# talmolab/VNL-Brax-Imitation

Hardware: AMD Instinct MI355X
Metric: env-steps/sec (whole node), rodent imitation, num_envs=4096/GPU (higher is better)
Workload: dtype f32; 1 GPU; rodent imitation rollout, single groom clip, 4096 envs/GPU: intention-policy forward (HIP) -> RodentTracking.step (5 substeps, CG 6/6) -> auto-reset on -> Transition logging (unroll 20, the 20 steps replayed as one captured hipGraph); envs_per_gpu=4096, clips=1, parallelism=env-sharded x1, no data-path collective

## Files before the change

### __graft_entry__.py

```python
from __future__ import annotations

import os
import sys

ROOT = os.path.dirname(os.path.abspath(__file__))
if ROOT not in sys.path:
    sys.path.insert(0, ROOT)


def build() -> None:
    import vnl_brax_imitation_amd
    from vnl_brax_imitation_amd.csrc import build as hip_build

    from concurrent.futures import ThreadPoolExecutor

    with ThreadPoolExecutor(5) as pool:
        futs = {v: pool.submit(hip_build.build, variant=v) for v in ("product", "spill", "noblk", "nospec", "tail")}
        paths = {v: f.result() for v, f in futs.items()}
    path = paths["product"]
    assert all(os.path.exists(p_) for p_ in paths.values()), paths
    from oracle import oracle as _oracle

    _oracle.build()
    from vnl_brax_imitation_amd import _lib

    _lib.load_library(path)
    print(f"[build] {path} ok; oracle ok")


def smoke() -> None:
    import numpy as np
    import torch

    sys.path.insert(0, os.path.join(ROOT, "tests"))
    import helpers as H
    from vnl_brax_imitation_amd.envs.rodent import RodentTracking

    assert torch.cuda.is_available(), "smoke() needs a HIP device"
    B = 256
    env = RodentTracking(H.reference_clip(), num_envs=B, device="cuda:0", **H.env_kwargs())
    rng = np.random.default_rng(0)
    sf = rng.integers(0, 235, B).astype(np.int32)
    noise = (1e-3 * rng.standard_normal((B, 74))).astype(np.float32)
    st = env.reset(start_frame=torch.from_numpy(sf), noise=torch.from_numpy(noise))
    act = np.clip(0.3 * rng.standard_normal((B, 30)), -1, 1).astype(np.float32)
    o = H.make_oracle(env, "f64")
    ost = o.env_reset(sf, noise)
    e_reset = H.scaled_err(st.pipeline_state.qacc_warmstart.cpu().numpy(), ost["qacc_warmstart"])
    e_obs = H.scaled_err(st.obs.cpu().numpy(), ost["obs"])
    import parity as P

    o32 = H.make_oracle(env, "f32")
    st, err, dev, rep, ost = P.control_step_follow(env, o, o32, sf, noise, act)
    torch.cuda.synchronize()
    print(f"[smoke] reset qacc err {e_reset:.2e}, obs err {e_obs:.2e}; control step vs oracle (following the product's "
          f"solver decisions): qvel err max {err['qvel'].max():.2e} median {np.median(err['qvel']):.2e}, qpos max "
          f"{err['qpos'].max():.2e}; reward {st.reward.mean().item():.5f} vs {ost['reward'].mean():.5f}")
    w = int(np.argmax(err["qvel"]))
    print(f"[smoke] worst env {w}: product vs float64 oracle {err['qvel'][w]:.2e}, float32 oracle vs float64 oracle "
          f"{dev['qvel'][w]:.2e} on the same env (bound: max(1e-5, {P.K_SENS} x that))")
    cp, co = P.compliance(err), P.compliance(dev)
    print(f"[smoke] envs within 1e-5 after ONE CONTROL STEP ({B} envs): product qpos {cp['qpos']:.3f} qvel {cp['qvel']:.3f} | "
          f"float32 oracle qpos {co['qpos']:.3f} qvel {co['qvel']:.3f}")
    env1 = RodentTracking(H.reference_clip(), num_envs=B, device="cuda:0", **{**H.env_kwargs(), "n_frames": 1})
    o1, o1_32 = H.make_oracle(env1, "f64"), H.make_oracle(env1, "f32")
    _, err1, dev1, rep1, _ = P.control_step_follow(env1, o1, o1_32, sf, noise, act)
    cp1, co1 = P.compliance(err1), P.compliance(dev1)
    print(f"[smoke] envs within 1e-5 after ONE SUBSTEP: product qpos {cp1['qpos']:.3f} qvel {cp1['qvel']:.3f} | float32 oracle "
          f"qpos {co1['qpos']:.3f} qvel {co1['qvel']:.3f}; followed decisions: {P.assert_legitimate(rep1)}")
    for f, idx in P.bound_violations(err1, dev1).items():
        assert len(idx) == 0, (f, idx[:8], err1[f][idx[:8]], dev1[f][idx[:8]])
    assert e_reset < 1e-4 and e_obs < 1e-5, (e_reset, e_obs)
    P.check_control_step(err, dev, rep)
    assert np.abs(st.reward.cpu().numpy() - ost["reward"]).max() < 2e-4
    assert np.array_equal(st.done.cpu().numpy(), ost["done"].astype(np.float32))
    assert torch.isfinite(st.obs).all()


if __name__ == "__main__":
    build()
    if "--smoke" in sys.argv:
        smoke()
```

### include/vnl.h

```cpp
#ifndef VNL_H_
#define VNL_H_

#include <stddef.h>
#include <stdint.h>

#ifdef __cplusplus
extern "C" {
#endif

#define VNL_OK 0
#define VNL_ERR_ARG -1
#define VNL_ERR_BLOB -2
#define VNL_ERR_HIP -3
#define VNL_ERR_NO_DEVICE -4
#define VNL_ERR_UNSUPPORTED -5

typedef struct vnl_model vnl_model;
typedef struct vnl_env vnl_env;
typedef struct vnl_policy vnl_policy;

typedef struct vnl_envspec {
  int32_t clip_frames;
  int32_t num_clips;
  int32_t ref_traj_length;
  int32_t sub_clip_length;
  int32_t n_frames;
  int32_t num_track_bodies;
  int32_t num_end_eff;
  int32_t num_appendages;
  int32_t num_joint_cols;
  int32_t com_ref_col;
  const int32_t* body_idxs;
  const int32_t* end_eff_idx;
  const int32_t* app_body;
  const int32_t* app_ref_col;
  const int32_t* joint_cols;
  float healthy_z_lo, healthy_z_hi;
  float termination_threshold;
  float body_error_multiplier;
  const float* position;
  const float* quaternion;
  const float* joints;
  const float* body_positions;
  const float* velocity;
  const float* angular_velocity;
  const float* joints_velocity;
  int32_t flags;
  float done_threshold;
  const float* center_of_mass;
  float reward_weights[6];
} vnl_envspec;
#define VNL_ENV_REWARD_OLD_STATE 1
#define VNL_ENV_TERM_MEAN 2
#define VNL_ENV_NO_RAPP 4
#define VNL_ENV_OBS_QPOS_QVEL 8
#define VNL_ENV_WEIGHTS 16
#define VNL_ENV_RACT_ACTION 32
#define VNL_ENV_METRICS_UNSCALED 64
#define VNL_ENV_TRAJ_OLD_FRAME 128

typedef struct vnl_state {
  float* qpos;
  float* qvel;
  float* act;
  float* qacc_warmstart;
  float* xpos;
  float* xquat;
  float* subtree_com1;
  float* qfrc_actuator;
  float* obs;
  float* reward;
  float* done;
  float* metrics;
  float* traj;
  float* termination_error;
  int32_t* cur_frame;
  int32_t* sub_clip_frame;
  int32_t* clip_id;
} vnl_state;

typedef struct vnl_dims {
  int32_t nq, nv, nu, nbody, njnt, ngeom_collide, ncon, nefc, obs_size, traj_size;
  int32_t workspace_floats_per_env;
  int32_t workgroups_per_cu;
  int32_t nbody_dynamic;
  int32_t kernel_specialised;
  int32_t factor_route;
} vnl_dims;

const char* vnl_last_error(void);
int vnl_version(void);

int vnl_model_create(const void* blob, size_t nbytes, vnl_model** out);
void vnl_model_destroy(vnl_model*);

int vnl_env_create(const vnl_model*, const vnl_envspec*, int32_t num_envs, int32_t device, vnl_env** out);
void vnl_env_destroy(vnl_env*);
int vnl_env_dims(const vnl_env*, vnl_dims* out);

int vnl_env_reset(vnl_env*, const int32_t* start_frame, const float* noise, const vnl_state* state, void* stream);

int vnl_env_step(vnl_env*, const float* action, const vnl_state* state, void* stream);
int vnl_env_fk(vnl_env* env, const float* qpos, const vnl_state* state, void* stream);

typedef struct vnl_domain {
  const double *cg_friction, *act_gain, *dof_damping, *dof_armature;
} vnl_domain;
int vnl_env_set_domain(vnl_env* env, const vnl_domain* domain, void* stream);

typedef struct vnl_body_domain {
  const double *body_mass, *body_inertia, *body_ipos;
} vnl_body_domain;
int vnl_env_set_body_domain(vnl_env* env, const vnl_body_domain* domain, void* stream);

int vnl_env_debug(vnl_env*, int32_t enable, int32_t* row_stride);
int vnl_env_scratch(const vnl_env*, const char* name, float** dev_ptr, int32_t* count);

typedef struct vnl_policy_spec {
  int32_t traj_size, obs_size, action_size, latent_size;
  int32_t num_encoder_layers, num_decoder_layers;
  int32_t encoder_layers[8], decoder_layers[8];
} vnl_policy_spec;

int vnl_policy_create(const vnl_policy_spec*, int32_t max_batch, int32_t device, vnl_policy** out);
void vnl_policy_destroy(vnl_policy*);
int64_t vnl_policy_num_params(const vnl_policy*);
int vnl_policy_forward(vnl_policy*, const float* params, const float* obs_mean, const float* obs_std,
                       const float* traj, const float* obs, const float* eps_latent, const float* eps_action,
                       int32_t batch, int32_t deterministic, float* action, float* raw_action, float* log_prob,
                       float* logits, float* latent_mean, float* latent_logvar,
                       const float* rand_action ,
                       float* rand_log_prob ,
                       void* stream);

typedef struct vnl_policy_noise {
  uint64_t seed;
  const int64_t* step_base;
  int64_t step_offset;
  int64_t env_offset;
  float *eps_latent_out, *eps_action_out, *rand_action_out;
} vnl_policy_noise;
int vnl_policy_forward_noise(vnl_policy*, const float* params, const float* obs_mean, const float* obs_std,
                             const float* traj, const float* obs, const vnl_policy_noise*, int32_t batch,
                             int32_t deterministic, float* action, float* raw_action, float* log_prob, float* logits,
                             float* latent_mean, float* latent_logvar, float* rand_log_prob , void* stream);

#define VNL_POST_MAX_OPS 24
typedef struct vnl_post_op {
  float* dst;
  const float* src;
  const float* first;
  float* log;
  int32_t width;
  int32_t pad_;
} vnl_post_op;
typedef struct vnl_post_desc {
  float *steps, *prev_done, *done, *truncation;
  const float* reward;
  float *log_reward, *log_discount, *log_truncation;
  int32_t episode_length, action_repeat, num_ops, pad_;
  vnl_post_op ops[VNL_POST_MAX_OPS];
} vnl_post_desc;
int vnl_rollout_post(const vnl_post_desc*, int32_t num_envs, void* stream);

typedef struct vnl_ppo_head_args {
  int32_t T, B, act, latent;
  const float *logits, *baseline, *bootstrap, *lat_mean, *lat_logvar;
  const float *raw_action, *behaviour_log_prob, *reward, *truncation, *discount, *eps_entropy;
  float entropy_cost, discounting, reward_scaling, gae_lambda, clipping_epsilon, kl_weight, min_std, var_scale;
  int32_t normalize_advantage, pad_;
  float *g_logits, *g_baseline, *g_lat_mean, *g_lat_logvar;
  float *vs, *advantages;
  float *metrics;
} vnl_ppo_head_args;
#define VNL_PPO_HEAD_WORKSPACE_FLOATS (4 + 4 * 256)
int vnl_ppo_head(const vnl_ppo_head_args*, float* workspace, void* stream);

typedef struct vnl_gather_op {
  float* dst;
  const float* src;
  int32_t T, width;
} vnl_gather_op;
typedef struct vnl_gather_desc {
  const int64_t* idx;
  int32_t N, M, num_ops, pad_;
  vnl_gather_op ops[VNL_POST_MAX_OPS];
} vnl_gather_desc;
int vnl_gather_rows(const vnl_gather_desc*, void* stream);

int vnl_adam_step(float* params, const float* grads, float* mu, float* nu, const int64_t* count, int64_t n,
                  double lr, double b1, double b2, double eps, void* stream);

typedef struct vnl_ppo_net_spec {
  int32_t traj_size, obs_size, action_size, latent_size;
  int32_t num_encoder_layers, num_decoder_layers , num_value_layers ;
  int32_t encoder_layers[8], decoder_layers[8], value_layers[8];
} vnl_ppo_net_spec;
typedef struct vnl_ppo_batch {
  const float *traj;
  const float *obs;
  const float *next_obs_last;
  const float *raw_action, *behaviour_log_prob, *reward, *truncation, *discount;
  const float *eps_latent;
  const float *eps_entropy;
  const float *obs_mean, *obs_std;
} vnl_ppo_batch;
typedef struct vnl_ppo_hparams {
  float entropy_cost, discounting, reward_scaling, gae_lambda, clipping_epsilon, kl_weight, min_std, var_scale;
  int32_t normalize_advantage, pad_;
} vnl_ppo_hparams;
typedef struct vnl_ppo_update vnl_ppo_update;
int vnl_ppo_update_create(const vnl_ppo_net_spec*, int32_t T, int32_t B, int32_t device, vnl_ppo_update** out);
void vnl_ppo_update_destroy(vnl_ppo_update*);
int64_t vnl_ppo_update_num_params(const vnl_ppo_update*);
int vnl_ppo_update_buffer(const vnl_ppo_update*, const char* name, float** dev_ptr, int64_t* count);
int vnl_ppo_minibatch_grad(vnl_ppo_update*, const float* params, const vnl_ppo_batch*, const vnl_ppo_hparams*, float* grads,
                           float* metrics, void* stream);
int vnl_ppo_minibatch_grad_part(vnl_ppo_update*, const float* params, const vnl_ppo_batch*, const vnl_ppo_hparams*, float* grads,
                                float* metrics, void* stream, int part);

typedef struct vnl_corr_plan {
  int32_t route;
  int32_t chunks, chunk_cols, row_tiles;
  int64_t workspace_floats;
} vnl_corr_plan;
int vnl_prediction_corr_plan(int32_t T, int32_t B, int32_t route_request, vnl_corr_plan* out);
int vnl_prediction_corr(const float* vs, const float* reward, float reward_scaling, int32_t T, int32_t B, int32_t route_request,
                        float* workspace, int64_t workspace_floats, float* out, void* stream);

#ifdef __cplusplus
}
#endif
#endif
```

### vnl-brax-imitation_amd/_lib.py

```python
from __future__ import annotations

import ctypes as C
import os

_HERE = os.path.dirname(os.path.abspath(__file__))
DEFAULT_LIB = os.path.join(_HERE, "csrc", "libvnl.so")

i32p = C.POINTER(C.c_int32)
f32p = C.POINTER(C.c_float)


class EnvSpec(C.Structure):
    _fields_ = [
        ("clip_frames", C.c_int32),
        ("num_clips", C.c_int32),
        ("ref_traj_length", C.c_int32),
        ("sub_clip_length", C.c_int32),
        ("n_frames", C.c_int32),
        ("num_track_bodies", C.c_int32),
        ("num_end_eff", C.c_int32),
        ("num_appendages", C.c_int32),
        ("num_joint_cols", C.c_int32),
        ("com_ref_col", C.c_int32),
        ("body_idxs", i32p),
        ("end_eff_idx", i32p),
        ("app_body", i32p),
        ("app_ref_col", i32p),
        ("joint_cols", i32p),
        ("healthy_z_lo", C.c_float),
        ("healthy_z_hi", C.c_float),
        ("termination_threshold", C.c_float),
        ("body_error_multiplier", C.c_float),
        ("position", f32p),
        ("quaternion", f32p),
        ("joints", f32p),
        ("body_positions", f32p),
        ("velocity", f32p),
        ("angular_velocity", f32p),
        ("joints_velocity", f32p),
        ("flags", C.c_int32),
        ("done_threshold", C.c_float),
        ("center_of_mass", f32p),
        ("reward_weights", C.c_float * 6),
    ]


ENV_REWARD_OLD_STATE, ENV_TERM_MEAN, ENV_NO_RAPP, ENV_OBS_QPOS_QVEL = 1, 2, 4, 8
ENV_WEIGHTS, ENV_RACT_ACTION, ENV_METRICS_UNSCALED, ENV_TRAJ_OLD_FRAME = 16, 32, 64, 128


STATE_FLOAT_FIELDS = ("qpos", "qvel", "act", "qacc_warmstart", "xpos", "xquat", "subtree_com1", "qfrc_actuator",
                      "obs", "reward", "done", "metrics", "traj", "termination_error")
STATE_INT_FIELDS = ("cur_frame", "sub_clip_frame", "clip_id")


class StatePtrs(C.Structure):
    _fields_ = [(n, C.c_void_p) for n in STATE_FLOAT_FIELDS + STATE_INT_FIELDS]


class Dims(C.Structure):
    _fields_ = [(n, C.c_int32) for n in ("nq", "nv", "nu", "nbody", "njnt", "ngeom_collide", "ncon", "nefc",
                                          "obs_size", "traj_size", "workspace_floats_per_env", "workgroups_per_cu",
                                          "nbody_dynamic", "kernel_specialised", "factor_route")]


class PolicySpec(C.Structure):
    _fields_ = [
        ("traj_size", C.c_int32),
        ("obs_size", C.c_int32),
        ("action_size", C.c_int32),
        ("latent_size", C.c_int32),
        ("num_encoder_layers", C.c_int32),
        ("num_decoder_layers", C.c_int32),
        ("encoder_layers", C.c_int32 * 8),
        ("decoder_layers", C.c_int32 * 8),
    ]


class PolicyNoise(C.Structure):
    _fields_ = [("seed", C.c_uint64), ("step_base", C.c_void_p), ("step_offset", C.c_int64), ("env_offset", C.c_int64),
                ("eps_latent_out", C.c_void_p), ("eps_action_out", C.c_void_p), ("rand_action_out", C.c_void_p)]


POST_MAX_OPS = 24


class PostOp(C.Structure):
    _fields_ = [("dst", C.c_void_p), ("src", C.c_void_p), ("first", C.c_void_p), ("log", C.c_void_p),
                ("width", C.c_int32), ("pad_", C.c_int32)]


class PostDesc(C.Structure):
    _fields_ = [(n, C.c_void_p) for n in ("steps", "prev_done", "done", "truncation", "reward", "log_reward",
                                          "log_discount", "log_truncation")] + \
               [("episode_length", C.c_int32), ("action_repeat", C.c_int32), ("num_ops", C.c_int32),
                ("pad_", C.c_int32), ("ops", PostOp * POST_MAX_OPS)]


class GatherOp(C.Structure):
    _fields_ = [("dst", C.c_void_p), ("src", C.c_void_p), ("T", C.c_int32), ("width", C.c_int32)]


class GatherDesc(C.Structure):
    _fields_ = [("idx", C.c_void_p), ("N", C.c_int32), ("M", C.c_int32), ("num_ops", C.c_int32), ("pad_", C.c_int32),
                ("ops", GatherOp * POST_MAX_OPS)]


class PPOHeadArgs(C.Structure):
    _fields_ = [(n, C.c_int32) for n in ("T", "B", "act", "latent")] + \
               [(n, C.c_void_p) for n in ("logits", "baseline", "bootstrap", "lat_mean", "lat_logvar", "raw_action",
                                          "behaviour_log_prob", "reward", "truncation", "discount", "eps_entropy")] + \
               [(n, C.c_float) for n in ("entropy_cost", "discounting", "reward_scaling", "gae_lambda",
                                         "clipping_epsilon", "kl_weight", "min_std", "var_scale")] + \
               [("normalize_advantage", C.c_int32), ("pad_", C.c_int32)] + \
               [(n, C.c_void_p) for n in ("g_logits", "g_baseline", "g_lat_mean", "g_lat_logvar", "vs", "advantages",
                                          "metrics")]


PPO_HEAD_WORKSPACE_FLOATS = 4 + 4 * 256


class PPONetSpec(C.Structure):
    _fields_ = [(n, C.c_int32) for n in ("traj_size", "obs_size", "action_size", "latent_size", "num_encoder_layers",
                                          "num_decoder_layers", "num_value_layers")] + \
               [("encoder_layers", C.c_int32 * 8), ("decoder_layers", C.c_int32 * 8), ("value_layers", C.c_int32 * 8)]


class PPOBatch(C.Structure):
    _fields_ = [(n, C.c_void_p) for n in ("traj", "obs", "next_obs_last", "raw_action", "behaviour_log_prob", "reward",
                                          "truncation", "discount", "eps_latent", "eps_entropy", "obs_mean", "obs_std")]


class PPOHParams(C.Structure):
    _fields_ = [(n, C.c_float) for n in ("entropy_cost", "discounting", "reward_scaling", "gae_lambda",
                                         "clipping_epsilon", "kl_weight", "min_std", "var_scale")] + \
               [("normalize_advantage", C.c_int32), ("pad_", C.c_int32)]

class CorrPlan(C.Structure):
    _fields_ = [(n, C.c_int32) for n in ("route", "chunks", "chunk_cols", "row_tiles")] + [("workspace_floats", C.c_int64)]


class Domain(C.Structure):
    _fields_ = [(n, C.c_void_p) for n in ("cg_friction", "act_gain", "dof_damping", "dof_armature")]

class BodyDomain(C.Structure):
    _fields_ = [(n, C.c_void_p) for n in ("body_mass", "body_inertia", "body_ipos")]


EXPORTS = (
    "vnl_last_error", "vnl_version", "vnl_model_create", "vnl_model_destroy", "vnl_env_create", "vnl_env_destroy",
    "vnl_env_dims", "vnl_env_reset", "vnl_env_step", "vnl_env_fk", "vnl_env_debug", "vnl_env_scratch", "vnl_policy_create", "vnl_policy_destroy",
    "vnl_policy_num_params", "vnl_policy_forward", "vnl_policy_forward_noise", "vnl_rollout_post", "vnl_ppo_head", "vnl_adam_step", "vnl_gather_rows",
    "vnl_ppo_update_create", "vnl_ppo_update_destroy", "vnl_ppo_update_num_params", "vnl_ppo_update_buffer",
    "vnl_ppo_minibatch_grad",
    "vnl_ppo_minibatch_grad_part",
    "vnl_env_set_domain", "vnl_env_set_body_domain",
    "vnl_prediction_corr_plan", "vnl_prediction_corr",
)
_HIP_ONLY = ("vnl_policy_", "vnl_ppo_update_", "vnl_ppo_minibatch_", "vnl_prediction_corr")


class VnlError(RuntimeError):
    pass


def _declare(lib: C.CDLL) -> C.CDLL:
    vp = C.c_void_p
    lib.vnl_last_error.restype = C.c_char_p
    lib.vnl_version.restype = C.c_int
    lib.vnl_model_create.argtypes = [vp, C.c_size_t, C.POINTER(vp)]
    lib.vnl_model_destroy.argtypes = [vp]
    lib.vnl_model_destroy.restype = None
    lib.vnl_env_create.argtypes = [vp, C.POINTER(EnvSpec), C.c_int32, C.c_int32, C.POINTER(vp)]
    lib.vnl_env_destroy.argtypes = [vp]
    lib.vnl_env_destroy.restype = None
    lib.vnl_env_dims.argtypes = [vp, C.POINTER(Dims)]
    lib.vnl_env_reset.argtypes = [vp, vp, vp, C.POINTER(StatePtrs), vp]
    lib.vnl_env_step.argtypes = [vp, vp, C.POINTER(StatePtrs), vp]
    lib.vnl_env_fk.argtypes = [vp, vp, C.POINTER(StatePtrs), vp]
    lib.vnl_env_debug.argtypes = [vp, C.c_int32, C.POINTER(C.c_int32)]
    lib.vnl_env_scratch.argtypes = [vp, C.c_char_p, C.POINTER(vp), C.POINTER(C.c_int32)]
    lib.vnl_env_set_domain.argtypes = [vp, C.POINTER(Domain), vp]
    lib.vnl_env_set_body_domain.argtypes = [vp, C.POINTER(BodyDomain), vp]
    lib.vnl_rollout_post.argtypes = [C.POINTER(PostDesc), C.c_int32, vp]
    lib.vnl_ppo_head.argtypes = [C.POINTER(PPOHeadArgs), vp, vp]
    lib.vnl_gather_rows.argtypes = [C.POINTER(GatherDesc), vp]
    lib.vnl_adam_step.argtypes = [vp, vp, vp, vp, vp, C.c_int64] + [C.c_double] * 4 + [vp]
    if hasattr(lib, "vnl_ppo_update_create"):
        lib.vnl_ppo_update_create.argtypes = [C.POINTER(PPONetSpec), C.c_int32, C.c_int32, C.c_int32, C.POINTER(vp)]
        lib.vnl_ppo_update_destroy.argtypes = [vp]
        lib.vnl_ppo_update_destroy.restype = None
        lib.vnl_ppo_update_num_params.argtypes = [vp]
        lib.vnl_ppo_update_num_params.restype = C.c_int64
        lib.vnl_ppo_update_buffer.argtypes = [vp, C.c_char_p, C.POINTER(vp), C.POINTER(C.c_int64)]
        lib.vnl_ppo_minibatch_grad.argtypes = [vp, vp, C.POINTER(PPOBatch), C.POINTER(PPOHParams), vp, vp, vp]
        lib.vnl_ppo_minibatch_grad_part.argtypes = [vp, vp, C.POINTER(PPOBatch), C.POINTER(PPOHParams), vp, vp, vp, C.c_int]
        lib.vnl_prediction_corr_plan.argtypes = [C.c_int32, C.c_int32, C.c_int32, C.POINTER(CorrPlan)]
        lib.vnl_prediction_corr.argtypes = [vp, vp, C.c_float, C.c_int32, C.c_int32, C.c_int32, vp, C.c_int64, vp, vp]
    if hasattr(lib, "vnl_policy_create"):
        lib.vnl_policy_create.argtypes = [C.POINTER(PolicySpec), C.c_int32, C.c_int32, C.POINTER(vp)]
        lib.vnl_policy_destroy.argtypes = [vp]
        lib.vnl_policy_destroy.restype = None
        lib.vnl_policy_num_params.argtypes = [vp]
        lib.vnl_policy_num_params.restype = C.c_int64
        lib.vnl_policy_forward.argtypes = [vp] + [vp] * 7 + [C.c_int32, C.c_int32] + [vp] * 6 + [vp, vp] + [vp]
        lib.vnl_policy_forward_noise.argtypes = [vp] + [vp] * 5 + [C.POINTER(PolicyNoise), C.c_int32, C.c_int32] + [vp] * 7 + [vp]
    return lib


_cache = {}


def load_library(path: str | None = None, env_only: bool = False) -> C.CDLL:
    path = os.path.abspath(path or os.environ.get("VNL_LIB", DEFAULT_LIB))
    if path not in _cache:
        if not os.path.exists(path):
            raise VnlError(
                f"HIP extension not found at {path}. Build it with `python -c 'import __graft_entry__ as g; "
                "g.build()'` (hipcc --offload-arch=gfx950). There is no CPU fallback for the rollout.")
        lib = C.CDLL(path)
        missing = [s for s in EXPORTS if not hasattr(lib, s) and not (env_only and s.startswith(_HIP_ONLY))]
        if missing:
            raise VnlError(f"{path} lacks symbols {missing}")
        _cache[path] = _declare(lib)
    return _cache[path]


def check(lib: C.CDLL, rc: int) -> None:
    if rc != 0:
        raise VnlError(f"vnl error {rc}: {lib.vnl_last_error().decode()}")
```

### vnl-brax-imitation_amd/csrc/build.py

```python
from __future__ import annotations

import os
import subprocess
import sys

HERE = os.path.dirname(os.path.abspath(__file__))
SOURCES = ["vnl_lib.hip", "vnl_policy.hip", "vnl_ppo.hip", "vnl_domain.hip"]
DEPS = SOURCES + ["vnl_env_kernels.h", "vnl_body.h", "vnl_types.h", "vnl_policy_train.h", "../../include/vnl.h"]
OUT = os.path.join(HERE, "libvnl.so")

VARIANTS = {
    "product": ("libvnl.so", ["-DVNL_KERNEL_ATTR=__attribute__((amdgpu_waves_per_eu(2,2)))"]),
    "prof": ("libvnl_prof.so", ["-DVNL_PROFILE", "-DVNL_KERNEL_ATTR=__attribute__((amdgpu_waves_per_eu(2,2)))"]),
    "knobs": ("libvnl_knobs.so", ["-DVNL_STAGE_KNOBS", "-DVNL_KERNEL_ATTR=__attribute__((amdgpu_waves_per_eu(2,2)))"]),
    "spill": ("libvnl_spill.so", ["-DVNL_KERNEL_ATTR=__attribute__((amdgpu_waves_per_eu(4,4)))"]),
    "noblk": ("libvnl_noblk.so", ["-DVNL_NO_BLK", "-DVNL_KERNEL_ATTR=__attribute__((amdgpu_waves_per_eu(2,2)))"]),
    "tail": ("libvnl_tail.so", ["-DVNL_SOLVER_TAIL", "-DVNL_KERNEL_ATTR=__attribute__((amdgpu_waves_per_eu(2,2)))"]),
    "nospec": ("libvnl_nospec.so", ["-DVNL_NO_SPEC", "-DVNL_KERNEL_ATTR=__attribute__((amdgpu_waves_per_eu(2,2)))"]),
}
ENV_KERNELS = ("vnl_step_kernel", "vnl_reset_kernel")


def resource_usage(stderr_text: str) -> dict:
    out, name = {}, None
    for line in stderr_text.splitlines():
        if "Function Name:" in line:
            name = line.split("Function Name:")[1].split()[0]
            out[name] = {}
        elif name and "remark:" in line:
            body = line.split("remark:")[1].split("[-Rpass")[0].strip()
            key, _, val = body.rpartition(":")
            try:
                out[name][key.strip()] = int(val.strip())
            except ValueError:
                pass
    return out


def build(force: bool = False, verbose: bool = False, profile: bool = False, knobs: bool = False,
          variant: str | None = None) -> str:
    variant = variant or ("prof" if profile else ("knobs" if knobs else "product"))
    fname, defs = VARIANTS[variant]
    out = os.path.join(HERE, fname)
    deps = [os.path.join(HERE, d) for d in DEPS] + [os.path.abspath(__file__)]
    newest = max(os.path.getmtime(d) for d in deps)
    if not force and os.path.exists(out) and os.path.getmtime(out) >= newest:
        return out
    hipcc = os.environ.get("HIPCC", "/opt/rocm/bin/hipcc")
    objdir = os.path.join(HERE, "_obj", variant)
    os.makedirs(objdir, exist_ok=True)
    flags = ["-Rpass-analysis=kernel-resource-usage", "--offload-arch=gfx950", "-O3", "-fno-slp-vectorize", "-std=c++17", "-fPIC"] + \
        defs + os.environ.get("VNL_HIPCC_EXTRA", "").split()
    stamp = " ".join(flags)
    headers = [d for d in deps if not d.endswith(".hip")]
    SRC_DEPS = {"vnl_lib.hip": headers, "vnl_policy.hip": [h for h in headers if h.endswith("vnl.h")] + [os.path.join(HERE, "vnl_policy_train.h")],
                "vnl_ppo.hip": [h for h in headers if h.endswith("vnl.h")] + [os.path.join(HERE, "vnl_policy_train.h")]}
    objs, remarks = [], ""
    for src in SOURCES:
        obj = os.path.join(objdir, src + ".o")
        rem = obj + ".remarks.txt"
        srcdeps = [os.path.join(HERE, src)] + [h for h in SRC_DEPS.get(src, headers) if os.path.exists(h)]
        fresh = (not force and os.path.exists(obj) and os.path.exists(rem) and
                 os.path.getmtime(obj) >= max(os.path.getmtime(d) for d in srcdeps) and
                 open(rem).readline().rstrip("\n") == stamp)
        if not fresh:
            cmd = [hipcc] + flags + ["-c", os.path.join(HERE, src), "-o", obj]
            if verbose:
                print(" ".join(cmd), file=sys.stderr)
            r = subprocess.run(cmd, stderr=subprocess.PIPE, text=True)
            if verbose or r.returncode:
                sys.stderr.write(r.stderr)
            if r.returncode:
                raise subprocess.CalledProcessError(r.returncode, cmd)
            with open(rem, "w") as f:
                f.write(stamp + "\n" + r.stderr)
        objs.append(obj)
        remarks += open(rem).read().split("\n", 1)[1]
    cmd = [hipcc, "--offload-arch=gfx950", "-shared", "-fPIC", "-o", out] + objs
    r = subprocess.run(cmd, stderr=subprocess.PIPE, text=True)
    if r.returncode:
        sys.stderr.write(r.stderr)
        raise subprocess.CalledProcessError(r.returncode, cmd)

    class _R:
        stderr = remarks
    r = _R()
    usage = resource_usage(r.stderr)
    seen = {k: [u for n, u in usage.items() if k in n] for k in ENV_KERNELS}
    missing = [k for k, v in seen.items() if not v or "Occupancy [waves/SIMD]" not in v[0]]
    if missing:
        os.remove(out)
        raise RuntimeError(f"no resource-usage remark for {missing}: cannot check the register budget of this build")
    if variant == "product":
        for k, u in ((k, u) for k, v in seen.items() for u in v):
            if u.get("ScratchSize [bytes/lane]", 0) > 64 or u["Occupancy [waves/SIMD]"] < 2:
                if os.environ.get("VNL_ALLOW_SPILL") != "1":
                    os.remove(out)
                    raise RuntimeError(
                        f"{k}: {u.get('VGPRs')} VGPRs, {u.get('ScratchSize [bytes/lane]')} B scratch per lane, "
                        f"{u['Occupancy [waves/SIMD]']} waves/SIMD -- below the two waves per SIMD without spilling that the "
                        "published numbers were measured with.  Results do not depend on spilling (tests/test_gpu_spill.py); "
                        "this gate keeps a performance regression from shipping silently: set VNL_ALLOW_SPILL=1 to build anyway")
                sys.stderr.write(f"[build] WARNING (performance): {k} uses {u.get('VGPRs')} VGPRs, "
                                 f"{u.get('ScratchSize [bytes/lane]')} B scratch per lane, "
                                 f"{u['Occupancy [waves/SIMD]']} waves/SIMD: below the two waves per SIMD without "
                                 "spilling that the published numbers were measured with\n")
    with open(os.path.join(HERE, fname + ".resources.txt"), "w") as f:
        for n, u in usage.items():
            f.write(n + " " + " ".join(f"{a}={b}" for a, b in sorted(u.items())) + "\n")
    return out


if __name__ == "__main__":
    v = next((k for k in VARIANTS if "--" + k in sys.argv), None)
    if "--profile" in sys.argv:
        v = "prof"
    print(build(force="--force" in sys.argv, verbose=True, variant=v))
```

### vnl-brax-imitation_amd/csrc/vnl_body.h

```cpp
#pragma once
#include <math.h>

#include "vnl_types.h"

#ifndef VNL_HD
#define VNL_HD __device__ __forceinline__
#endif

#ifndef VNL_FORKJOIN_DEFINED
#define VNL_LANES 64
#define VNL_ROWS_PER_LANE 8
#define VNL_ROWS_SMALL 5
#define VNL_CHAIN_WIDTH 8
#define VNL_ROWSETS_1 1
#define VNL_ROWSETS_2 2
#define VNL_FOR(i, n) for (int i = (int)lane; i < (n); i += VNL_LANES)
#define VNL_SERIAL if (lane == 0)
#define VNL_SYNC() __builtin_amdgcn_fence(__ATOMIC_ACQ_REL, "wavefront")
#define VNL_SYNC_GLOBAL()                                     \
  do {                                                        \
    __builtin_amdgcn_fence(__ATOMIC_ACQ_REL, "wavefront");    \
    asm volatile("s_waitcnt vmcnt(0)" ::: "memory");          \
    __builtin_amdgcn_fence(__ATOMIC_ACQ_REL, "wavefront");    \
  } while (0)
#define VNL_LDS_DECL(name) extern __shared__ __align__(16) vreal name[]
VNL_HD float vnl_wave_sum(float x) {
#define VNL_DPP_STEP(ctrl) x += __builtin_bit_cast(float, __builtin_amdgcn_update_dpp(0, __builtin_bit_cast(int, x), ctrl, 0xf, 0xf, true))
  VNL_DPP_STEP(0xB1);
  VNL_DPP_STEP(0x4E);
  VNL_DPP_STEP(0x141);
  VNL_DPP_STEP(0x140);
#undef VNL_DPP_STEP
  x += __builtin_bit_cast(float, __builtin_amdgcn_update_dpp(0, __builtin_bit_cast(int, x), 0x142, 0xa, 0xf, false));
  x += __builtin_bit_cast(float, __builtin_amdgcn_update_dpp(0, __builtin_bit_cast(int, x), 0x143, 0xc, 0xf, false));
  return __builtin_bit_cast(float, __builtin_amdgcn_readlane(__builtin_bit_cast(int, x), 63));
}
VNL_HD float vnl_wave_sum16(float x) {
#define VNL_DPP_STEP(ctrl) x += __builtin_bit_cast(float, __builtin_amdgcn_update_dpp(0, __builtin_bit_cast(int, x), ctrl, 0xf, 0xf, true))
  VNL_DPP_STEP(0xB1);
  VNL_DPP_STEP(0x4E);
  VNL_DPP_STEP(0x141);
  VNL_DPP_STEP(0x140);
#undef VNL_DPP_STEP
  return __builtin_bit_cast(float, __builtin_amdgcn_readlane(__builtin_bit_cast(int, x), 0));
}
VNL_HD bool vnl_wave_any(bool x) { return __ballot(x) != 0ull; }
VNL_HD float vnl_wave_scan(float x) {
#define VNL_DPP_SCAN(ctrl, rmask) \
  x += __builtin_bit_cast(float, __builtin_amdgcn_update_dpp(0, __builtin_bit_cast(int, x), ctrl, rmask, 0xf, false))
  VNL_DPP_SCAN(0x111, 0xf);
  VNL_DPP_SCAN(0x112, 0xf);
  VNL_DPP_SCAN(0x114, 0xf);
  VNL_DPP_SCAN(0x118, 0xf);
  VNL_DPP_SCAN(0x142, 0xa);
  VNL_DPP_SCAN(0x143, 0xc);
#undef VNL_DPP_SCAN
  return x;
}
#define VNL_SCAN_ADD(x, run) (x = vnl_wave_scan(x))
#define VNL_WAVE_ITEMS(n) VNL_LANES
#define VNL_PAD_ITEMS(n) (((n) + VNL_LANES - 1) / VNL_LANES * VNL_LANES)
#define VNL_SCAN_ADD_C(x, run, carry) \
  (x = vnl_wave_scan(x) + carry, carry = __builtin_bit_cast(float, __builtin_amdgcn_readlane(__builtin_bit_cast(int, x), 63)))
#define VNL_PERLANE(T, name) T name
#define VNL_AT(name, j) name
#define VNL_GETF(name, a) __builtin_bit_cast(float, __builtin_amdgcn_readlane(__builtin_bit_cast(int, name), a))
#define VNL_GETI(name, a) __builtin_amdgcn_readlane(name, a)
#define VNL_ROWGETI(name, q, l) __builtin_amdgcn_readlane(name[q], l)
#define VNL_ROWGETF(expr, q, l) __builtin_bit_cast(float, __builtin_amdgcn_readlane(__builtin_bit_cast(int, expr), l))
VNL_HD float vnl_seg_sum(float x, unsigned cont, int steps) {
#define VNL_DPP_SEG(ctrl, bit)                                                                                          \
  do {                                                                                                                  \
    const float t_ = __builtin_bit_cast(float, __builtin_amdgcn_update_dpp(0, __builtin_bit_cast(int, x), ctrl, 0xf, 0xf, true)); \
    x += (cont & (bit)) ? t_ : 0.0f;                                                                                     \
  } while (0)
  if (steps > 0) VNL_DPP_SEG(0x101, 1u);
  if (steps > 1) VNL_DPP_SEG(0x102, 2u);
  if (steps > 2) VNL_DPP_SEG(0x104, 4u);
  if (steps > 3) VNL_DPP_SEG(0x108, 8u);
#undef VNL_DPP_SEG
  return x;
}
#define VNL_SEG_SUM(part, dsc, steps) (part = vnl_seg_sum(part, (dsc) >> 28, steps))
#define VNL_WAVE_FENCE() __builtin_amdgcn_fence(__ATOMIC_ACQ_REL, "wavefront")
#define VNL_LINE_HEADERS(out, base, stride)                                                       \
  do {                                                                                            \
    int hv_ = (int)(base)[((int)lane < VNL_FAC_LINES ? (int)lane : VNL_FAC_LINES - 1) * (stride)]; \
    _Pragma("unroll") for (int k_ = 0; k_ < VNL_FAC_LINES; k_++) out[k_] = __builtin_amdgcn_readlane(hv_, k_); \
  } while (0)
#define VNL_COUNT(pred) __popcll(__ballot(pred))
#define VNL_RANK(pred, run, rank)                                                   \
  do {                                                                              \
    const unsigned long long b_ = __ballot(pred);                                   \
    rank = run + (int)__popcll(b_ & ((1ull << (threadIdx.x & 63)) - 1ull));         \
    run += (int)__popcll(b_);                                                       \
  } while (0)
#define VNL_UNIFORM_I(x) __builtin_amdgcn_readfirstlane(x)
VNL_HD float vnl_recip(float x) {
  float r = __builtin_amdgcn_rcpf(x);
  return r * (2.0f - x * r);
}
#endif

#ifdef VNL_PROFILE
#define VNL_NPROF 40
__device__ unsigned long long g_vnl_prof[VNL_NPROF];
#define VNL_PROF(i)                                                                             \
  do {                                                                                          \
    if (lane == 0) {                                                                            \
      unsigned t_ = (unsigned)__builtin_amdgcn_s_memtime();                                     \
      s[LO(prof) + (i)] += (float)(t_ - __builtin_bit_cast(unsigned, (float)s[LO(prof) + VNL_NPROF])); \
      s[LO(prof) + VNL_NPROF] = __builtin_bit_cast(float, (unsigned)__builtin_amdgcn_s_memtime()); \
    }                                                                                           \
  } while (0)
#else
#define VNL_PROF(i)
#endif

#define VNL_MINVAL vreal(1e-15)
#define VNL_MINIMP vreal(0.0001)
#define VNL_MAXIMP vreal(0.9999)

struct V3 {
  vreal x, y, z;
};
VNL_HD V3 v3(vreal x, vreal y, vreal z) { return V3{x, y, z}; }
VNL_HD V3 operator+(V3 a, V3 b) { return V3{a.x + b.x, a.y + b.y, a.z + b.z}; }
VNL_HD V3 operator-(V3 a, V3 b) { return V3{a.x - b.x, a.y - b.y, a.z - b.z}; }
VNL_HD V3 operator*(V3 a, vreal s) { return V3{a.x * s, a.y * s, a.z * s}; }
VNL_HD vreal dot(V3 a, V3 b) { return a.x * b.x + a.y * b.y + a.z * b.z; }
VNL_HD V3 cross(V3 a, V3 b) { return V3{a.y * b.z - a.z * b.y, a.z * b.x - a.x * b.z, a.x * b.y - a.y * b.x}; }
struct Q4 {
  vreal w, x, y, z;
};
VNL_HD Q4 qmul(Q4 u, Q4 v) {
  return Q4{u.w * v.w - u.x * v.x - u.y * v.y - u.z * v.z, u.w * v.x + u.x * v.w + u.y * v.z - u.z * v.y,
            u.w * v.y - u.x * v.z + u.y * v.w + u.z * v.x, u.w * v.z + u.x * v.y - u.y * v.x + u.z * v.w};
}
VNL_HD V3 qrot(V3 v, Q4 q) {
  V3 u = v3(q.x, q.y, q.z);
  vreal uv = dot(u, v), uu = dot(u, u);
  V3 c = cross(u, v);
  return u * (vreal(2.) * uv) + v * (q.w * q.w - uu) + c * (vreal(2.) * q.w);
}
struct M3 {
  vreal a[9];
};
VNL_HD M3 qmat(Q4 q) {
  M3 m;
  vreal q00 = q.w * q.w, q01 = q.w * q.x, q02 = q.w * q.y, q03 = q.w * q.z;
  vreal q11 = q.x * q.x, q12 = q.x * q.y, q13 = q.x * q.z, q22 = q.y * q.y, q23 = q.y * q.z, q33 = q.z * q.z;
  m.a[0] = q00 + q11 - q22 - q33, m.a[1] = vreal(2.) * (q12 - q03), m.a[2] = vreal(2.) * (q13 + q02);
  m.a[3] = vreal(2.) * (q12 + q03), m.a[4] = q00 - q11 + q22 - q33, m.a[5] = vreal(2.) * (q23 - q01);
  m.a[6] = vreal(2.) * (q13 - q02), m.a[7] = vreal(2.) * (q23 + q01), m.a[8] = q00 - q11 - q22 + q33;
  return m;
}
VNL_HD V3 mmul(const M3& m, V3 v) {
  return V3{m.a[0] * v.x + m.a[1] * v.y + m.a[2] * v.z, m.a[3] * v.x + m.a[4] * v.y + m.a[5] * v.z,
            m.a[6] * v.x + m.a[7] * v.y + m.a[8] * v.z};
}
struct S6 {
  V3 a, l;
};
VNL_HD S6 operator+(S6 p, S6 q) { return S6{p.a + q.a, p.l + q.l}; }
VNL_HD S6 operator*(S6 p, vreal s) { return S6{p.a * s, p.l * s}; }
VNL_HD vreal dot(S6 p, S6 q) { return dot(p.a, q.a) + dot(p.l, q.l); }
VNL_HD S6 mcross(S6 u, S6 v) { return S6{cross(u.a, v.a), cross(u.l, v.a) + cross(u.a, v.l)}; }
VNL_HD S6 mcross_force(S6 v, S6 f) { return S6{cross(v.a, f.a) + cross(v.l, f.l), cross(v.a, f.l)}; }

#if defined(__HIP_DEVICE_COMPILE__)
#define VNL_CAS __attribute__((address_space(4)))
#define VNL_TO_CAS(T, p) ((const VNL_CAS T*)(unsigned long long)(p))
#define VNL_LAUNDER(p) asm volatile("" : "+s"(p))
#else
#define VNL_CAS
#define VNL_TO_CAS(T, p) ((const T*)(p))
#define VNL_LAUNDER(p)
#endif
#define MI(f) (SP::fixed ? SP::D.f : m.f)
#define LO(f) (SP::fixed ? SP::L.f : L.f)
template <class SP>
struct EnvWaveT {
  const VNL_CAS DevModel& m;
  const VNL_CAS DevEnv& ev;
  const DevState& st;
  const VNL_CAS WsLayout& L;
  vreal* s;
  unsigned e, lane;
  const VNL_CAS KernelConsts* kc;
  int* trace;
  VNL_HD EnvWaveT with_trace(int* t) const { return EnvWaveT{m, ev, st, L, s, e, lane, kc, t}; }
  VNL_HD EnvWaveT fresh() const {
    const VNL_CAS KernelConsts* k = kc;
    VNL_LAUNDER(k);
    return EnvWaveT{k->m, k->ev, st, k->L, s, e, lane, k, trace};
  }
#ifdef VNL_PROFILE
  VNL_HD void prof_begin() const {
    if (lane == 0) {
      for (int i = 0; i < VNL_NPROF; i++) s[LO(prof) + i] = 0.f;
      s[LO(prof) + VNL_NPROF] = __builtin_bit_cast(float, (unsigned)__builtin_amdgcn_s_memtime());
    }
  }
  VNL_HD void prof_end() const {
    if (lane == 0)
      for (int i = 0; i < VNL_NPROF; i++) atomicAdd(&g_vnl_prof[i], (unsigned long long)s[LO(prof) + i]);
  }
#else
  VNL_HD void prof_begin() const {}
  VNL_HD void prof_end() const {}
#endif

  VNL_HD V3 ld3(int o) const { return V3{s[o], s[o + 1], s[o + 2]}; }
  VNL_HD void st3(int o, V3 v) const { s[o] = v.x, s[o + 1] = v.y, s[o + 2] = v.z; }
  VNL_HD Q4 ld4(int o) const { return Q4{s[o], s[o + 1], s[o + 2], s[o + 3]}; }
  VNL_HD S6 ld6(int o) const { return S6{ld3(o), ld3(o + 3)}; }
  VNL_HD void st6(int o, S6 v) const { st3(o, v.a), st3(o + 3, v.l); }
  VNL_HD static V3 t3(const vreal* t, int i) { return V3{t[3 * i], t[3 * i + 1], t[3 * i + 2]}; }
  VNL_HD static Q4 t4(const vreal* t, int i) { return Q4{t[4 * i], t[4 * i + 1], t[4 * i + 2], t[4 * i + 3]}; }

  VNL_HD S6 inert_mul(int o, S6 v) const {
    vreal ixx = s[o], iyy = s[o + 1], izz = s[o + 2], ixy = s[o + 3], ixz = s[o + 4], iyz = s[o + 5];
    V3 mp = ld3(o + 6);
    vreal mass = s[o + 9];
    V3 ang = V3{ixx * v.a.x + ixy * v.a.y + ixz * v.a.z, ixy * v.a.x + iyy * v.a.y + iyz * v.a.z,
                ixz * v.a.x + iyz * v.a.y + izz * v.a.z} +
             cross(mp, v.l);
    V3 lin = v.l * mass - cross(mp, v.a);
    return S6{ang, lin};
  }

  VNL_HD vreal* gxpos() const { return st.xpos + (size_t)e * 3 * MI(nbody_out); }
  VNL_HD vreal* gxquat() const { return st.xquat + (size_t)e * 4 * MI(nbody_out); }
  VNL_HD vreal* gqfrc_act() const { return st.qfrc_actuator + (size_t)e * MI(nv); }
  VNL_HD vreal* fac2() const { return ev.fac2 + (size_t)e * (MI(nM) + MI(nv)); }
  enum { P_MU, P_INVW, P_GAIN, P_DAMP, P_ARM, P_MASS, P_IPOS, P_INERTIA6 };
// ... 452 lines not shown
      int a = (int)lane + q * VNL_LANES;
      bool ok = a < MI(nv);
      int adr = ok ? madr(a) : 0, d = ok ? eadr(a) - adr : 0;
      dep[q] = d, last[q] = ok ? a + ndesc(a) : -1;
      dg[q] = ok ? s[LDb + adr] : vreal(1.);
#pragma unroll
      for (int c = 0; c < MAXD; c++)
        if (c < qd(q)) rr[q][c] = c < d ? s[LDb + adr + d - c] : vreal(0.);
    }
    constexpr int LW = MAXD + 4;
    int ftime[NSET], fslot[NSET];
#pragma unroll
    for (int q = 0; q < NSET; q++) {
      int a = (int)lane + q * VNL_LANES;
      fslot[q] = a < MI(nv) ? m.dof_fslot[a] : 0;
      ftime[q] = a < MI(nv) ? m.dof_ftime[a] : -1;
    }
    VNL_SYNC();
    VNL_PROF(7);
    const int nsteps = with_loop ? MI(fac_steps) : 0;
    for (int step = 0; step < nsteps; step++) {
      int npub = 0;
#pragma unroll
      for (int q = 0; q < NSET; q++) {
        bool mine = ftime[q] == step;
        npub += VNL_COUNT(mine);
        if (mine) {
          int line = sc + fslot[q] * LW, a = (int)lane + q * VNL_LANES;
#pragma unroll
          for (int c0 = 0; c0 < MAXD; c0 += CH) {
            if (c0 < qd(q) && c0 < dep[q]) {
#pragma unroll
              for (int c = c0; c < c0 + CH; c += 4)
                if (c < qd(q)) st4a(s + line + c, rr[q][c], rr[q][c + 1], rr[q][c + 2], rr[q][c + 3]);
            }
          }
          if constexpr (GUARD) {
            if (!(dg[q] > vreal(0.))) dg[q] = VNL_MINVAL;
          }
          vreal inv = vnl_recip(dg[q]);
          s[line + MAXD] = inv;
          s[line + MAXD + 1] = vreal(a);
          s[dinvb + a] = inv;
        }
      }
      VNL_WAVE_FENCE();
      unsigned match[NSET];
#pragma unroll
      for (int q = 0; q < NSET; q++) match[q] = 0u;
      int jk[VNL_FAC_LINES];
      VNL_LINE_HEADERS(jk, s + sc + MAXD + 1, LW);
#pragma unroll
      for (int k = 0; k < VNL_FAC_LINES; k++) {
        if (k < npub) {
          const int j = jk[k];
#pragma unroll
          for (int q = 0; q < NSET; q++) {
            int a = (int)lane + q * VNL_LANES;
            match[q] |= (a < j && j <= last[q]) ? (1u << k) : 0u;
          }
        }
      }
      for (int pass = 0; pass < VNL_FAC_LINES; pass++) {
        bool more = false;
#pragma unroll
        for (int q = 0; q < NSET; q++) more = more || match[q] != 0u;
        if (!vnl_wave_any(more)) break;
#pragma unroll
        for (int q = 0; q < NSET; q++) {
          if (match[q] != 0u) {
            const int k = __builtin_ctz(match[q]);
            match[q] &= match[q] - 1u;
            const vreal* line = s + sc + k * LW;
            R4 x0[CH / 4];
#pragma unroll
            for (int c = 0; c < CH; c += 4) x0[c / 4] = ld4a(line + c);
            vreal traw = line[dep[q]];
            vreal t = traw * line[MAXD];
#pragma unroll
            for (int c = 0; c < CH; c += 4) {
              R4 x = x0[c / 4];
              rr[q][c] -= t * x.x, rr[q][c + 1] -= t * x.y, rr[q][c + 2] -= t * x.z, rr[q][c + 3] -= t * x.w;
            }
#pragma unroll
            for (int c0 = CH; c0 < MAXD; c0 += CH) {
              if (c0 < qd(q) && c0 < dep[q]) {
#pragma unroll
                for (int c = c0; c < c0 + CH; c += 4) {
                  if (c < qd(q)) {
                    R4 x = ld4a(line + c);
                    rr[q][c] -= t * x.x, rr[q][c + 1] -= t * x.y, rr[q][c + 2] -= t * x.z, rr[q][c + 3] -= t * x.w;
                  }
                }
              }
            }
            dg[q] -= t * traw;
          }
        }
      }
      VNL_WAVE_FENCE();
    }
    VNL_SYNC();
    VNL_PROF(8);
#pragma unroll
    for (int q = 0; q < NSET; q++) {
      int a = (int)lane + q * VNL_LANES;
      if (a < MI(nv)) {
        int adr = madr(a), d = dep[q];
        vreal di = s[dinvb + a];
        s[LDb + adr] = dg[q];
#pragma unroll
        for (int c = 0; c < MAXD; c++)
          if (c < qd(q) && c < d) s[LDb + adr + d - c] = rr[q][c] * di;
      }
    }
    VNL_SYNC();
    VNL_PROF(9);
  }

  template <int NSET, int MAXD, int MAXD1 = MAXD>
  VNL_HD void invert_rows(int LDb) const {
    auto qd = [](int q) constexpr { return (NSET == 2 && q == 1) ? MAXD1 : MAXD; };
#pragma unroll
    for (int q = NSET - 1; q >= 0; q--) {
      vreal nn[MAXD];
      int a = (int)lane + q * VNL_LANES;
      bool ok = a < MI(nv);
      int adr = ok ? madr(a) : 0, d = ok ? eadr(a) - adr : 0;
      int own = LDb + adr;
      const vreal* pb[MAXD];
#pragma unroll
      for (int u = 1; u < MAXD; u++)
        if (u < qd(q)) pb[u] = s + LDb + (u < d ? madr(anc_of(adr + u)) : 0);
#pragma unroll
      for (int t = 1; t < MAXD; t++) {
        if (t < qd(q) && vnl_wave_any(t <= d)) {
          vreal x[MAXD];
#pragma unroll
          for (int u = 1; u < t; u++) x[u] = pb[u][t - u];
          vreal acc = t <= d ? -s[own + t] : vreal(0.);
#pragma unroll
          for (int u = 1; u < t; u++) acc -= nn[u] * x[u];
          nn[t] = acc;
        }
      }
      VNL_SYNC();
#pragma unroll
      for (int t = 1; t < MAXD; t++)
        if (t < qd(q) && t <= d) s[own + t] = nn[t];
      VNL_SYNC();
    }
  }

  template <int NSET>
  VNL_HD void factor_aba(vreal h) const {
    constexpr int LW = 16;
    const int sc = (LO(Mgrad) + 3) & ~3;
    const int VS = vstore();
    vreal* g2 = fac2();
    const int nsteps = MI(fac_steps);
    v2r U[NSET][6], diag[NSET];
    vreal S[NSET][6];
    int dep[NSET], ftime[NSET], myline[NSET], adrs[NSET];
    const unsigned char* mt[NSET];
    unsigned nxt[NSET];
#pragma unroll
    for (int q = 0; q < NSET; q++) {
      const int a = (int)lane + q * VNL_LANES;
      const bool ok = a < MI(nv);
      const int aa = ok ? a : 0;
      const S6 c = ld6(LO(cdof) + 6 * aa), f = inert_mul(LO(P) + 10 * m.dof_body[aa], c);
      S[q][0] = c.a.x, S[q][1] = c.a.y, S[q][2] = c.a.z, S[q][3] = c.l.x, S[q][4] = c.l.y, S[q][5] = c.l.z;
      U[q][0] = v2r{f.a.x, f.a.x}, U[q][1] = v2r{f.a.y, f.a.y}, U[q][2] = v2r{f.a.z, f.a.z};
      U[q][3] = v2r{f.l.x, f.l.x}, U[q][4] = v2r{f.l.y, f.l.y}, U[q][5] = v2r{f.l.z, f.l.z};
      const vreal arm = par<P_ARM>(aa);
      diag[q] = v2r{arm, arm + h * par<P_DAMP>(aa)};
      adrs[q] = madr(aa), dep[q] = eadr(aa) - adrs[q];
      myline[q] = m.dof_fslot[aa];
      ftime[q] = ok ? m.dof_ftime[aa] : -1;
      mt[q] = m.fac_match + (size_t)aa * nsteps;
      nxt[q] = (ok && nsteps > 0) ? mt[q][0] : 0u;
    }
    VNL_SYNC();
    VNL_PROF(7);
    for (int step = 0; step < nsteps; step++) {
      unsigned cur[NSET];
#pragma unroll
      for (int q = 0; q < NSET; q++) {
        cur[q] = nxt[q];
        nxt[q] = (ftime[q] >= 0 && step + 1 < nsteps) ? mt[q][step + 1] : 0u;
        if (ftime[q] == step) {
          const int a = (int)lane + q * VNL_LANES;
          v2r D = diag[q];
#pragma unroll
          for (int i = 0; i < 6; i++) D += v2r{S[q][i], S[q][i]} * U[q][i];
          const v2r iv = v2r{vnl_recip(D[0]), vnl_recip(D[1])};
          vreal* ln = s + sc + myline[q] * LW;
          st4a(ln, U[q][0][0], U[q][0][1], U[q][1][0], U[q][1][1]);
          st4a(ln + 4, U[q][2][0], U[q][2][1], U[q][3][0], U[q][3][1]);
          st4a(ln + 8, U[q][4][0], U[q][4][1], U[q][5][0], U[q][5][1]);
          st4a(ln + 12, iv[0], iv[1], (vreal)(adrs[q] + dep[q]), vreal(0.));
          vreal* vs = s + VS + 12 * a;
          const v2r v0 = U[q][0] * iv, v1 = U[q][1] * iv, v2 = U[q][2] * iv, v3_ = U[q][3] * iv, v4 = U[q][4] * iv, v5 = U[q][5] * iv;
          st4a(vs, v0[0], v0[1], v1[0], v1[1]);
          st4a(vs + 4, v2[0], v2[1], v3_[0], v3_[1]);
          st4a(vs + 8, v4[0], v4[1], v5[0], v5[1]);
          s[LO(dinv) + a] = iv[0];
          g2[MI(nM) + a] = iv[1];
        }
      }
      VNL_WAVE_FENCE();
      for (int pass = 0; pass < VNL_FAC_LINES; pass++) {
        bool more = false;
#pragma unroll
        for (int q = 0; q < NSET; q++) more = more || cur[q] != 0u;
        if (!vnl_wave_any(more)) break;
#pragma unroll
        for (int q = 0; q < NSET; q++) {
          if (cur[q] != 0u) {
            const int k = __builtin_ctz(cur[q]);
            cur[q] &= cur[q] - 1u;
            const vreal* ln = s + sc + k * LW;
            const R4 u0 = ld4a(ln), u1 = ld4a(ln + 4), u2 = ld4a(ln + 8), hd = ld4a(ln + 12);
            const v2r Uk[6] = {v2r{u0.x, u0.y}, v2r{u0.z, u0.w}, v2r{u1.x, u1.y}, v2r{u1.z, u1.w}, v2r{u2.x, u2.y}, v2r{u2.z, u2.w}};
            v2r pa = v2r{S[q][0], S[q][0]} * Uk[0], pb = v2r{S[q][1], S[q][1]} * Uk[1];
            pa += v2r{S[q][2], S[q][2]} * Uk[2], pb += v2r{S[q][3], S[q][3]} * Uk[3];
            pa += v2r{S[q][4], S[q][4]} * Uk[4], pb += v2r{S[q][5], S[q][5]} * Uk[5];
            const v2r Lk = (pa + pb) * v2r{hd.x, hd.y};
#pragma unroll
            for (int i = 0; i < 6; i++) U[q][i] -= Lk * Uk[i];
            s[LO(LD) + (int)hd.z - dep[q]] = Lk[0];
          }
        }
      }
      VNL_WAVE_FENCE();
    }
    VNL_SYNC();
    VNL_PROF(8);
    VNL_PROF(9);
  }

  VNL_HD int vstore() const { return vnl_vstore(LO(P)); }
  VNL_HD int cvel_at() const { return vnl_cvel_at(LO(P), LO(smooth), MI(nbody), MI(nv)); }

  template <int NSET, bool GUESTS>
  VNL_HD void invert_aba(vreal* g2) const {
    const int VS = vstore();
    const unsigned char* an = (const unsigned char*)(s + LO(tab_anc));
    auto load_v = [&](int r, v2r* C) {
      const vreal* vs = s + VS + 12 * r;
      const R4 a = ld4a(vs), b = ld4a(vs + 4), c = ld4a(vs + 8);
      C[0] = v2r{a.x, a.y}, C[1] = v2r{a.z, a.w}, C[2] = v2r{b.x, b.y}, C[3] = v2r{b.z, b.w}, C[4] = v2r{c.x, c.y}, C[5] = v2r{c.z, c.w};
    };
#pragma unroll
    for (int q = 0; q < NSET; q++) {
      const int a = (int)lane + q * VNL_LANES;
      int row = a < MI(nv) ? a : -1, next = -1;
      if (GUESTS && q == 0 && m.fac_guest) next = m.fac_guest[lane];
      int adr = madr(row >= 0 ? row : 0), d = row >= 0 ? eadr(row) - adr : 0, tt = 0;
      v2r C[6];
      load_v(row >= 0 ? row : 0, C);
      int jn = an[adr + (d > 0 ? 1 : 0)];
      while (vnl_wave_any(row >= 0)) {
        if (row >= 0 && tt == d) {
          row = next, next = -1;
          if (row >= 0) {
            adr = madr(row), d = eadr(row) - adr, tt = 0;
            load_v(row, C);
            jn = an[adr + (d > 0 ? 1 : 0)];
          }
        }
        if (row >= 0 && tt < d) {
          const int j = jn;
          jn = an[adr + (tt + 2 <= d ? tt + 2 : d)];
          const S6 c = ld6(LO(cdof) + 6 * j);
          v2r V[6];
          load_v(j, V);
          v2r pa = v2r{c.a.x, c.a.x} * C[0], pb = v2r{c.a.y, c.a.y} * C[1];
          pa += v2r{c.a.z, c.a.z} * C[2], pb += v2r{c.l.x, c.l.x} * C[3];
          pa += v2r{c.l.y, c.l.y} * C[4], pb += v2r{c.l.z, c.l.z} * C[5];
          const v2r n = -(pa + pb);
#pragma unroll
          for (int i = 0; i < 6; i++) C[i] += n * V[i];
          tt++;
          s[LO(LD) + adr + tt] = n[0], g2[adr + tt] = n[1];
        }
      }
    }
    VNL_SYNC();
  }

  VNL_HD int route(int at) const { return (MI(fac_route) >> at) & 0xf; }
  VNL_HD bool factor_pair_ok() const { return route(VNL_ROUTE_PAIR) != 0; }
  VNL_HD void factor_both(vreal h) const {
    if (route(VNL_ROUTE_PAIR) == 1) factor_aba<VNL_ROWSETS_1>(h);
    else factor_aba<VNL_ROWSETS_2>(h);
  }
  VNL_HD void factor(bool with_loop = true) const {
    const int sc = (LO(Ma) + 3) & ~3;
    switch (route(VNL_ROUTE_QM_FACTOR)) {
      case VNL_ROUTE_ROWS16: factor_rows_at<VNL_ROWSETS_1, 16>(with_loop, LO(LD), LO(dinv), sc); break;
      case VNL_ROUTE_ROWS36: factor_rows_at<VNL_ROWSETS_1, 36>(with_loop, LO(LD), LO(dinv), sc); break;
      case VNL_ROUTE_ROWS36X2: factor_rows_at<VNL_ROWSETS_2, 36, 16>(with_loop, LO(LD), LO(dinv), sc); break;
      default: factor_lds(LO(LD), LO(dinv), false);
    }
  }
  VNL_HD void invert_factor(int LDb) const {
    switch (route(VNL_ROUTE_QM_INVERSE)) {
      case VNL_ROUTE_ROWS16: invert_rows<VNL_ROWSETS_1, 16>(LDb); break;
      case VNL_ROUTE_ROWS36: invert_rows<VNL_ROWSETS_1, 36>(LDb); break;
      case VNL_ROUTE_ROWS36X2: invert_rows<VNL_ROWSETS_2, 36, 16>(LDb); break;
      default: invert_factor_lds();
    }
  }
  VNL_HD void invert_factor() const { invert_factor(LO(LD)); }

  template <int ST = 1>
  VNL_HD vreal row_dot(int adr, int dep, int in, int LDb) const {
    const unsigned char* an = (const unsigned char*)(s + LO(tab_anc)) + adr;
    const vreal* row = s + LDb + ST * adr;
    vreal acc = vreal(0.);
    int t = 1;
    constexpr int W = VNL_CHAIN_WIDTH;
    for (; t + W - 1 <= dep; t += W) {
      int j[W];
      vreal l[W], x[W];
#pragma unroll
      for (int u = 0; u < W; u++) j[u] = an[t + u];
#pragma unroll
      for (int u = 0; u < W; u++) l[u] = row[ST * (t + u)];
#pragma unroll
      for (int u = 0; u < W; u++) x[u] = s[in + j[u]];
      vreal p0 = vreal(0.), p1 = vreal(0.);
#pragma unroll
      for (int u = 0; u < W; u += 2) p0 += l[u] * x[u], p1 += l[u + 1] * x[u + 1];
      acc += p0 + p1;
    }
    if (t <= dep) {
      int j[W];
      vreal l[W], x[W];
#pragma unroll
      for (int u = 0; u < W; u++) {
        const int tt = t + u <= dep ? t + u : dep;
        j[u] = an[tt], l[u] = row[ST * tt];
      }
#pragma unroll
      for (int u = 0; u < W; u++) x[u] = s[in + j[u]];
      vreal p0 = vreal(0.), p1 = vreal(0.);
#pragma unroll
      for (int u = 0; u < W; u += 2) {
        p0 += t + u <= dep ? l[u] * x[u] : vreal(0.);
        p1 += t + u + 1 <= dep ? l[u + 1] * x[u + 1] : vreal(0.);
      }
      acc += p0 + p1;
    }
    return acc;
  }

  VNL_HD void row_apply(int in, int out, bool scale_by_dinv, int LDb, int dinvb) const {
    VNL_FOR(i, MI(nv)) {
      int adr = madr(i), dep = eadr(i) - adr;
      vreal acc = s[in + i] + row_dot(adr, dep, in, LDb);
      s[out + i] = scale_by_dinv ? acc * s[dinvb + i] : acc;
    }
    VNL_SYNC();
  }
  template <int ST = 1>
  VNL_HD void col_apply(int in, int out, int dmode , int LDb, int dinvb) const {
    VNL_FOR(a, MI(nv)) {
      int da = eadr(a) - madr(a), nd = ndesc(a);
      vreal acc = s[in + a];
      const unsigned short* ea = (const unsigned short*)(s + LO(tab_madr)) + MI(nv);
      const vreal* ld = s + LDb - ST * da;
      int i = a + 1, iend = a + nd;
      constexpr int W = VNL_CHAIN_WIDTH;
      for (; i + W - 1 <= iend; i += W) {
        int e[W];
        vreal l[W], x[W];
#pragma unroll
        for (int u = 0; u < W; u++) e[u] = ea[i + u];
#pragma unroll
        for (int u = 0; u < W; u++) x[u] = s[in + i + u];
#pragma unroll
        for (int u = 0; u < W; u++) l[u] = ld[ST * e[u]];
        vreal p0 = vreal(0.), p1 = vreal(0.);
#pragma unroll
        for (int u = 0; u < W; u += 2) p0 += l[u] * x[u], p1 += l[u + 1] * x[u + 1];
        acc += p0 + p1;
      }
      if (i <= iend) {
        int e[W];
        vreal l[W], x[W];
#pragma unroll
// ... 1272 lines not shown
```

### vnl-brax-imitation_amd/csrc/vnl_domain.hip

```cpp
#include <hip/hip_runtime.h>
#include <stdint.h>

#include "../../include/vnl.h"
#ifdef VNL_PROFILE
#define g_vnl_prof g_vnl_prof_domain
#endif
#include "vnl_env_kernels.h"

int vnl_domain_reset_(const KernelConsts* kc, int spec, int B, size_t lds, void* stream, const DevState& ds, const int* start_frame,
                      const vreal* noise, vreal* dump, int* trace) {
  if (spec)
    hipLaunchKernelGGL((vnl_reset_kernel<VnlSpecDom<VnlSpecRodent>>), dim3(B), dim3(64), lds, (hipStream_t)stream, kc, ds,
                       start_frame, noise, dump, trace);
  else
    hipLaunchKernelGGL((vnl_reset_kernel<VnlSpecDom<VnlSpecGeneric>>), dim3(B), dim3(64), lds, (hipStream_t)stream, kc, ds,
                       start_frame, noise, dump, trace);
  return (int)hipGetLastError();
}

int vnl_domain_step_(const KernelConsts* kc, int spec, int B, size_t lds, void* stream, const DevState& ds, const vreal* action,
                     vreal* dump, vreal* dump_mid, int* trace) {
  if (spec)
    hipLaunchKernelGGL((vnl_step_kernel<VnlSpecDom<VnlSpecRodent>>), dim3(B), dim3(64), lds, (hipStream_t)stream, kc, ds,
                       action, dump, dump_mid, trace);
  else
    hipLaunchKernelGGL((vnl_step_kernel<VnlSpecDom<VnlSpecGeneric>>), dim3(B), dim3(64), lds, (hipStream_t)stream, kc, ds,
                       action, dump, dump_mid, trace);
  return (int)hipGetLastError();
}
```

### vnl-brax-imitation_amd/csrc/vnl_env_kernels.h

```cpp
#pragma once
#include "vnl_body.h"

#ifndef VNL_KERNEL_ATTR
#define VNL_KERNEL_ATTR
#endif
#define VNL_ENV_KERNEL __launch_bounds__(64) VNL_KERNEL_ATTR

template <class SP>
__global__ void VNL_ENV_KERNEL vnl_step_kernel(const KernelConsts* kc, DevState st, const vreal* action,
                                                      vreal* dump, vreal* dump_mid, int* trace) {
  VNL_LDS_DECL(lds);
  const VNL_CAS KernelConsts* k = VNL_TO_CAS(KernelConsts, kc);
  EnvWaveT<SP> w{k->m, k->ev, st, k->L, lds, blockIdx.x, threadIdx.x, k, nullptr};
  w.step(action, dump_mid, trace);
  if (dump) w.dump(dump);
}

template <class SP>
__global__ void VNL_ENV_KERNEL vnl_reset_kernel(const KernelConsts* kc, DevState st, const int* start_frame,
                                                       const vreal* noise, vreal* dump, int* trace) {
  VNL_LDS_DECL(lds);
  const VNL_CAS KernelConsts* k = VNL_TO_CAS(KernelConsts, kc);
  EnvWaveT<SP> w{k->m, k->ev, st, k->L, lds, blockIdx.x, threadIdx.x, k, nullptr};
  w.reset(start_frame, noise, trace);
  if (dump) w.dump(dump);
}
```

### vnl-brax-imitation_amd/csrc/vnl_lib.hip

```cpp
#include <hip/hip_runtime.h>
#include <stdint.h>
#include <stdio.h>
#include <stdlib.h>
#include <string.h>

#include <algorithm>
#include <cmath>
#include <cstddef>
#include <map>
#include <string>
#include <vector>

#include "../../include/vnl.h"
#include "vnl_body.h"

static thread_local char g_err[512] = "";
static int fail(int code, const char* fmt, const char* a = "", const char* b = "") {
  snprintf(g_err, sizeof(g_err), fmt, a, b);
  return code;
}
#define HIPCHK(call)                                                              \
  do {                                                                            \
    hipError_t e_ = (call);                                                       \
    if (e_ != hipSuccess) return fail(VNL_ERR_HIP, "%s: %s", #call, hipGetErrorString(e_)); \
// ... 149 lines not shown
                          std::vector<double>* Mo, std::vector<double>* nipo, std::vector<double>* nIo) {
  const FuseMap* fm = &fmr;
  const int nb = fm->nb_out;
  std::vector<double>&M = *Mo, &nip = *nipo, &nI = *nIo;
  if (nd == nb) {
    M.assign(mass, mass + nb), nip.assign(ipos, ipos + 3 * (size_t)nb), nI.assign(ifull, ifull + 9 * (size_t)nb);
    return;
  }
  M.assign(nd, 0.0);
  std::vector<double> mc(3 * (size_t)nd, 0.0), J(9 * (size_t)nd, 0.0);
  for (int b = 0; b < nb; b++) {
    const int dyn = fm->out_dyn[b];
    double R[9], c[3], t[3];
    qmat_d(&fm->out_quat[4 * (size_t)b], R), mulv_d(R, &ipos[3 * (size_t)b], t);
    for (int k = 0; k < 3; k++) c[k] = fm->out_pos[3 * (size_t)b + k] + t[k];
    const double m = mass[b], cc = c[0] * c[0] + c[1] * c[1] + c[2] * c[2];
    M[dyn] += m;
    for (int k = 0; k < 3; k++) mc[3 * (size_t)dyn + k] += m * c[k];
    const double* I = &ifull[9 * (size_t)b];
    for (int r = 0; r < 3; r++)
      for (int q = 0; q < 3; q++) {
        double v = 0;
        for (int a = 0; a < 3; a++)
          for (int e = 0; e < 3; e++) v += R[3 * r + a] * I[3 * a + e] * R[3 * q + e];
        J[9 * (size_t)dyn + 3 * r + q] += v + m * ((r == q ? cc : 0.0) - c[r] * c[q]);
      }
  }
  nip.assign(3 * (size_t)nd, 0.0), nI.assign(9 * (size_t)nd, 0.0);
  for (int dyn = 0; dyn < nd; dyn++) {
    double c[3] = {0, 0, 0};
    if (M[dyn] > 0)
      for (int k = 0; k < 3; k++) c[k] = mc[3 * (size_t)dyn + k] / M[dyn];
    else
      for (int k = 0; k < 3; k++) c[k] = ipos[3 * (size_t)fm->body_out[dyn] + k];
    const double cc = c[0] * c[0] + c[1] * c[1] + c[2] * c[2];
    for (int k = 0; k < 3; k++) nip[3 * (size_t)dyn + k] = c[k];
    for (int r = 0; r < 3; r++)
      for (int q = 0; q < 3; q++) nI[9 * (size_t)dyn + 3 * r + q] = J[9 * (size_t)dyn + 3 * r + q] - M[dyn] * ((r == q ? cc : 0.0) - c[r] * c[q]);
  }
}
static std::vector<double> pack_inertia6(const std::vector<double>& f9) {
  const size_t nb = f9.size() / 9;
  std::vector<double> i6(6 * nb);
  for (size_t b = 0; b < nb; b++) {
    const double* s = &f9[9 * b];
    double* o = &i6[6 * b];
    o[0] = s[0], o[1] = s[4], o[2] = s[8], o[3] = s[1], o[4] = s[2], o[5] = s[5];
  }
  return i6;
}
static double total_mass_inv_of(const std::vector<double>& mass) {
  double tm = 0;
  for (double x : mass) tm += x;
  return 1.0 / tm;
}
static bool fuse_welded_bodies(const vnl_model& in, vnl_model* out, FuseMap* fm) {
  const int nb = (int)in.scalar("nbody");
  const auto& bp = in.i.at("body_parentid");
  const auto& jn = in.i.at("body_jntnum");
  std::vector<char> keep(nb, 1);
  int nd = 0;
  for (int b = 0; b < nb; b++) {
    keep[b] = (b < 2 || jn[b] > 0) ? 1 : 0;
    if (!keep[b]) {
      int a = bp[b];
      while (a > 1 && !keep[a]) a = bp[a];
      if (a == 0) keep[b] = 1;
    }
    nd += keep[b];
  }
  fm->nb_out = nb;
  fm->out_dyn.assign(nb, 0), fm->out_pos.assign(3 * (size_t)nb, 0.0), fm->out_quat.assign(4 * (size_t)nb, 0.0);
  fm->body_out.clear();
  const auto& bpos = in.f.at("body_pos");
  const auto& bquat = in.f.at("body_quat");
  for (int b = 0, k = 0; b < nb; b++) {
    double* fp = &fm->out_pos[3 * (size_t)b];
    double* fq = &fm->out_quat[4 * (size_t)b];
    if (keep[b]) {
      fm->out_dyn[b] = k++, fm->body_out.push_back(b);
      fq[0] = 1.0;
    } else {
      const int p = bp[b];
      fm->out_dyn[b] = fm->out_dyn[p];
      double R[9], t[3];
      qmat_d(&fm->out_quat[4 * (size_t)p], R), mulv_d(R, &bpos[3 * (size_t)b], t);
      for (int c = 0; c < 3; c++) fp[c] = fm->out_pos[3 * (size_t)p + c] + t[c];
      qmul_d(&fm->out_quat[4 * (size_t)p], &bquat[4 * (size_t)b], fq);
    }
  }
  if (nd == nb) return false;
  *out = in;
  out->f["nbody"] = {(double)nd};
  auto pick_i = [&](const char* k) {
    std::vector<int> v;
    for (int b = 0; b < nb; b++)
      if (keep[b]) v.push_back(in.i.at(k)[b]);
    out->i[k] = v;
  };
  auto pick_f = [&](const char* k, int w) {
    std::vector<double> v;
    for (int b = 0; b < nb; b++)
      if (keep[b]) v.insert(v.end(), in.f.at(k).begin() + (size_t)w * b, in.f.at(k).begin() + (size_t)w * (b + 1));
    out->f[k] = v;
  };
  pick_i("body_jntadr"), pick_i("body_jntnum"), pick_i("body_rootid"), pick_i("body_dofadr"), pick_i("body_dofnum");
  pick_f("body_invweight0", 2);
  std::vector<int> par;
  std::vector<double> pos, quat;
  for (int b = 0; b < nb; b++) {
    if (!keep[b]) continue;
    const int p = b > 0 ? bp[b] : 0;
    par.push_back(fm->out_dyn[p]);
    double R[9], t[3], q[4];
    qmat_d(&fm->out_quat[4 * (size_t)p], R), mulv_d(R, &bpos[3 * (size_t)b], t);
    for (int c = 0; c < 3; c++) pos.push_back(fm->out_pos[3 * (size_t)p + c] + t[c]);
    qmul_d(&fm->out_quat[4 * (size_t)p], &bquat[4 * (size_t)b], q);
    quat.insert(quat.end(), q, q + 4);
  }
  out->i["body_parentid"] = par, out->f["body_pos"] = pos, out->f["body_quat"] = quat;
  std::vector<double> M, nip, nI;
  fuse_inertial(*fm, nd, in.f.at("body_mass").data(), in.f.at("body_ipos").data(), in.f.at("body_inertia_full").data(), &M, &nip, &nI);
  out->f["body_mass"] = M, out->f["body_ipos"] = nip, out->f["body_inertia_full"] = nI;
  for (const char* k : {"jnt_bodyid", "dof_bodyid"}) {
    std::vector<int> v = in.i.at(k);
    for (int& x : v) x = fm->out_dyn[x];
    out->i[k] = v;
  }
  {
    const auto& gb = in.i.at("cg_bodyid");
    const auto& gp = in.f.at("cg_pos");
    const auto& gq = in.f.at("cg_quat");
    const auto& iw0 = in.f.at("body_invweight0");
    std::vector<int> nb_(gb.size());
    std::vector<double> np = gp, nq = gq, giw(gb.size());
    for (size_t g = 0; g < gb.size(); g++) {
      const int ob = gb[g];
      nb_[g] = fm->out_dyn[ob], giw[g] = iw0[2 * (size_t)ob];
      double R[9], t[3];
      qmat_d(&fm->out_quat[4 * (size_t)ob], R), mulv_d(R, &gp[3 * g], t);
      for (int c = 0; c < 3; c++) np[3 * g + c] = fm->out_pos[3 * (size_t)ob + c] + t[c];
      qmul_d(&fm->out_quat[4 * (size_t)ob], &gq[4 * g], &nq[4 * g]);
    }
    out->i["cg_bodyid"] = nb_, out->f["cg_pos"] = np, out->f["cg_quat"] = nq, out->f["cg_body_invweight0"] = giw;
  }
  return true;
}

static double contact_invweight(double t, double mu, double impratio) { return (t + mu * mu * t) * 2 * mu * mu / impratio; }

static VnlDims dims_of(const DevModel& d) {
  return VnlDims{d.nq, d.nv, d.nu, d.nbody, d.njnt, d.ncg, d.ncon, d.nlimit, d.nefc, d.nM, d.iterations, d.ls_iterations, d.eulerdamp,
                 d.root_free, d.max_depth, d.jump_rounds, d.fac_steps, d.fac_route, d.solver_newton, d.blk_cfg, d.path_runs, d.nbody_out};
}

static int choose_routes(const DevModel& d, int deep1) {
  const WsLayout L = vnl_make_layout(dims_of(d));
  const int nv = d.nv, md = d.max_depth, set1 = VNL_ROWSETS_1 * VNL_LANES, set2 = VNL_ROWSETS_2 * VNL_LANES;
  auto rows = [&](int room) {
    auto fits = [&](int maxd) { return room < 0 || VNL_FAC_LINES * (maxd + 4) <= room; };
    if (nv <= set1 && md < 16 && fits(16)) return VNL_ROUTE_ROWS16;
    if (nv <= set1 && md < 36 && fits(36)) return VNL_ROUTE_ROWS36;
    if (nv <= set2 && md < 36 && deep1 < 16 && fits(36)) return VNL_ROUTE_ROWS36X2;
    return VNL_ROUTE_LDS;
  };
  const int factor = rows(4 * nv - 3);
  const int inverse = rows(-1);
  const int hessian = d.solver_newton ? rows(L.smooth - ((L.P + 3 * d.nefc + 3) & ~3)) : 0;
  const bool pair = d.eulerdamp && nv <= set2 && vnl_vstore(L.P) + 12 * nv <= vnl_cvel_at(L.P, L.smooth, d.nbody, nv) &&
                    VNL_FAC_LINES * 16 + 3 <= 6 * nv;
  return factor << VNL_ROUTE_QM_FACTOR | inverse << VNL_ROUTE_QM_INVERSE | hessian << VNL_ROUTE_HESSIAN |
         (pair ? (nv <= set1 ? 1 : 2) : 0) << VNL_ROUTE_PAIR;
}

static int build_dev_model(vnl_env* env, const vnl_model* hm) {
  DevModel& d = env->dm;
  vnl_model fused;
  FuseMap fmap;
  for (const char* k : {"body_parentid", "body_jntnum"})
    if (hm->i.find(k) == hm->i.end()) return fail(VNL_ERR_BLOB, "blob section %s missing", k);
  for (const char* k : {"body_pos", "body_quat", "body_ipos", "body_inertia_full", "body_mass", "body_invweight0", "cg_pos", "cg_quat"})
    if (hm->f.find(k) == hm->f.end()) return fail(VNL_ERR_BLOB, "blob section %s missing", k);
  for (const char* k : {"jnt_bodyid", "dof_bodyid", "cg_bodyid", "body_jntadr", "body_rootid", "body_dofadr", "body_dofnum"})
    if (hm->i.find(k) == hm->i.end()) return fail(VNL_ERR_BLOB, "blob section %s missing", k);
  {
    env->mass0 = hm->f.at("body_mass"), env->ipos0 = hm->f.at("body_ipos"), env->ifull0 = hm->f.at("body_inertia_full");
    const size_t nbo = env->mass0.size();
    if (env->ipos0.size() != 3 * nbo || env->ifull0.size() != 9 * nbo || (double)nbo != hm->scalar("nbody"))
      return fail(VNL_ERR_BLOB, "blob section %s missing or of unexpected size", "body_ipos / body_inertia_full");
    if (hm->has_f("body_inertia", 3 * nbo) && hm->has_f("body_iquat", 4 * nbo))
      env->inertia0 = hm->f.at("body_inertia"), env->iquat0 = hm->f.at("body_iquat");
  }
  if (fuse_welded_bodies(*hm, &fused, &fmap)) hm = &fused;
  d.nbody_out = fmap.nb_out;
  env->fmap = new FuseMap(fmap);
  env->dyn_dofnum = hm->i.at("body_dofnum");
  auto S = [&](const char* k) { return hm->scalar(k); };
  d.nq = (int)S("nq"), d.nv = (int)S("nv"), d.nu = (int)S("nu"), d.nbody = (int)S("nbody"), d.njnt = (int)S("njnt");
  d.ncg = (int)S("ncg"), d.ncon = (int)S("ncon"), d.nlimit = (int)S("nlimit"), d.nefc = (int)S("nefc");
  d.iterations = (int)S("iterations"), d.ls_iterations = (int)S("ls_iterations"), d.eulerdamp = (int)S("eulerdamp");
  d.dt = (vreal)S("timestep"), d.tolerance = (vreal)S("tolerance"), d.ls_tolerance = (vreal)S("ls_tolerance");
  d.solver_newton = S("solver_newton") != 0;
  d.dbg_stage = 0, d.dbg_count = 0;
#ifdef VNL_STAGE_KNOBS
  if (const char* dbg = getenv("VNL_DBG_REPEAT")) sscanf(dbg, "%d:%d", &d.dbg_stage, &d.dbg_count);
#endif
  d.scale = (vreal)(S("meaninertia") * (d.nv > 1 ? d.nv : 1));
  const int nb = d.nbody, nj = d.njnt, nv = d.nv, nu = d.nu, ng = d.ncg;
  std::vector<int> nsub_host, limrow_host;
  struct Need {
    const char* k;
    size_t n;
    bool isint;
  } needs[] = {{"body_parentid", (size_t)nb, true}, {"body_jntadr", (size_t)nb, true}, {"body_jntnum", (size_t)nb, true},
               {"body_rootid", (size_t)nb, true}, {"body_dofadr", (size_t)nb, true}, {"body_dofnum", (size_t)nb, true}, {"body_pos", 3u * nb, false}, {"body_quat", 4u * nb, false},
               {"body_ipos", 3u * nb, false}, {"body_inertia_full", 9u * nb, false}, {"body_mass", (size_t)nb, false},
               {"body_invweight0", 2u * nb, false}, {"jnt_type", (size_t)nj, true}, {"jnt_qposadr", (size_t)nj, true},
               {"jnt_dofadr", (size_t)nj, true}, {"jnt_bodyid", (size_t)nj, true}, {"jnt_limited", (size_t)nj, true}, {"jnt_pos", 3u * nj, false},
               {"jnt_axis", 3u * nj, false}, {"jnt_range", 2u * nj, false}, {"jnt_stiffness", (size_t)nj, false},
               {"jnt_margin", (size_t)nj, false}, {"jnt_solref", 2u * nj, false}, {"jnt_solimp", 5u * nj, false},
               {"qpos0", (size_t)d.nq, false}, {"qpos_spring", (size_t)d.nq, false}, {"dof_bodyid", (size_t)nv, true},
               {"dof_parentid", (size_t)nv, true}, {"dof_armature", (size_t)nv, false},
               {"dof_damping", (size_t)nv, false}, {"dof_invweight0", (size_t)nv, false}, {"act_dof", (size_t)nu, true},
               {"act_ctrllimited", (size_t)nu, true}, {"act_gain", (size_t)nu, false}, {"act_gear", (size_t)nu, false},
               {"act_tau", (size_t)nu, false}, {"act_ctrlrange", 2u * nu, false}, {"cg_type", (size_t)ng, true},
               {"cg_bodyid", (size_t)ng, true}, {"cg_ncon", (size_t)ng, true}, {"cg_conadr", (size_t)ng, true},
               {"cg_pos", 3u * ng, false}, {"cg_quat", 4u * ng, false}, {"cg_size", 3u * ng, false},
               {"cg_friction", 3u * ng, false}, {"cg_solref", 2u * ng, false}, {"cg_solimp", 5u * ng, false},
               {"cg_margin", (size_t)ng, false}, {"gravity", 3, false}, {"plane_pos", 3, false},
               {"plane_normal", 3, false}};
  for (auto& n : needs)
    if (!(n.isint ? hm->has_i(n.k, n.n) : hm->has_f(n.k, n.n)))
      return fail(VNL_ERR_BLOB, "blob section %s missing or of unexpected size", n.k);
  auto F = [&](const char* k) -> const std::vector<double>& { return hm->f.at(k); };
  auto I = [&](const char* k) -> const std::vector<int>& { return hm->i.at(k); };

  for (int b = 1; b < nb; b++)
    if (I("body_rootid")[b] != 1) return fail(VNL_ERR_UNSUPPORTED, "model must be a single tree rooted at body 1");
  const auto& jt = I("jnt_type");
  for (int j = 0; j < nj; j++)
    if (jt[j] != VNL_JNT_FREE && jt[j] != VNL_JNT_HINGE)
      return fail(VNL_ERR_UNSUPPORTED, "only free and hinge joints are implemented");
  d.root_free = (I("body_jntnum")[1] > 0 && jt[I("body_jntadr")[1]] == VNL_JNT_FREE) ? 1 : 0;
  d.root_px = (vreal)F("body_pos")[3], d.root_py = (vreal)F("body_pos")[4], d.root_pz = (vreal)F("body_pos")[5];
  d.gx = (vreal)F("gravity")[0], d.gy = (vreal)F("gravity")[1], d.gz = (vreal)F("gravity")[2];
  const auto& pn = F("plane_normal");
  const auto& pp = F("plane_pos");
  d.pnx = (vreal)pn[0], d.pny = (vreal)pn[1], d.pnz = (vreal)pn[2];
  d.ppx = (vreal)pp[0], d.ppy = (vreal)pp[1], d.ppz = (vreal)pp[2];
  {
    double a[3] = {pn[0], pn[1], pn[2]}, bb[3] = {0, 0, 0};
    if (-0.5 < a[1] && a[1] < 0.5) bb[1] = 1; else bb[2] = 1;
    double ab = a[0] * bb[0] + a[1] * bb[1] + a[2] * bb[2];
    for (int k = 0; k < 3; k++) bb[k] -= a[k] * ab;
    double nn = sqrt(bb[0] * bb[0] + bb[1] * bb[1] + bb[2] * bb[2]);
    d.t1x = (vreal)(bb[0] / nn), d.t1y = (vreal)(bb[1] / nn), d.t1z = (vreal)(bb[2] / nn);
  }
  d.total_mass_inv = (vreal)total_mass_inv_of(F("body_mass"));

  int rc;
#define UPF(name, vec) if ((rc = upload<vreal, double>(env, vec, &d.name)) != VNL_OK) return rc;
#define UPI(name, vec) if ((rc = upload<int, int>(env, vec, &d.name)) != VNL_OK) return rc;
  UPI(body_parent, I("body_parentid")) UPI(body_jntadr, I("body_jntadr")) UPI(body_jntnum, I("body_jntnum"))
  UPI(out_dyn, fmap.out_dyn) UPI(body_out, fmap.body_out) UPF(out_pos, fmap.out_pos) UPF(out_quat, fmap.out_quat)
  {
    std::vector<int> da(nb, 0), dn(nb, 0);
    for (int b = 0; b < nb; b++) {
      dn[b] = I("body_dofnum")[b];
      da[b] = dn[b] > 0 ? I("body_dofadr")[b] : 0;
    }
    UPI(body_dofadr, da) UPI(body_dofnum, dn)
    const auto& bp = I("body_parentid");
    std::vector<int> nsub(nb, 0);
    for (int b = nb - 1; b > 0; b--) nsub[bp[b]] += nsub[b] + 1;
    for (int b = 1; b < nb; b++)
      for (int c = b + 1; c <= b + nsub[b]; c++) {
        bool in = false;
        for (int a = c; a > 0; a = bp[a]) in |= (a == b);
        if (!in) return fail(VNL_ERR_UNSUPPORTED, "body numbering is not depth-first");
      }
    UPI(body_nsub, nsub)
    nsub_host = nsub;
    std::vector<int> lastdof(nb, nv);
    for (int b = 1; b < nb; b++) lastdof[b] = dn[b] > 0 ? da[b] + dn[b] - 1 : lastdof[bp[b]];
    UPI(body_lastdof, lastdof)
    {
      const auto& dpar = I("dof_parentid");
      std::vector<int> seg(8 * (size_t)nb, 0);
      int most = 1;
      for (int b = 1; b < nb; b++) {
        {
          std::vector<int> anc;
          for (int a = b; a > 0; a = bp[a]) anc.push_back(a);
          std::sort(anc.begin(), anc.end());
          int nseg = 0;
          for (size_t i = 0; i < anc.size();) {
            size_t j = i;
            while (j + 1 < anc.size() && anc[j + 1] == anc[j] + 1) j++;
            if (nseg == 4) return fail(VNL_ERR_UNSUPPORTED, "a body has more than 4 runs of consecutive ancestor bodies");
            seg[8 * b + 4 + nseg++] = anc[i] | ((anc[j] + 1) << 8);
            i = j + 1;
          }
          most = nseg > most ? nseg : most;
        }
        std::vector<int> path;
        for (int dd = lastdof[b] < nv ? lastdof[b] : -1; dd >= 0; dd = dpar[dd]) path.push_back(dd);
        std::sort(path.begin(), path.end());
        int nseg = 0;
        for (size_t i = 0; i < path.size();) {
          size_t j = i;
          while (j + 1 < path.size() && path[j + 1] == path[j] + 1) j++;
          if (nseg == 4) return fail(VNL_ERR_UNSUPPORTED, "a body path has more than 4 runs of consecutive dofs");
          seg[8 * b + nseg++] = path[i] | ((path[j] + 1) << 8);
          i = j + 1;
        }
        most = nseg > most ? nseg : most;
      }
      d.path_runs = most;
      UPI(body_pathseg, seg)
    }
    int bdepth = 0;
    for (int b = 1; b < nb; b++) {
      int dd = 0;
      for (int a = b; a > 0; a = bp[a]) dd++;
      bdepth = dd > bdepth ? dd : bdepth;
    }
    int rounds = 0;
    while ((1 << rounds) < bdepth) rounds++;
    d.jump_rounds = rounds;
    std::vector<unsigned char> jump((size_t)(rounds > 0 ? rounds : 1) * nb, 0);
    for (int b = 0; b < nb; b++) jump[b] = (unsigned char)bp[b];
    for (int r = 1; r < rounds; r++)
      for (int b = 0; b < nb; b++) jump[(size_t)r * nb + b] = jump[(size_t)(r - 1) * nb + jump[(size_t)(r - 1) * nb + b]];
    {
      const unsigned char* dp = nullptr;
      if ((rc = upload<unsigned char, unsigned char>(env, jump, &dp)) != VNL_OK) return rc;
      d.jump = dp;
    }
  }
  UPF(body_pos, F("body_pos")) UPF(body_quat, F("body_quat")) UPF(body_ipos, F("body_ipos")) UPF(body_mass, F("body_mass"))
  UPF(body_inertia6, pack_inertia6(F("body_inertia_full")))
  UPI(jnt_type, jt) UPI(jnt_qposadr, I("jnt_qposadr")) UPI(jnt_dofadr, I("jnt_dofadr")) UPI(jnt_body, I("jnt_bodyid"))
  UPF(jnt_pos, F("jnt_pos")) UPF(jnt_axis, F("jnt_axis")) UPF(jnt_stiffness, F("jnt_stiffness"))
  {
    std::vector<double> q0(nj), qs(nj);
    for (int j = 0; j < nj; j++) q0[j] = F("qpos0")[I("jnt_qposadr")[j]], qs[j] = F("qpos_spring")[I("jnt_qposadr")[j]];
    UPF(jnt_qpos0, q0) UPF(jnt_springref, qs)
  }
  {
    std::vector<int> qa, dof;
    std::vector<double> lo, hi, mg, iw, sr, si;
    for (int j = 0; j < nj; j++) {
      if (!I("jnt_limited")[j] || jt[j] != VNL_JNT_HINGE) continue;
      qa.push_back(I("jnt_qposadr")[j]), dof.push_back(I("jnt_dofadr")[j]);
      lo.push_back(F("jnt_range")[2 * j]), hi.push_back(F("jnt_range")[2 * j + 1]), mg.push_back(F("jnt_margin")[j]);
      iw.push_back(F("dof_invweight0")[I("jnt_dofadr")[j]]);
      for (int k = 0; k < 2; k++) sr.push_back(F("jnt_solref")[2 * j + k]);
      for (int k = 0; k < 5; k++) si.push_back(F("jnt_solimp")[5 * j + k]);
    }
    if ((int)qa.size() != d.nlimit) return fail(VNL_ERR_BLOB, "nlimit does not match jnt_limited");
    UPI(lim_qadr, qa) UPI(lim_dof, dof) UPF(lim_lo, lo) UPF(lim_hi, hi) UPF(lim_margin, mg) UPF(lim_invweight, iw)
    UPF(lim_solref, sr) UPF(lim_solimp, si)
  }
  {
    const auto& par = I("dof_parentid");
    std::vector<int> madr(nv), depth(nv), anc;
    for (int i = 0; i < nv; i++) {
      madr[i] = (int)anc.size();
      int dep = 0;
      for (int j = i; j >= 0; j = par[j]) anc.push_back(j), dep++;
      depth[i] = dep - 1;
    }
    d.nM = (int)anc.size();
    std::vector<int> row(anc.size());
    for (int i = 0; i < nv; i++)
      for (int a = 0; a <= depth[i]; a++) row[madr[i] + a] = i;
    std::vector<int> ndesc(nv, 0);
    for (int i = 0; i < nv; i++)
      for (int j = par[i]; j >= 0; j = par[j]) ndesc[j]++;
    for (int a = 0; a < nv; a++)
      for (int i = a + 1; i <= a + ndesc[a]; i++) {
        bool is_desc = false;
        for (int j = par[i]; j >= 0; j = par[j]) is_desc |= (j == a);
        if (!is_desc) return fail(VNL_ERR_UNSUPPORTED, "dof numbering is not depth-first");
      }
    int maxd = 0;
    for (int i = 0; i < nv; i++) maxd = depth[i] > maxd ? depth[i] : maxd;
    d.max_depth = maxd;
    if (nv > 255 || nb > 255 || maxd > 62) return fail(VNL_ERR_UNSUPPORTED, "model too large for 8-bit index tables");
    std::vector<unsigned char> lvl_tab;
    std::vector<int> lvl_start(maxd + 2, 0);
    for (int lev = 0; lev <= maxd; lev++) {
      lvl_start[lev] = (int)lvl_tab.size();
      int cnt = 0;
      for (int i = 0; i < nv; i++)
        if (depth[i] == lev) lvl_tab.push_back((unsigned char)i), cnt++;
      if (cnt * lev > 2 * nv) return fail(VNL_ERR_UNSUPPORTED, "tree level too wide for the inversion staging buffer");
    }
    lvl_start[maxd + 1] = (int)lvl_tab.size();
    for (int v : lvl_start) lvl_tab.push_back((unsigned char)v);
    {
      const unsigned char* dp = nullptr;
      if ((rc = upload<unsigned char, unsigned char>(env, lvl_tab, &dp)) != VNL_OK) return rc;
      d.lvl_tab = dp;
    }
    std::vector<int> limrow(nv, -1);
    {
      int r = 0;
      for (int j = 0; j < nj; j++)
        if (I("jnt_limited")[j] && jt[j] == VNL_JNT_HINGE) limrow[I("jnt_dofadr")[j]] = r++;
    }
    UPI(dof_body, I("dof_bodyid")) UPI(dof_Madr, madr) UPI(dof_depth, depth) UPI(M_anc, anc) UPI(M_row, row)
    UPI(dof_ndesc, ndesc)
    limrow_host = limrow;
    std::vector<int> ftime(nv, 0), fslot(nv, 0), count;
    for (int j = nv - 1; j >= 0; j--) {
      int t = 0;
      for (int i = j + 1; i <= j + ndesc[j]; i++)
        if (par[i] == j) t = ftime[i] + 1 > t ? ftime[i] + 1 : t;
      while ((int)count.size() <= t) count.push_back(0);
      while (count[t] >= VNL_FAC_LINES) {
        t++;
        if ((int)count.size() <= t) count.push_back(0);
      }
      ftime[j] = t, fslot[j] = count[t]++;
    }
    for (int j = nv - 1; j >= 0; j--)
      if (par[j] >= 0 && ftime[par[j]] <= ftime[j]) return fail(VNL_ERR_UNSUPPORTED, "factorisation schedule is not causal");
    d.fac_steps = (int)count.size();
    UPI(dof_ftime, ftime) UPI(dof_fslot, fslot)
    {
      int deep1 = 0;
      for (int j = 64; j < nv; j++) deep1 = depth[j] > deep1 ? depth[j] : deep1;
      d.fac_route = choose_routes(d, deep1);
    }
    {
      d.fac_guest = nullptr;
      if (nv > 64 && nv <= 128) {
        std::vector<int> guest(64, -1), order;
        for (int j = 64; j < nv; j++) order.push_back(j);
        std::sort(order.begin(), order.end(), [&](int x, int y) { return depth[x] > depth[y]; });
        bool ok = true;
        for (int j : order) {
          int host = -1;
          for (int l = 0; l < 64 && host < 0; l++)
            if (guest[l] < 0 && depth[l] <= 12) host = l;
          if (host < 0 || depth[j] > 24) ok = false;
          else guest[host] = j;
        }
        if (ok) UPI(fac_guest, guest)
      }
    }
    {
      const int nst = d.fac_steps;
      std::vector<unsigned char> match((size_t)nv * (nst > 0 ? nst : 1), 0);
      for (int j = 0; j < nv; j++)
        for (int a = par[j]; a >= 0; a = par[a]) match[(size_t)a * nst + ftime[j]] |= (unsigned char)(1u << fslot[j]);
      const unsigned char* dp = nullptr;
      if ((rc = upload<unsigned char, unsigned char>(env, match, &dp)) != VNL_OK) return rc;
      d.fac_match = dp;
    }
    {
      d.blk_tab = nullptr, d.blk_cfg = 0;
      auto pack = [&](bool colform, std::vector<unsigned>& out, int& trips, int& steps) -> bool {
        struct Item { int r, nblk; };
        std::vector<Item> items;
        int total = 0, longest = 1;
        for (int r = 0; r < nv; r++) {
          const int len = colform ? ndesc[r] : depth[r], nb_ = len > 0 ? (len + VNL_BLK_W - 1) / VNL_BLK_W : 1;
          if (nb_ > 16) return false;
          items.push_back({r, nb_}), total += nb_, longest = nb_ > longest ? nb_ : longest;
        }
        std::stable_sort(items.begin(), items.end(), [](const Item& a, const Item& b) { return a.nblk > b.nblk; });
        steps = longest > 8 ? 4 : (longest > 4 ? 3 : (longest > 2 ? 2 : (longest > 1 ? 1 : 0)));
        for (trips = (total + 63) / 64; trips <= 8; trips++) {
          std::vector<int> fill(trips * 4, 0);
          std::vector<unsigned> tab((size_t)trips * 64, 0u);
          bool ok = true;
          for (const Item& it : items) {
            int bin = -1;
            for (int b = 0; b < trips * 4 && bin < 0; b++)
              if (fill[b] + it.nblk <= 16) bin = b;
            if (bin < 0) { ok = false; break; }
            const int len = colform ? ndesc[it.r] : depth[it.r];
            for (int k = 0; k < it.nblk; k++) {
              const int slot = bin * 16 + fill[bin] + k, left = it.nblk - 1 - k;
              const int n = len - VNL_BLK_W * k > VNL_BLK_W ? VNL_BLK_W : (len - VNL_BLK_W * k > 0 ? len - VNL_BLK_W * k : 0);
              unsigned payload;
              if (colform) payload = (unsigned)(n > 0 ? it.r + 1 + VNL_BLK_W * k : it.r) | ((unsigned)depth[it.r] << 7);
              else payload = (unsigned)(madr[it.r] + (n > 0 ? 1 + VNL_BLK_W * k : 0));
              unsigned mask = 0;
              for (int b = 0; b < 4; b++)
                if ((1 << b) <= left) mask |= 1u << b;
              tab[slot] = payload | ((unsigned)n << 16) | ((unsigned)it.r << 20) | ((k == 0 ? 1u : 0u) << 27) | (mask << 28);
            }
            fill[bin] += it.nblk;
          }
          if (ok) {
            out = tab;
            return true;
          }
        }
        return false;
      };
      std::vector<unsigned> rowtab, coltab;
      int tr = 0, tc = 0, sr = 0, sc = 0;
      if (nv <= 127 && maxd <= 63 && d.nM < 65536 && pack(false, rowtab, tr, sr) && pack(true, coltab, tc, sc)) {
        rowtab.insert(rowtab.end(), coltab.begin(), coltab.end());
        const unsigned* dp = nullptr;
        if ((rc = upload<unsigned, unsigned>(env, rowtab, &dp)) != VNL_OK) return rc;
        d.blk_tab = dp;
        d.blk_cfg = tr | (tc << 4) | (sr << 8) | (sc << 12);
      }
    }
  }
  UPF(dof_armature, F("dof_armature")) UPF(dof_damping, F("dof_damping"))
  UPI(act_dof, I("act_dof")) UPI(act_limited, I("act_ctrllimited")) UPF(act_gain, F("act_gain"))
  {
    std::vector<int> packed(nv, 0), cnt(nv, 0);
    bool ok = nu < 255;
    for (int a = 0; a < nu && ok; a++) {
      const int dd = I("act_dof")[a];
      if (dd < 0 || dd >= nv) continue;
      if (cnt[dd] == 4) ok = false;
      else packed[dd] |= (a + 1) << (8 * cnt[dd]++);
    }
    d.dof_act = nullptr;
    if (ok) UPI(dof_act, packed)
  }
  UPF(act_tau, F("act_tau")) UPF(act_gear, F("act_gear"))
  {
    std::vector<double> lo(nu), hi(nu);
    for (int k = 0; k < nu; k++) lo[k] = F("act_ctrlrange")[2 * k], hi[k] = F("act_ctrlrange")[2 * k + 1];
    UPF(act_lo, lo) UPF(act_hi, hi)
  }
  UPI(cg_type, I("cg_type")) UPI(cg_body, I("cg_bodyid")) UPI(cg_conadr, I("cg_conadr")) UPI(cg_ncon, I("cg_ncon"))
  {
    std::vector<int> cgeom(d.ncon, 0);
    for (int g = 0; g < ng; g++)
      for (int q = 0; q < I("cg_ncon")[g]; q++) cgeom[I("cg_conadr")[g] + q] = g;
    const auto& cgb = I("cg_bodyid");
    const bool ok_ = d.ncon <= 64 && d.nlimit < 1023 && ng < 256;
    if (!ok_) return fail(VNL_ERR_UNSUPPORTED, "more than 64 contacts / 255 collision geoms / 1022 limit rows (constraint_force scans the contact wrenches in one wave)");
    std::vector<int> order(d.ncon);
    for (int c = 0; c < d.ncon; c++) order[c] = c;
    std::stable_sort(order.begin(), order.end(), [&](int a, int b) { return cgb[cgeom[a]] < cgb[cgeom[b]]; });
    if (ok_)
      for (int k = 0; k < d.ncon; k++) cgeom[k] |= order[k] << 8;
    UPI(con_geom, cgeom)
    std::vector<int> packed(nv);
    for (int dd = 0; dd < nv; dd++) {
      int b0 = I("dof_bodyid")[dd], b1 = b0 + nsub_host[b0], c0 = 0, c1 = 0;
      while (c0 < d.ncon && cgb[cgeom[order[c0]] & 0xff] < b0) c0++;
      c1 = c0;
      while (c1 < d.ncon && cgb[cgeom[order[c1]] & 0xff] <= b1) c1++;
      packed[dd] = (limrow_host[dd] + 1) | (c0 << 10) | (c1 << 18) | ((ok_ ? 1 : 0) << 26);
    }
    UPI(dof_limrow, packed)
  }
  UPF(cg_pos, F("cg_pos")) UPF(cg_quat, F("cg_quat")) UPF(cg_size, F("cg_size")) UPF(cg_solref, F("cg_solref"))
  UPF(cg_solimp, F("cg_solimp")) UPF(cg_margin, F("cg_margin"))
  {
    std::vector<double> mu(ng), iw(ng);
    double impratio = S("impratio");
    env->cg_t.assign(ng, 0.0);
    for (int g = 0; g < ng; g++) {
      mu[g] = F("cg_friction")[3 * g];
      double t = F("body_invweight0")[0] + (hm->f.count("cg_body_invweight0") ? F("cg_body_invweight0")[g]
                                                                                : F("body_invweight0")[2 * (size_t)I("cg_bodyid")[g]]);
      iw[g] = contact_invweight(t, mu[g], impratio);
      env->cg_t[g] = t;
    }
    UPF(cg_mu, mu) UPF(cg_invweight, iw)
    env->impratio = impratio, env->mu0 = mu;
    env->gain0 = F("act_gain"), env->damp0 = F("dof_damping"), env->arm0 = F("dof_armature");
  }
#undef UPF
#undef UPI
  if (d.solver_newton) {
    std::vector<int> nlim(nv, 0);
    for (int j = 0; j < nj; j++)
      if (I("jnt_limited")[j] && I("jnt_type")[j] == VNL_JNT_HINGE) {
// ... 86 lines not shown
  for (int k = 0; ok && k < e.napp; k++)
    ok = es->app_body[k] >= 0 && es->app_body[k] < d.nbody_out && es->app_ref_col[k] >= 0 && es->app_ref_col[k] < e.nb;
  for (int k = 0; ok && k < e.njc; k++) ok = es->joint_cols[k] >= 0 && es->joint_cols[k] < d.nq - 7;
  if (!ok) {
    vnl_env_destroy(env);
    return fail(VNL_ERR_ARG, "vnl_envspec: index out of range or unsupported shape");
  }
  size_t CT = (size_t)e.C * e.T, nj = d.nq - 7;
#define UP(call)              \
  if ((rc = (call)) != VNL_OK) { \
    vnl_env_destroy(env);     \
    return rc;                \
  }
  UP(upload_raw<int>(env, es->body_idxs, e.nb, &e.body_idxs))
  UP(upload_raw<int>(env, es->end_eff_idx, e.nee, &e.end_eff_idx))
  UP(upload_raw<int>(env, es->app_body, e.napp, &e.app_body))
  UP(upload_raw<int>(env, es->app_ref_col, e.napp, &e.app_ref_col))
  UP(upload_raw<int>(env, es->joint_cols, e.njc, &e.joint_cols))
  UP(upload_raw<float>(env, es->position, CT * 3, &e.position))
  UP(upload_raw<float>(env, es->quaternion, CT * 4, &e.quaternion))
  UP(upload_raw<float>(env, es->joints, CT * nj, &e.joints))
  UP(upload_raw<float>(env, es->body_positions, CT * e.nb * 3, &e.body_positions))
  UP(upload_raw<float>(env, es->velocity, CT * 3, &e.velocity))
  UP(upload_raw<float>(env, es->angular_velocity, CT * 3, &e.angular_velocity))
  UP(upload_raw<float>(env, es->joints_velocity, CT * nj, &e.joints_velocity))
  if (es->center_of_mass) UP(upload_raw<float>(env, es->center_of_mass, CT * 3, &e.center_of_mass))
#undef UP
  {
    void* p = nullptr;
    HIPCHK(hipMalloc(&p, (size_t)num_envs * (d.nM + d.nv) * sizeof(vreal)));
    env->allocs.push_back(p);
    e.fac2 = (vreal*)p;
  }
  layout(env);
  env->spec = (same_dims(dims_of(env->dm), VnlSpecRodent::D) && same_layout(env->L, VnlSpecRodent::L)) ? 1 : 0;
#ifdef VNL_NO_SPEC
  env->spec = 0;
#endif
  env->lds_bytes = (size_t)env->L.total * sizeof(vreal);
#ifdef VNL_STAGE_KNOBS
  if (const char* padk = getenv("VNL_DBG_LDS_BYTES")) {
    size_t want = (size_t)atol(padk);
    if (want > env->lds_bytes) env->lds_bytes = want;
  }
#endif
  if (6 * d.nbody > 512) {
    vnl_env_destroy(env);
    return fail(VNL_ERR_UNSUPPORTED, "more than 85 dynamic bodies (the per-body scans of bias_forces keep 8 elements per lane)");
  }
  if (d.nu > d.nv) {
    vnl_env_destroy(env);
    return fail(VNL_ERR_UNSUPPORTED, "more actuators than dofs (the actuator forces are staged in two dof vectors)");
  }
  if (d.nefc > 512) {
    vnl_env_destroy(env);
    return fail(VNL_ERR_UNSUPPORTED, "more than 512 constraint rows (line-search rows are register-resident)");
  }
  if (env->lds_bytes > 64 * 1024) {
    vnl_env_destroy(env);
    return fail(VNL_ERR_UNSUPPORTED, "model too large: per-env working set exceeds 64 KB of LDS");
  }
  {
    int nb_ = 0;
    hipError_t r = env->spec ? hipOccupancyMaxActiveBlocksPerMultiprocessor(&nb_, vnl_step_kernel<VnlSpecRodent>, 64, env->lds_bytes)
                             : hipOccupancyMaxActiveBlocksPerMultiprocessor(&nb_, vnl_step_kernel<VnlSpecGeneric>, 64, env->lds_bytes);
    if (r == hipSuccess) env->blocks_per_cu = nb_;
  }
  {
    KernelConsts host{env->dm, env->de, env->L};
    void* p = nullptr;
    HIPCHK(hipMalloc(&p, sizeof(KernelConsts)));
    env->allocs.push_back(p);
    HIPCHK(hipMemcpy(p, &host, sizeof(KernelConsts), hipMemcpyHostToDevice));
    env->kc = (KernelConsts*)p;
  }
  *out = env;
  return VNL_OK;
}

extern "C" int vnl_env_dims(const vnl_env* env, vnl_dims* o) {
  if (!env || !o) return fail(VNL_ERR_ARG, "vnl_env_dims: null argument");
  const DevModel& d = env->dm;
  o->nq = d.nq, o->nv = d.nv, o->nu = d.nu, o->nbody = d.nbody_out, o->njnt = d.njnt, o->ngeom_collide = d.ncg;
  o->ncon = d.ncon, o->nefc = d.nefc, o->obs_size = env->de.obs_size, o->traj_size = env->de.traj_size;
  o->workspace_floats_per_env = env->L.total;
  o->workgroups_per_cu = env->blocks_per_cu;
  o->nbody_dynamic = d.nbody, o->kernel_specialised = env->spec;
  o->factor_route = d.fac_route;
  return VNL_OK;
}

extern "C" int vnl_env_scratch(const vnl_env* env, const char* name, float** dev_ptr, int32_t* count) {
  if (!env || !name || !dev_ptr || !count) return fail(VNL_ERR_ARG, "vnl_env_scratch: null argument");
  if (strncmp(name, "dom_", 4) == 0) {
    if (!env->has_dom) return fail(VNL_ERR_ARG, "vnl_env_scratch: %s: the env has no domain (vnl_env_set_domain / vnl_env_set_body_domain)", name);
    const DevModel& d = env->dm;
    const size_t B = (size_t)env->B;
    const size_t n4 = B * (2 * d.ncg + d.nu + 2 * d.nv), nd = (size_t)d.nbody;
    const struct { const char* k; size_t off; int n; } tabs[] = {
        {"dom_mu", 0, d.ncg}, {"dom_invw", B * d.ncg, d.ncg}, {"dom_gain", 2 * B * d.ncg, d.nu},
        {"dom_damp", B * (2 * d.ncg + d.nu), d.nv}, {"dom_arm", B * (2 * d.ncg + d.nu + d.nv), d.nv},
        {"dom_mass", n4, d.nbody}, {"dom_ipos", n4 + B * nd, 3 * d.nbody}, {"dom_inertia6", n4 + 4 * B * nd, 6 * d.nbody},
        {"dom_tminv", n4 + 10 * B * nd, 1}};
    for (const auto& t : tabs)
      if (strcmp(name, t.k) == 0) {
        *dev_ptr = (float*)(env->dom + t.off);
        *count = t.n;
        return VNL_OK;
      }
    return fail(VNL_ERR_ARG, "unknown scratch section %s", name);
  }
  if (!env->dump) return fail(VNL_ERR_ARG, "scratch dump is off: call vnl_env_debug(env, 1) before reset/step");
  if (strcmp(name, "solver_trace") == 0) {
    *dev_ptr = (float*)env->trace;
    *count = (env->de.n_frames > 0 ? env->de.n_frames : 1) * VNL_TRACE_INTS;
    return VNL_OK;
  }
  auto it = env->sections.find(name);
  if (it == env->sections.end()) return fail(VNL_ERR_ARG, "unknown scratch section %s", name);
  *dev_ptr = (float*)(env->dump + it->second.first);
  *count = it->second.second;
  return VNL_OK;
}

extern "C" int vnl_env_debug(vnl_env* env, int32_t enable, int32_t* row_stride) {
  if (!env) return fail(VNL_ERR_ARG, "vnl_env_debug: null argument");
  if (enable < 0 || enable > 2) return fail(VNL_ERR_ARG, "vnl_env_debug: mode must be 0, 1 or 2");
  if (enable && !env->dump) {
    void* p = nullptr;
    HIPCHK(hipMalloc(&p, (size_t)env->L.total * env->B * sizeof(vreal)));
    env->allocs.push_back(p);
    env->dump = (vreal*)p;
    const size_t nt = (size_t)env->B * (env->de.n_frames > 0 ? env->de.n_frames : 1) * VNL_TRACE_INTS * sizeof(int);
    HIPCHK(hipMalloc(&p, nt));
    env->allocs.push_back(p);
    HIPCHK(hipMemset(p, 0, nt));
    env->trace = (int*)p;
  }
  env->debug = enable;
  if (row_stride) *row_stride = env->L.total;
  return VNL_OK;
}

__global__ void __launch_bounds__(64) vnl_fk_kernel(const KernelConsts* kc, DevState st, const vreal* qpos) {
  VNL_LDS_DECL(lds);
  const VNL_CAS KernelConsts* k = VNL_TO_CAS(KernelConsts, kc);
  EnvWave w{k->m, k->ev, st, k->L, lds, blockIdx.x, threadIdx.x, k, nullptr};
  w.fk(qpos);
}

int vnl_domain_reset_(const KernelConsts* kc, int spec, int B, size_t lds, void* stream, const DevState& ds, const int* start_frame,
                      const vreal* noise, vreal* dump, int* trace);
int vnl_domain_step_(const KernelConsts* kc, int spec, int B, size_t lds, void* stream, const DevState& ds, const vreal* action,
                     vreal* dump, vreal* dump_mid, int* trace);

static int to_dev_state(const vnl_state* s, DevState* d) {
  const void* ptrs[] = {s->qpos, s->qvel, s->act, s->qacc_warmstart, s->xpos, s->xquat, s->subtree_com1,
                        s->qfrc_actuator, s->obs, s->reward, s->done, s->metrics, s->traj, s->termination_error,
                        s->cur_frame, s->sub_clip_frame, s->clip_id};
  for (const void* p : ptrs)
    if (!p) return fail(VNL_ERR_ARG, "vnl_state: null buffer");
  d->qpos = (vreal*)s->qpos, d->qvel = (vreal*)s->qvel, d->act = (vreal*)s->act, d->warm = (vreal*)s->qacc_warmstart;
  d->xpos = (vreal*)s->xpos, d->xquat = (vreal*)s->xquat, d->com1 = (vreal*)s->subtree_com1;
  d->qfrc_actuator = (vreal*)s->qfrc_actuator, d->obs = (vreal*)s->obs, d->reward = (vreal*)s->reward;
  d->done = (vreal*)s->done, d->metrics = (vreal*)s->metrics, d->traj = (vreal*)s->traj;
  d->term_err = (vreal*)s->termination_error, d->cur_frame = s->cur_frame, d->sub_clip_frame = s->sub_clip_frame;
  d->clip_id = s->clip_id;
  return VNL_OK;
}

extern "C" int vnl_env_reset(vnl_env* env, const int32_t* start_frame, const float* noise, const vnl_state* state,
                             void* stream) {
  if (!env || !start_frame || !noise || !state) return fail(VNL_ERR_ARG, "vnl_env_reset: null argument");
  DevState ds;
  int rc = to_dev_state(state, &ds);
  if (rc != VNL_OK) return rc;
  DeviceGuard guard(env->device);
  if (!guard.ok) return fail(VNL_ERR_HIP, "hipSetDevice failed");
  if (env->has_dom) {
    HIPCHK((hipError_t)vnl_domain_reset_(env->kc, env->spec, env->B, env->lds_bytes, stream, ds, (const int*)start_frame,
                                         (const vreal*)noise, env->debug ? env->dump : nullptr, env->debug ? env->trace : nullptr));
    return VNL_OK;
  }
  if (env->spec)
    hipLaunchKernelGGL((vnl_reset_kernel<VnlSpecRodent>), dim3(env->B), dim3(64), env->lds_bytes, (hipStream_t)stream,
                       (const KernelConsts*)env->kc, ds, (const int*)start_frame, (const vreal*)noise,
                       env->debug ? env->dump : nullptr, env->debug ? env->trace : nullptr);
  else
    hipLaunchKernelGGL((vnl_reset_kernel<VnlSpecGeneric>), dim3(env->B), dim3(64), env->lds_bytes, (hipStream_t)stream,
                       (const KernelConsts*)env->kc, ds, (const int*)start_frame, (const vreal*)noise,
                       env->debug ? env->dump : nullptr, env->debug ? env->trace : nullptr);
  HIPCHK(hipGetLastError());
  return VNL_OK;
}

extern "C" int vnl_env_fk(vnl_env* env, const float* qpos, const vnl_state* state, void* stream) {
  if (!env || !qpos || !state) return fail(VNL_ERR_ARG, "vnl_env_fk: null argument");
  DevState ds;
  int rc = to_dev_state(state, &ds);
  if (rc != VNL_OK) return rc;
  DeviceGuard guard(env->device);
  if (!guard.ok) return fail(VNL_ERR_HIP, "hipSetDevice failed");
  hipLaunchKernelGGL(vnl_fk_kernel, dim3(env->B), dim3(64), env->lds_bytes, (hipStream_t)stream, (const KernelConsts*)env->kc, ds,
                     (const vreal*)qpos);
  HIPCHK(hipGetLastError());
  return VNL_OK;
}

extern "C" int vnl_env_step(vnl_env* env, const float* action, const vnl_state* state, void* stream) {
  if (!env || !action || !state) return fail(VNL_ERR_ARG, "vnl_env_step: null argument");
  DevState ds;
  int rc = to_dev_state(state, &ds);
  if (rc != VNL_OK) return rc;
  DeviceGuard guard(env->device);
  if (!guard.ok) return fail(VNL_ERR_HIP, "hipSetDevice failed");
  if (env->has_dom) {
    HIPCHK((hipError_t)vnl_domain_step_(env->kc, env->spec, env->B, env->lds_bytes, stream, ds, (const vreal*)action,
                                        env->debug == 1 ? env->dump : nullptr, env->debug == 2 ? env->dump : nullptr,
                                        env->debug ? env->trace : nullptr));
    return VNL_OK;
  }
  if (env->spec)
    hipLaunchKernelGGL((vnl_step_kernel<VnlSpecRodent>), dim3(env->B), dim3(64), env->lds_bytes, (hipStream_t)stream,
                       (const KernelConsts*)env->kc, ds, (const vreal*)action, env->debug == 1 ? env->dump : nullptr,
                       env->debug == 2 ? env->dump : nullptr, env->debug ? env->trace : nullptr);
  else
    hipLaunchKernelGGL((vnl_step_kernel<VnlSpecGeneric>), dim3(env->B), dim3(64), env->lds_bytes, (hipStream_t)stream,
                       (const KernelConsts*)env->kc, ds, (const vreal*)action, env->debug == 1 ? env->dump : nullptr,
                       env->debug == 2 ? env->dump : nullptr, env->debug ? env->trace : nullptr);
  HIPCHK(hipGetLastError());
  return VNL_OK;
}


static std::vector<vreal> four_field_tables(const vnl_env* env, const std::vector<double> v[4]) {
  const DevModel& d = env->dm;
  std::vector<vreal> tab;
  tab.reserve((size_t)env->B * (2 * d.ncg + d.nu + 2 * d.nv));
  for (double x : v[0]) tab.push_back((vreal)x);
  for (size_t k = 0; k < v[0].size(); k++) tab.push_back((vreal)contact_invweight(env->cg_t[k % d.ncg], v[0][k], env->impratio));
  for (int f = 1; f < 4; f++)
    for (double x : v[f]) tab.push_back((vreal)x);
  return tab;
}
static std::vector<vreal> four_field_compiled(const vnl_env* env) {
  const std::vector<double>* model[4] = {&env->mu0, &env->gain0, &env->damp0, &env->arm0};
  std::vector<double> v[4];
  for (int f = 0; f < 4; f++)
    for (int e = 0; e < env->B; e++) v[f].insert(v[f].end(), model[f]->begin(), model[f]->end());
  return four_field_tables(env, v);
}

static const char* body_row(const vnl_env* env, const double* mass, const double* inertia, const double* ipos, std::vector<double>* out,
                            char* why, size_t nwhy) {
  const int nb = env->fmap->nb_out, nd = env->dm.nbody;
  std::vector<double> full;
  if (inertia) {
    full = env->ifull0;
    for (int b = 1; b < nb; b++) {
      double dl[3], R[9];
      for (int k = 0; k < 3; k++) dl[k] = inertia[3 * (size_t)b + k] - env->inertia0[3 * (size_t)b + k];
      if (dl[0] == 0 && dl[1] == 0 && dl[2] == 0) continue;
      qmat_d(&env->iquat0[4 * (size_t)b], R);
      for (int r = 0; r < 3; r++)
        for (int q = 0; q < 3; q++) {
          double v = 0;
          for (int a = 0; a < 3; a++) v += R[3 * r + a] * dl[a] * R[3 * q + a];
          full[9 * (size_t)b + 3 * r + q] += v;
        }
    }
  }
  std::vector<double> M, nip, nI;
  fuse_inertial(*env->fmap, nd, mass ? mass : env->mass0.data(), ipos ? ipos : env->ipos0.data(),
                inertia ? full.data() : env->ifull0.data(), &M, &nip, &nI);
  double tm = 0;
  for (int b = 0; b < nd; b++) {
    tm += M[b];
    if (!why || b == 0 || env->dyn_dofnum[b] <= 0) continue;
    if (!(M[b] > 0)) {
      snprintf(why, nwhy, "dynamic body %d (body %d as given, with what is welded to it) carries dofs and has mass %g", b, env->fmap->body_out[b], M[b]);
      return "body_mass";
    }
    for (int k = 0; k < 3; k++)
      if (!(nI[9 * (size_t)b + 4 * k] > 0)) {
        snprintf(why, nwhy, "dynamic body %d (body %d as given) carries dofs and has inertia diagonal %g", b, env->fmap->body_out[b], nI[9 * (size_t)b + 4 * k]);
        return "body_inertia";
      }
  }
  if (why && !(tm > 0)) {
    snprintf(why, nwhy, "total mass %g", tm);
    return "body_mass";
  }
  const std::vector<double> i6 = pack_inertia6(nI);
  out->clear();
  out->insert(out->end(), M.begin(), M.end()), out->insert(out->end(), nip.begin(), nip.end());
  out->insert(out->end(), i6.begin(), i6.end()), out->push_back(total_mass_inv_of(M));
  return nullptr;
}
static std::vector<vreal> body_tables(const vnl_env* env, const std::vector<std::vector<double>>& rows) {
  const size_t B = (size_t)env->B, nd = (size_t)env->dm.nbody;
  std::vector<vreal> tab(B * (10 * nd + 1));
  const size_t off[4] = {0, B * nd, 4 * B * nd, 10 * B * nd}, w[4] = {nd, 3 * nd, 6 * nd, 1}, at[4] = {0, nd, 4 * nd, 10 * nd};
  for (size_t e = 0; e < B; e++) {
    const std::vector<double>& r = rows[rows.size() == 1 ? 0 : e];
    for (int t = 0; t < 4; t++)
      for (size_t k = 0; k < w[t]; k++) tab[off[t] + e * w[t] + k] = (vreal)r[at[t] + k];
  }
  return tab;
}
static std::vector<vreal> body_compiled(const vnl_env* env) {
  std::vector<std::vector<double>> rows(1);
  (void)body_row(env, nullptr, nullptr, nullptr, &rows[0], nullptr, 0);
  return body_tables(env, rows);
}

static int domain_tables(vnl_env* env) {
  if (env->dom) return VNL_OK;
  const DevModel& d = env->dm;
  const size_t B = (size_t)env->B, n4 = B * (2 * d.ncg + d.nu + 2 * d.nv), nd = (size_t)d.nbody;
  std::vector<vreal> tab = four_field_compiled(env);
  const std::vector<vreal> body = body_compiled(env);
  tab.insert(tab.end(), body.begin(), body.end());
  void* p = nullptr;
  HIPCHK(hipMalloc(&p, tab.size() * sizeof(vreal)));
  env->allocs.push_back(p);
  HIPCHK(hipMemcpy(p, tab.data(), tab.size() * sizeof(vreal), hipMemcpyHostToDevice));
  env->dom = (vreal*)p;
  DevDomain dd;
  dd.cg_mu = env->dom, dd.cg_invweight = env->dom + B * d.ncg, dd.act_gain = env->dom + 2 * B * d.ncg;
  dd.dof_damping = dd.act_gain + B * d.nu, dd.dof_armature = dd.dof_damping + B * d.nv;
  dd.body_mass = env->dom + n4, dd.body_ipos = dd.body_mass + B * nd, dd.body_inertia6 = dd.body_mass + 4 * B * nd;
  dd.total_mass_inv = dd.body_mass + 10 * B * nd;
  HIPCHK(hipMemcpy((char*)env->kc + offsetof(KernelConsts, dom), &dd, sizeof(DevDomain), hipMemcpyHostToDevice));
  return VNL_OK;
}

extern "C" int vnl_env_set_domain(vnl_env* env, const vnl_domain* dom, void* stream) {
  if (!env) return fail(VNL_ERR_ARG, "vnl_env_set_domain: null env");
  DeviceGuard guard(env->device);
  if (!guard.ok) return fail(VNL_ERR_HIP, "hipSetDevice failed");
#ifndef VNL_FORKJOIN_DEFINED
  HIPCHK(hipStreamSynchronize((hipStream_t)stream));
#else
  (void)stream;
#endif
  const DevModel& d = env->dm;
  const size_t B = (size_t)env->B;
  if (!dom) {
    if (env->dom) {
      const std::vector<vreal> tab = four_field_compiled(env);
      if (!tab.empty()) HIPCHK(hipMemcpy(env->dom, tab.data(), tab.size() * sizeof(vreal), hipMemcpyHostToDevice));
    }
    env->has_dom4 = 0, env->has_dom = env->has_body;
    return VNL_OK;
  }
  struct Field {
    const char* name;
    const double* src;
    const std::vector<double>& model;
    int n;
    int rule;
  } fields[] = {{"cg_friction", dom->cg_friction, env->mu0, d.ncg, 0}, {"act_gain", dom->act_gain, env->gain0, d.nu, 2},
                {"dof_damping", dom->dof_damping, env->damp0, d.nv, 1}, {"dof_armature", dom->dof_armature, env->arm0, d.nv, 1}};
  std::vector<double> v[4];
  for (int f = 0; f < 4; f++) {
    const Field& F = fields[f];
    v[f].resize(B * F.n);
    if (F.src) {
      if (F.n > 0) HIPCHK(hipMemcpy(v[f].data(), F.src, v[f].size() * sizeof(double), hipMemcpyDeviceToHost));
    } else {
      for (size_t e = 0; e < B; e++) std::copy(F.model.begin(), F.model.end(), v[f].begin() + e * F.n);
    }
    for (size_t k = 0; k < v[f].size(); k++) {
      const double x = v[f][k];
      const bool ok = std::isfinite(x) && (F.rule == 2 || (F.rule == 1 ? x >= 0 : x > 0));
      if (!ok) {
        char where[96];
        snprintf(where, sizeof(where), "env %zu, index %zu (%g)", k / F.n, k % F.n, x);
        return fail(VNL_ERR_ARG, F.rule == 0 ? "vnl_env_set_domain: %s must be finite and > 0: %s"
                                 : F.rule == 1 ? "vnl_env_set_domain: %s must be finite and >= 0: %s"
                                               : "vnl_env_set_domain: %s must be finite: %s",
                    F.name, where);
      }
    }
  }
  const std::vector<vreal> tab = four_field_tables(env, v);
  int rc = domain_tables(env);
  if (rc != VNL_OK) return rc;
  if (!tab.empty()) HIPCHK(hipMemcpy(env->dom, tab.data(), tab.size() * sizeof(vreal), hipMemcpyHostToDevice));
  env->has_dom4 = 1, env->has_dom = 1;
  return VNL_OK;
}

extern "C" int vnl_env_set_body_domain(vnl_env* env, const vnl_body_domain* bd, void* stream) {
  if (!env) return fail(VNL_ERR_ARG, "vnl_env_set_body_domain: null env");
  DeviceGuard guard(env->device);
  if (!guard.ok) return fail(VNL_ERR_HIP, "hipSetDevice failed");
#ifndef VNL_FORKJOIN_DEFINED
  HIPCHK(hipStreamSynchronize((hipStream_t)stream));
#else
  (void)stream;
#endif
  const DevModel& d = env->dm;
  const size_t B = (size_t)env->B, nb = (size_t)d.nbody_out, n4 = B * (2 * d.ncg + d.nu + 2 * d.nv);
  if (!bd) {
    if (env->dom) {
      const std::vector<vreal> tab = body_compiled(env);
      HIPCHK(hipMemcpy(env->dom + n4, tab.data(), tab.size() * sizeof(vreal), hipMemcpyHostToDevice));
    }
    env->has_body = 0, env->has_dom = env->has_dom4;
    return VNL_OK;
  }
  if (bd->body_inertia && env->inertia0.empty())
    return fail(VNL_ERR_BLOB, "vnl_env_set_body_domain: body_inertia needs the model's body_inertia and body_iquat sections");
  struct Field {
    const char* name;
    const double* src;
    const std::vector<double>& model;
    size_t w;
    bool nonneg;
  } fields[] = {{"body_mass", bd->body_mass, env->mass0, 1, true}, {"body_inertia", bd->body_inertia, env->inertia0, 3, true},
                {"body_ipos", bd->body_ipos, env->ipos0, 3, false}};
  std::vector<double> v[3];
  for (int f = 0; f < 3; f++) {
    const Field& F = fields[f];
    if (!F.src) continue;
    const size_t n = nb * F.w;
    v[f].resize(B * n);
    HIPCHK(hipMemcpy(v[f].data(), F.src, v[f].size() * sizeof(double), hipMemcpyDeviceToHost));
    for (size_t e = 0; e < B; e++) std::copy(F.model.begin(), F.model.begin() + F.w, v[f].begin() + e * n);
    for (size_t k = 0; k < v[f].size(); k++) {
      const double x = v[f][k];
      if (!(std::isfinite(x) && (!F.nonneg || x >= 0))) {
        char where[96];
        snprintf(where, sizeof(where), "env %zu, index %zu (%g)", k / n, k % n, x);
        return fail(VNL_ERR_ARG, F.nonneg ? "vnl_env_set_body_domain: %s must be finite and >= 0: %s"
                                          : "vnl_env_set_body_domain: %s must be finite: %s", F.name, where);
      }
    }
  }
  std::vector<std::vector<double>> rows(B);
  for (size_t e = 0; e < B; e++) {
    char why[160], where[200];
    const char* bad = body_row(env, v[0].empty() ? nullptr : &v[0][e * nb], v[1].empty() ? nullptr : &v[1][e * 3 * nb],
                               v[2].empty() ? nullptr : &v[2][e * 3 * nb], &rows[e], why, sizeof(why));
    if (bad) {
      snprintf(where, sizeof(where), "env %zu: %s", e, why);
      return fail(VNL_ERR_ARG, "vnl_env_set_body_domain: %s: %s", bad, where);
    }
  }
  const std::vector<vreal> tab = body_tables(env, rows);
  int rc = domain_tables(env);
  if (rc != VNL_OK) return rc;
  HIPCHK(hipMemcpy(env->dom + n4, tab.data(), tab.size() * sizeof(vreal), hipMemcpyHostToDevice));
  env->has_body = 1, env->has_dom = 1;
  return VNL_OK;
}

#ifdef VNL_PROFILE
extern "C" int vnl_prof_read(unsigned long long* out) {
  unsigned long long z[VNL_NPROF] = {0};
  HIPCHK(hipMemcpyFromSymbol(out, HIP_SYMBOL(g_vnl_prof), sizeof(z)));
  HIPCHK(hipMemcpyToSymbol(HIP_SYMBOL(g_vnl_prof), z, sizeof(z)));
  return VNL_OK;
}
#endif

#ifndef VNL_POST_THREADS
#define VNL_POST_THREADS 256
#endif
__global__ void __launch_bounds__(VNL_POST_THREADS) vnl_post_kernel(vnl_post_desc d) {
  const unsigned e = blockIdx.x, tid = threadIdx.x;
  float st = d.steps ? ((d.prev_done && d.prev_done[e] != 0.f) ? 0.f : d.steps[e]) + (float)d.action_repeat : 0.f;
  float done = d.done[e];
  bool over = d.steps && st >= (float)d.episode_length;
  float trunc = over ? 1.f - done : 0.f;
  done = over ? 1.f : done;
  __syncthreads();
  if (tid == 0) {
    if (d.steps) d.steps[e] = st;
    if (d.prev_done) d.prev_done[e] = done;
    d.done[e] = done;
    if (d.truncation) d.truncation[e] = trunc;
    if (d.log_reward) d.log_reward[e] = d.reward[e];
    if (d.log_discount) d.log_discount[e] = 1.f - done;
    if (d.log_truncation) d.log_truncation[e] = trunc;
  }
  const bool reset = done != 0.f;
  for (int k = 0; k < d.num_ops; k++) {
    const vnl_post_op& op = d.ops[k];
    const bool from_first = op.first && reset;
    const unsigned* src = (const unsigned*)(from_first ? op.first : op.src) + (size_t)e * op.width;
    unsigned* dst = op.dst ? (unsigned*)op.dst + (size_t)e * op.width : nullptr;
    unsigned* log = op.log ? (unsigned*)op.log + (size_t)e * op.width : nullptr;
    const bool store = dst && (from_first || (const float*)op.dst != op.src);
    for (int i = (int)tid; i < op.width; i += VNL_POST_THREADS) {
      unsigned v = src[i];
      if (store) dst[i] = v;
      if (log) log[i] = v;
    }
  }
}

extern "C" int vnl_rollout_post(const vnl_post_desc* desc, int32_t num_envs, void* stream) {
  if (!desc || num_envs <= 0 || !desc->done) return fail(VNL_ERR_ARG, "vnl_rollout_post: null argument");
  if (desc->num_ops < 0 || desc->num_ops > VNL_POST_MAX_OPS) return fail(VNL_ERR_ARG, "vnl_rollout_post: too many ops");
  for (int k = 0; k < desc->num_ops; k++)
    if (!desc->ops[k].src || desc->ops[k].width <= 0) return fail(VNL_ERR_ARG, "vnl_rollout_post: bad op");
  if ((desc->log_reward && !desc->reward)) return fail(VNL_ERR_ARG, "vnl_rollout_post: log_reward without reward");
  hipLaunchKernelGGL(vnl_post_kernel, dim3(num_envs), dim3(VNL_POST_THREADS), 0, (hipStream_t)stream, *desc);
  HIPCHK(hipGetLastError());
  return VNL_OK;
}

#ifndef VNL_HEAD_THREADS
#define VNL_HEAD_THREADS 256
#define VNL_HEAD_GROUP 32
#define VNL_GROUP_SUM(v) \
  (v += __shfl_xor(v, 16, 32), v += __shfl_xor(v, 8, 32), v += __shfl_xor(v, 4, 32), v += __shfl_xor(v, 2, 32), v += __shfl_xor(v, 1, 32))
#endif
#define VNL_HEAD_MAXBLK 256
#ifndef VNL_FINISH_THREADS
#define VNL_FINISH_THREADS 64
#define VNL_FINISH_SUM(v) \
  (v += __shfl_xor(v, 32), v += __shfl_xor(v, 16), v += __shfl_xor(v, 8), v += __shfl_xor(v, 4), v += __shfl_xor(v, 2), v += __shfl_xor(v, 1))
#endif
__device__ __forceinline__ float vnl_block_sum(float v, float* red) {
  const unsigned tid = threadIdx.x;
  __syncthreads();
  red[tid] = v;
  __syncthreads();
  for (unsigned w = VNL_HEAD_THREADS / 2; w > 0; w >>= 1) {
    if (tid < w) red[tid] += red[tid + w];
    __syncthreads();
  }
  return red[0];
}
__device__ __forceinline__ float vnl_softplus(float x) { return x > 20.f ? x : log1pf(expf(x)); }

__global__ void __launch_bounds__(VNL_HEAD_THREADS) vnl_ppo_gae_kernel(vnl_ppo_head_args a, float* stats) {
#if VNL_HEAD_THREADS > 1
  __shared__ float red[VNL_HEAD_THREADS];
#else
  float red[1];
#endif
  const int tid = (int)threadIdx.x, T = a.T, B = a.B, N = T * B;
  float sa = 0.f, sr = 0.f;
  for (int b = tid; b < B; b += VNL_HEAD_THREADS) {
    float acc = 0.f, v_next = a.bootstrap[b], vs_next = a.bootstrap[b];
    for (int t1 = T; t1 > 0; t1 -= 8) {
      const int t0 = t1 > 8 ? t1 - 8 : 0;
      float tr[8], dc[8], rw[8], bl[8];
#pragma unroll
      for (int k = 0; k < 8; k++) {
        const int t = t1 - 1 - k, n = (t >= t0 ? t : t0) * B + b;
        tr[k] = a.truncation[n], dc[k] = a.discount[n], rw[k] = a.reward[n], bl[k] = a.baseline[n];
      }
#pragma unroll
      for (int k = 0; k < 8; k++) {
        const int t = t1 - 1 - k;
        if (t >= t0) {
          const int n = t * B + b;
          const float trunc = tr[k], mask = 1.f - trunc;
          const float term = (1.f - dc[k]) * (1.f - trunc);
          const float r = rw[k] * a.reward_scaling, v = bl[k];
          const float delta = (r + a.discounting * (1.f - term) * v_next - v) * mask;
          acc = delta + a.discounting * (1.f - term) * mask * a.gae_lambda * acc;
          const float vs = acc + v;
          const float adv = (r + a.discounting * (1.f - term) * vs_next - v) * mask;
          a.vs[n] = vs, a.advantages[n] = adv;
          sa += adv, sr += r;
          v_next = v, vs_next = vs;
        }
      }
    }
  }
  const float adv_mean = vnl_block_sum(sa, red) / (float)N, r_mean = vnl_block_sum(sr, red) / (float)N;
  float qa = 0.f, qr = 0.f;
  __syncthreads();
  const float inv_n = 1.f / (float)N;
  for (int n = tid; n < N; n += VNL_HEAD_THREADS) {
    const float da = a.advantages[n] - adv_mean, dr = a.reward[n] * a.reward_scaling - r_mean;
    qa += da * da, qr += dr * dr;
    a.g_baseline[n] = -0.5f * (a.vs[n] - a.baseline[n]) * inv_n;
  }
  const float va = vnl_block_sum(qa, red) / (float)N, vr = vnl_block_sum(qr, red) / (float)N;
  if (tid == 0) stats[0] = adv_mean, stats[1] = sqrtf(va), stats[2] = vr;
}

__global__ void __launch_bounds__(VNL_HEAD_THREADS) vnl_ppo_head_kernel(vnl_ppo_head_args a, float* stats) {
#if VNL_HEAD_THREADS > 1
  __shared__ float red[VNL_HEAD_THREADS];
#else
  float red[1];
#endif
#if defined(__HIP_DEVICE_COMPILE__)
  __builtin_amdgcn_s_setprio(3);
#endif
  const int tid = (int)threadIdx.x, A = a.act, N = a.T * a.B;
  const int lane = tid % VNL_HEAD_GROUP, group = (int)(blockIdx.x * (VNL_HEAD_THREADS / VNL_HEAD_GROUP)) + tid / VNL_HEAD_GROUP;
  const int ngroups = (int)gridDim.x * (VNL_HEAD_THREADS / VNL_HEAD_GROUP);
  const float adv_mean = stats[0], adv_std = stats[1];
  const float inv_n = 1.f / (float)N, half_log_2pi = 0.91893853320467274178f, ln2 = 0.69314718055994530942f;
  const float lo = 1.f - a.clipping_epsilon, hi = 1.f + a.clipping_epsilon;
  float s_pl = 0.f, s_vl = 0.f, s_ent = 0.f;
  for (int n = group; n < N; n += ngroups) {
    const float* lg = a.logits + (size_t)n * 2 * A;
    const float* ra = a.raw_action + (size_t)n * A;
    const float* ee = a.eps_entropy + (size_t)n * A;
    float tlp = 0.f, ent = 0.f;
    for (int k = lane; k < A; k += VNL_HEAD_GROUP) {
      const float loc = lg[k], scale = (vnl_softplus(lg[A + k]) + a.min_std) * a.var_scale;
      const float x = ra[k], z = (x - loc) / scale, lsc = logf(scale);
      tlp += (-0.5f * z * z - half_log_2pi - lsc) - 2.f * (ln2 - x - vnl_softplus(-2.f * x));
      const float xe = loc + scale * ee[k];
      ent += (0.5f + half_log_2pi + lsc) + 2.f * (ln2 - xe - vnl_softplus(-2.f * xe));
    }
    VNL_GROUP_SUM(tlp);
    VNL_GROUP_SUM(ent);
    float adv = a.advantages[n];
    if (a.normalize_advantage) adv = (adv - adv_mean) / (adv_std + 1e-8f);
    const float rho = expf(tlp - a.behaviour_log_prob[n]);
    const float rc = fminf(fmaxf(rho, lo), hi);
    const float s1 = rho * adv, s2 = rc * adv;
    const float dmin = (s1 < s2 || (s1 == s2 && rho >= lo && rho <= hi)) ? adv : ((s1 == s2) ? 0.5f * adv : 0.f);
    const float g_tlp = -inv_n * dmin * rho;
    const float g_ent = -a.entropy_cost * inv_n;
    const float verr = a.vs[n] - a.baseline[n];
    if (lane == 0) s_pl += -fminf(s1, s2), s_vl += verr * verr, s_ent += ent;
    float* gl = a.g_logits + (size_t)n * 2 * A;
    for (int k = lane; k < A; k += VNL_HEAD_GROUP) {
      const float sraw = lg[A + k], scale = (vnl_softplus(sraw) + a.min_std) * a.var_scale;
      const float loc = lg[k], z = (ra[k] - loc) / scale, xe = loc + scale * ee[k], th = tanhf(xe);
      const float dscale_ds = a.var_scale / (1.f + expf(-sraw));
      gl[k] = g_tlp * (z / scale) + g_ent * (-2.f * th);
      gl[A + k] = (g_tlp * ((z * z - 1.f) / scale) + g_ent * (1.f / scale - 2.f * th * ee[k])) * dscale_ds;
    }
  }
  float s_kl = 0.f;
  const int NL = N * a.latent;
  const float kscale = a.kl_weight / (float)NL;
  for (int i = (int)(blockIdx.x * VNL_HEAD_THREADS) + tid; i < NL; i += (int)gridDim.x * VNL_HEAD_THREADS) {
    const float mu = a.lat_mean[i], lv = a.lat_logvar[i], ev = expf(lv);
    s_kl += 1.f + lv - mu * mu - ev;
    a.g_lat_mean[i] = kscale * mu;
    a.g_lat_logvar[i] = -0.5f * kscale * (1.f - ev);
  }
  const float p0 = vnl_block_sum(s_pl, red), p1 = vnl_block_sum(s_vl, red), p2 = vnl_block_sum(s_ent, red),
              p3 = vnl_block_sum(s_kl, red);
  if (tid == 0) {
    float* part = stats + 4 + 4 * blockIdx.x;
    part[0] = p0, part[1] = p1, part[2] = p2, part[3] = p3;
  }
}

__global__ void vnl_ppo_finish_kernel(vnl_ppo_head_args a, const float* stats, int nblk) {
#if defined(__HIP_DEVICE_COMPILE__)
  __builtin_amdgcn_s_setprio(3);
#endif
  const int lane = (int)threadIdx.x;
  float s[4] = {0.f, 0.f, 0.f, 0.f};
  for (int b = lane; b < nblk; b += VNL_FINISH_THREADS)
// ... 106 lines not shown
```

### vnl-brax-imitation_amd/csrc/vnl_types.h

```cpp
#pragma once
#include <stdint.h>

#ifndef VNL_REAL
#define VNL_REAL float
#endif
typedef VNL_REAL vreal;

#define VNL_JNT_FREE 0
#define VNL_JNT_HINGE 3
#define VNL_GEOM_SPHERE 2
#define VNL_GEOM_CAPSULE 3
#define VNL_GEOM_ELLIPSOID 4

#define VNL_TRACE_ITERS 8
#define VNL_TRACE_REC 64
#define VNL_TRACE_ROWS (8 + VNL_TRACE_REC * VNL_TRACE_ITERS)
#define VNL_TRACE_INTS (VNL_TRACE_ROWS + 16)

#define VNL_LIVE_MAX 128
#define VNL_BLK_W 13
#define VNL_FAC_LINES 6

#define VNL_ROUTE_LDS 1
#define VNL_ROUTE_ROWS16 2
#define VNL_ROUTE_ROWS36 3
#define VNL_ROUTE_ROWS36X2 4
#define VNL_ROUTE_QM_FACTOR 0
#define VNL_ROUTE_QM_INVERSE 4
#define VNL_ROUTE_HESSIAN 8
#define VNL_ROUTE_PAIR 12

struct DevModel {
  int nq, nv, nu, nbody, njnt, ncg, ncon, nlimit, nefc, nM;
  int iterations, ls_iterations, eulerdamp, root_free, max_depth, jump_rounds;
  int solver_newton;
  int fac_steps;
  int fac_route;
  int nbody_out;
  int path_runs;
  int blk_cfg;
  int dbg_stage, dbg_count;
  vreal dt, tolerance, ls_tolerance, scale ;
  vreal gx, gy, gz;
  vreal pnx, pny, pnz, ppx, ppy, ppz;
  vreal t1x, t1y, t1z;
  vreal total_mass_inv;
  vreal root_px, root_py, root_pz;
  const int *body_parent, *body_jntadr, *body_jntnum, *body_dofadr, *body_dofnum, *body_nsub, *body_lastdof;
  const int *body_pathseg;
  const unsigned char* jump;
  const vreal *body_pos, *body_quat, *body_ipos, *body_inertia6, *body_mass;
  const int *out_dyn, *body_out;
  const vreal *out_pos, *out_quat;
  const int *jnt_type, *jnt_qposadr, *jnt_dofadr, *jnt_body;
  const vreal *jnt_pos, *jnt_axis, *jnt_qpos0, *jnt_stiffness, *jnt_springref;
  const int *lim_qadr, *lim_dof;
  const vreal *lim_lo, *lim_hi, *lim_margin, *lim_invweight, *lim_solref, *lim_solimp;
  const int *dof_body, *dof_Madr, *dof_depth, *dof_limrow;
  const int *M_anc, *M_row;
  const int *dof_ftime, *dof_fslot;
  const int* fac_guest;
  const unsigned* blk_tab;
  const unsigned char* fac_match;
  const int *dof_ndesc;
  const unsigned char* lvl_tab;
  const vreal *dof_armature, *dof_damping;
  const int *act_dof, *act_limited;
  const int* dof_act;
  const vreal *act_gain, *act_tau, *act_lo, *act_hi, *act_gear;
  const int *cg_type, *cg_body, *cg_conadr, *cg_ncon, *con_geom;
  const vreal *cg_pos, *cg_quat, *cg_size, *cg_mu, *cg_solref, *cg_solimp, *cg_margin, *cg_invweight;
};

struct DevEnv {
  int T, C, ref_len, sub_clip_length, n_frames, nb, nee, napp, njc, com_ref_col;
  int obs_size, traj_size;
  int flags;
  vreal healthy_lo, healthy_hi, inv_term_threshold, body_err_mult, done_threshold;
  vreal w_reward[6];
  const int *body_idxs, *end_eff_idx, *app_body, *app_ref_col, *joint_cols;
  const float *position, *quaternion, *joints, *body_positions, *velocity, *angular_velocity, *joints_velocity;
  const float* center_of_mass;
  vreal* fac2;
};

struct DevState {
  vreal *qpos, *qvel, *act, *warm, *xpos, *xquat, *com1, *qfrc_actuator;
  vreal *obs, *reward, *done, *metrics, *traj, *term_err;
  int *cur_frame, *sub_clip_frame, *clip_id;
};

struct WsLayout {
  int qpos, qvel, act, ctrl, actdot, com;
  int cdof, LD, dinv;
  int P;
  int efc_D, Jaref, jv;
  int smooth, qacc_smooth, qacc, Ma, grad, Mgrad, search, mv, qfrc_c, tmp, tmp2;
  int prof;
  int con_r, con_t1;
  int tab_anc, tab_madr, tab_body, tab_jump, tab_lvl;
  int act_list;
  int newt_M, newt_H;
  int total;
};

struct VnlDims {
  int nq, nv, nu, nbody, njnt, ncg, ncon, nlimit, nefc, nM;
  int iterations, ls_iterations, eulerdamp, root_free, max_depth, jump_rounds, fac_steps, fac_route, solver_newton, blk_cfg, path_runs, nbody_out;
};

#ifndef VNL_NPROF_SLOTS
#ifdef VNL_PROFILE
#define VNL_NPROF_SLOTS (2 * (40 + 1))
#else
#define VNL_NPROF_SLOTS 0
#endif
#endif
constexpr int vnl_imax(int a, int b) { return a > b ? a : b; }
constexpr int vnl_words(long bytes) { return (int)((bytes + (long)sizeof(vreal) - 1) / (long)sizeof(vreal)); }
constexpr WsLayout vnl_make_layout(const VnlDims& d) {
  WsLayout L{};
  int o = 0;
  auto sec = [&o](int n) {
    int at = o;
    o += n;
    return at;
  };
  L.qpos = sec(d.nq), L.qvel = sec(d.nv), L.act = sec(d.nu), L.ctrl = sec(d.nu);
  L.actdot = sec(d.nu), L.com = sec(4);
  L.cdof = sec(6 * d.nv);
  L.LD = sec(vnl_imax(d.nM, 6 * (d.nv + 1) + 6 * (d.nbody + 1)));
  L.dinv = sec(d.nv);
  int pool = vnl_imax(vnl_imax(14 * d.nbody, 22 * d.nbody), 3 * d.nefc + vnl_imax(6 * (d.ncon + 1), 6 * (d.nv + 1)));
  if (d.eulerdamp) pool = vnl_imax(pool, d.nM + d.nv);
  L.P = sec(pool);
  L.efc_D = L.P, L.Jaref = L.P + d.nefc, L.jv = L.P + 2 * d.nefc;
  L.smooth = sec(d.nv), L.qacc_smooth = sec(d.nv), L.qacc = sec(d.nv);
  L.Ma = sec(d.nv), L.grad = sec(d.nv), L.Mgrad = sec(d.nv), L.search = sec(d.nv);
  L.mv = sec(d.nv), L.qfrc_c = sec(d.nv), L.tmp = sec(d.nv), L.tmp2 = sec(d.nv);
  L.con_r = sec(3 * d.ncon), L.con_t1 = sec(3 * d.ncg);
  L.tab_anc = sec(vnl_words(d.nM)), L.tab_madr = sec(vnl_words(6 * (long)d.nv));
  L.tab_body = sec(vnl_words(3 * (long)d.nbody + 2 * (long)d.ncon));
  L.tab_jump = sec(vnl_words((long)(d.jump_rounds > 0 ? d.jump_rounds : 1) * d.nbody));
  L.tab_lvl = sec(vnl_words((long)d.nv + d.max_depth + 2));
  L.act_list = sec(vnl_words(4 * (long)((d.ncon + 3) / 4) + 8 + 2 * VNL_LIVE_MAX));
  L.newt_M = L.newt_H = 0;
  if (d.solver_newton) L.newt_M = sec(d.nM), L.newt_H = sec(d.nM + d.nv);
  if (VNL_NPROF_SLOTS) {
    o = (o + 1) & ~1;
    L.prof = sec(VNL_NPROF_SLOTS);
  }
  L.total = (o + 3) & ~3;
  return L;
}

constexpr int vnl_vstore(int P) { return (P + 3) & ~3; }
constexpr int vnl_cvel_at(int P, int smooth, int nbody, int nv) {
  const int a = P + 16 * nbody, b = vnl_vstore(P) + 12 * nv;
  return (b > a && b + 6 * nbody <= smooth) ? b : a;
}

struct VnlSpecGeneric {
  static constexpr bool fixed = false;
  static constexpr bool dom = false;
  static constexpr VnlDims D{};
  static constexpr WsLayout L{};
};
struct VnlSpecRodent {
  static constexpr bool fixed = true;
  static constexpr bool dom = false;
  static constexpr VnlDims D{74, 73, 30, 53, 68, 32, 59, 67, 303, 1119, 6, 6, 1, 1, 35, 5, 36,
                             VNL_ROUTE_ROWS36X2 | (VNL_ROUTE_ROWS36X2 << VNL_ROUTE_QM_INVERSE) | (2 << VNL_ROUTE_PAIR), 0,
                             2 | (2 << 4) | (2 << 8) | (3 << 12), 2, 66};
  static constexpr WsLayout L = vnl_make_layout(D);
};
template <class BASE>
struct VnlSpecDom : BASE {
  static constexpr bool dom = true;
};

struct DevDomain {
  const vreal *cg_mu, *cg_invweight;
  const vreal *act_gain;
  const vreal *dof_damping, *dof_armature;
  const vreal *body_mass, *body_ipos, *body_inertia6;
  const vreal *total_mass_inv;
};

struct KernelConsts {
  DevModel m;
  DevEnv ev;
  WsLayout L;
  DevDomain dom;
};
```

### vnl-brax-imitation_amd/envs/rodent.py

```python
from __future__ import annotations

import ctypes as C
import os
from typing import Any, Dict, List, Mapping, Optional, Sequence

import numpy as np
import torch

from .. import _lib
from ..model import blob as _blob
from ..model import mjcf as _mjcf
from .base import Env, PipelineState, State

_PKG = os.path.dirname(os.path.dirname(os.path.abspath(__file__)))
_TEST_BACKEND = None
_METRICS = ("rcom", "rvel", "rtrunk", "rquat", "ract", "rapp", "termination_error")
DOMAIN_FIELDS = {"cg_friction": ("ngeom_collide", 0.0, False), "act_gain": ("nu", None, False),
                 "dof_damping": ("nv", 0.0, True), "dof_armature": ("nv", 0.0, True)}
BODY_DOMAIN_FIELDS = {"body_mass": ((), 0.0), "body_inertia": ((3,), 0.0), "body_ipos": ((3,), None)}


def packaged_model_path(name: str = "rodent", scale_factor: Optional[float] = 0.9) -> str:
    if scale_factor is None:
        return os.path.join(_PKG, "data", f"{name}.npz")
# ... 177 lines not shown
                raise ValueError(f"domain field {k!r} must have shape {shape}, got {tuple(t.shape)}")
            if not bool(torch.isfinite(t).all()):
                raise ValueError(f"domain field {k!r} has non-finite values")
            if lo is not None and not bool(((t >= lo) if closed else (t > lo)).all()):
                raise ValueError(f"domain field {k!r} must be {'>=' if closed else '>'} {lo}")
            tables[k] = t.to(self.device).contiguous()
        return self._with_domains(tables, self._body_domain)

    def with_body_domain(self, bodies: Mapping[str, Any]) -> "RodentTracking":
        nbody = int(self.dims.nbody)
        tables = {}
        for k, v in dict(bodies).items():
            if k not in BODY_DOMAIN_FIELDS:
                raise ValueError(f"unknown body domain field {k!r}: expected some of {sorted(BODY_DOMAIN_FIELDS)}")
            tail, lo = BODY_DOMAIN_FIELDS[k]
            t = torch.as_tensor(v).detach().to(dtype=torch.float64)
            shape = (self.num_envs, nbody) + tail
            if tuple(t.shape) != shape:
                raise ValueError(f"body domain field {k!r} must have shape {shape}, got {tuple(t.shape)}")
            if not bool(torch.isfinite(t).all()):
                raise ValueError(f"body domain field {k!r} has non-finite values")
            if lo is not None and not bool((t[:, 1:] >= lo).all()):
                raise ValueError(f"body domain field {k!r} must be >= {lo}")
            tables[k] = t.to(self.device).contiguous()
        return self._with_domains(self._domain, tables)

    @property
    def domain(self) -> Optional[Dict[str, torch.Tensor]]:
        if self._domain is None and self._body_domain is None:
            return None
        return dict(self._domain or {}, **(self._body_domain or {}))

    def domain_table(self, name: str) -> torch.Tensor:
        ptr, cnt = C.c_void_p(), C.c_int32()
        _lib.check(self._L, self._L.vnl_env_scratch(self._env_h, name.encode(), C.byref(ptr), C.byref(cnt)))
        total = self.num_envs * cnt.value
        if self.device.type == "cuda":
            torch.cuda.synchronize(self.device)
            flat = torch.empty(total, dtype=self._dtype, device=self.device)
            esz = flat.element_size()
            rc = C.CDLL("libamdhip64.so").hipMemcpy(C.c_void_p(flat.data_ptr()), ptr, C.c_size_t(esz * total), C.c_int(3))
            if rc != 0:
                raise _lib.VnlError(f"hipMemcpy failed: {rc}")
            flat = flat.cpu()
        else:
            ct = C.c_double if self._dtype == torch.float64 else C.c_float
            flat = torch.from_numpy(np.ctypeslib.as_array(C.cast(ptr, C.POINTER(ct)), shape=(total,)).copy())
        return flat.view(self.num_envs, cnt.value)

    def __del__(self):
        try:
            if getattr(self, "_env_h", None):
                self._L.vnl_env_destroy(self._env_h)
            if getattr(self, "_model_h", None):
                self._L.vnl_model_destroy(self._model_h)
        except Exception:
            pass

    @property
    def observation_size(self) -> int:
        return int(self.dims.obs_size)

    @property
    def traj_size(self) -> int:
        return int(self.dims.traj_size)

    @property
    def action_size(self) -> int:
        return int(self.dims.nu)

    @property
    def dt(self) -> float:
        return float(self.sys.scalars["timestep"]) * self._n_frames

    def env_spec(self) -> Dict[str, Any]:
        return dict(
            T=self._T, ref_len=self._ref_traj_length, sub_clip_length=self._sub_clip_length, n_frames=self._n_frames,
            nb=len(self._body_idxs), nee=len(self._end_eff_idx), napp=len(self._app_idx), njc=len(self._joint_cols),
            com_ref_col=self._com_ref_col, body_idxs=self._body_idxs.tolist(), end_eff_idx=self._end_eff_idx.tolist(),
            app_body=self._app_idx.tolist(), app_ref_col=self._app_ref_col.tolist(),
            joint_cols=self._joint_cols.tolist(), healthy_z_lo=self._healthy_z_range[0],
            healthy_z_hi=self._healthy_z_range[1], termination_threshold=self._termination_threshold,
            body_error_multiplier=self._body_error_multiplier, flags=int(self._env_flags),
            done_threshold=float(self._done_threshold),
            reward_weights=list(self._reward_weights) if self._reward_weights else None,
        )

    def clip_arrays(self, clip: int = 0) -> Dict[str, np.ndarray]:
        return {k: v[clip] for k, v in self._clip.items()}

    def _stream(self):
        if self.device.type == "cuda":
            return C.c_void_p(torch.cuda.current_stream(self.device).cuda_stream)
        return C.c_void_p(0)

    def _alloc_state(self) -> State:
        B, dv, d = self.num_envs, self.device, self.dims
        ps = PipelineState.allocate(d, B, dv, self._dtype)
        z = lambda n, dt=self._dtype: torch.zeros((B, n) if n else (B,), dtype=dt, device=dv)
        raw = dict(obs=z(d.obs_size), reward=z(0), done=z(0), metrics=z(7), traj=z(d.traj_size),
                   termination_error=z(0), cur_frame=z(0, torch.int32), sub_clip_frame=z(0, torch.int32),
                   clip_id=z(0, torch.int32))
        metrics = {k: raw["metrics"][:, i] for i, k in enumerate(_METRICS)}
        info = dict(cur_frame=raw["cur_frame"], sub_clip_frame=raw["sub_clip_frame"], traj=raw["traj"],
                    termination_error=raw["termination_error"], clip_id=raw["clip_id"], _raw=raw)
        return State(ps, raw["obs"], raw["reward"], raw["done"], metrics, info)

    def _ptrs(self, state: State) -> _lib.StatePtrs:
        raw, ps = state.info["_raw"], state.pipeline_state
        p = _lib.StatePtrs()
        for k in PipelineState._FIELDS:
            setattr(p, k, ps.raw(k).data_ptr())
        for k in ("obs", "reward", "done", "metrics", "traj", "termination_error", "cur_frame", "sub_clip_frame",
                  "clip_id"):
            setattr(p, k, raw[k].data_ptr())
        return p

    def reset(self, rng=None, *, start_frame: Optional[torch.Tensor] = None, noise: Optional[torch.Tensor] = None,
              clip_id: Optional[torch.Tensor] = None, out: Optional[State] = None) -> State:
        B, nq = self.num_envs, int(self.dims.nq)
        gen = self._gen
        if isinstance(rng, torch.Generator):
            gen = rng
        elif rng is not None:
            gen = torch.Generator(device="cpu")
            gen.manual_seed(int(rng))
        if start_frame is None:
            hi = self._clip_length - self._sub_clip_length - self._ref_traj_length
            start_frame = torch.randint(0, max(hi, 1), (B,), generator=gen, dtype=torch.int32)
        if noise is None:
            noise = self._reset_noise_scale * torch.randn((B, nq), generator=gen, dtype=torch.float32)
        if clip_id is None:
            clip_id = (torch.zeros(B, dtype=torch.int32) if self._num_clips == 1 else
                       torch.randint(0, self._num_clips, (B,), generator=gen, dtype=torch.int32))
        state = out if out is not None else self._alloc_state()
        sf = torch.as_tensor(start_frame, dtype=torch.int32).to(self.device).contiguous()
        nz = torch.as_tensor(noise).to(device=self.device, dtype=self._dtype).contiguous()
        state.info["_raw"]["clip_id"].copy_(torch.as_tensor(clip_id, dtype=torch.int32).to(self.device))
        p = self._ptrs(state)
        _lib.check(self._L, self._L.vnl_env_reset(self._env_h, sf.data_ptr(), nz.data_ptr(), C.byref(p),
                                                  self._stream()))
        self._hold = (sf, nz)
        return state

    def step(self, state: State, action: torch.Tensor) -> State:
        nu, B = int(self.dims.nu), self.num_envs
        if tuple(action.shape) != (B, nu):
            raise ValueError(f"action must be ({B},{nu}), got {tuple(action.shape)}")
        a = action.to(device=self.device, dtype=self._dtype).contiguous()
        p = self._ptrs(state)
        ev = getattr(self, "kernel_events", None)
        if ev is not None:
            ev[0].record()
        _lib.check(self._L, self._L.vnl_env_step(self._env_h, a.data_ptr(), C.byref(p), self._stream()))
        if ev is not None:
            ev[1].record()
        self._hold = (a,)
        return state

    def forward_kinematics(self, qpos: torch.Tensor, out: Optional[State] = None) -> State:
        B, nq = self.num_envs, int(self.dims.nq)
        if tuple(qpos.shape) != (B, nq):
            raise ValueError(f"qpos must be ({B},{nq}), got {tuple(qpos.shape)}")
        state = out if out is not None else self._alloc_state()
        q = qpos.to(device=self.device, dtype=self._dtype).contiguous()
        state.pipeline_state.qpos.copy_(q)
        p = self._ptrs(state)
        _lib.check(self._L, self._L.vnl_env_fk(self._env_h, q.data_ptr(), C.byref(p), self._stream()))
        self._hold = (q,)
        return state

    def debug(self, mode=True) -> None:
        stride = C.c_int32()
        _lib.check(self._L, self._L.vnl_env_debug(self._env_h, int(mode), C.byref(stride)))
        self._dump_stride = stride.value

    def solver_trace(self) -> torch.Tensor:
        ptr, cnt = C.c_void_p(), C.c_int32()
        _lib.check(self._L, self._L.vnl_env_scratch(self._env_h, b"solver_trace", C.byref(ptr), C.byref(cnt)))
        B, n = self.num_envs, cnt.value
        if self.device.type == "cuda":
            torch.cuda.synchronize(self.device)
            flat = torch.empty(B * n, dtype=torch.int32, device=self.device)
            rc = C.CDLL("libamdhip64.so").hipMemcpy(C.c_void_p(flat.data_ptr()), ptr, C.c_size_t(4 * B * n), C.c_int(3))
            if rc != 0:
                raise _lib.VnlError(f"hipMemcpy failed: {rc}")
            flat = flat.cpu()
        else:
            flat = torch.from_numpy(np.ctypeslib.as_array(C.cast(ptr, C.POINTER(C.c_int32)), shape=(B * n,)).copy())
        return flat.view(B, max(self._n_frames, 1), -1)

    def scratch(self, name: str) -> torch.Tensor:
        ptr, cnt = C.c_void_p(), C.c_int32()
        _lib.check(self._L, self._L.vnl_env_scratch(self._env_h, name.encode(), C.byref(ptr), C.byref(cnt)))
        B, n, stride = self.num_envs, cnt.value, self._dump_stride
        esz = 8 if self._dtype == torch.float64 else 4
        total = (B - 1) * stride + n
        if self.device.type == "cuda":
            torch.cuda.synchronize(self.device)
            flat = torch.empty(total, dtype=self._dtype, device=self.device)
            hip = C.CDLL("libamdhip64.so")
            rc = hip.hipMemcpy(C.c_void_p(flat.data_ptr()), ptr, C.c_size_t(esz * total), C.c_int(3))
            if rc != 0:
                raise _lib.VnlError(f"hipMemcpy failed: {rc}")
        else:
            ct = C.c_double if self._dtype == torch.float64 else C.c_float
            flat = torch.from_numpy(np.ctypeslib.as_array(C.cast(ptr, C.POINTER(ct)), shape=(total,)).copy())
        return torch.as_strided(flat, (B, n), (stride, 1)).contiguous()


class RodentMultiClipTracking(RodentTracking):
    """Multi-clip variant.  The reference only has a stub (rodent.py:473-475); here the clip
    container carries a leading clip axis and each env tracks `info['clip_id']`."""
```

### vnl-brax-imitation_amd/ppo_imitation/acting.py

```python
from __future__ import annotations

import dataclasses
import time
from typing import Any, Callable, Dict, Optional, Sequence, Tuple

import numpy as np
import torch

from ..envs.base import State
from ..envs.wrappers import EvalWrapper


@dataclasses.dataclass
class Transition:

    observation: torch.Tensor
    action: torch.Tensor
    reward: torch.Tensor
    discount: torch.Tensor
    next_observation: torch.Tensor
    extras: Dict[str, Dict[str, torch.Tensor]]

    def map(self, fn: Callable[[torch.Tensor], torch.Tensor]) -> "Transition":
        return Transition(fn(self.observation), fn(self.action), fn(self.reward), fn(self.discount),
                          fn(self.next_observation),
                          {k: {kk: fn(vv) for kk, vv in v.items()} for k, v in self.extras.items()})


def actor_step(env, env_state: State, policy, key, extra_fields: Sequence[str] = ()) -> Tuple[State, Transition]:
    obs = env_state.obs.clone()
    traj = env_state.info["traj"]
    actions, policy_extras = policy(traj, obs, key)
    nstate = env.step(env_state, actions)
    state_extras = {x: nstate.info[x] for x in extra_fields}
    return nstate, Transition(observation=obs, action=actions, reward=nstate.reward, discount=1 - nstate.done,
                              next_observation=nstate.obs,
                              extras={"policy_extras": policy_extras, "state_extras": state_extras})


def _fusable(env):
    from ..envs import wrappers as W

    if not isinstance(env, W.AutoResetWrapper) or not isinstance(env.env, W.EpisodeWrapper):
        return None
    ep, base = env.env, env.env.env
    if ep.action_repeat != 1 or base is not base.unwrapped or not hasattr(getattr(base, "_L", None), "vnl_rollout_post"):
        return None
    return env, ep, base


def _device_noise(policy) -> bool:
    return getattr(policy, "noise", None) == "device"


_DIRECT_LOG = True


def _generate_unroll_fused(fz, env_state: State, policy, key, unroll_length: int, extra_fields) -> Tuple[State, Transition]:
    import ctypes as C

    from .. import _lib

    ar, ep, base = fz
    st = env_state
    T, info, dev = unroll_length, env_state.info, env_state.obs.device
    B = st.obs.shape[0]
    new = lambda *shape, like: torch.empty((T, *shape), dtype=like.dtype, device=dev)
    obs0, nobs_log = st.obs.clone(), new(*st.obs.shape, like=st.obs)
    rew_log, disc_log = new(B, like=st.reward), new(B, like=st.reward)
    sx_log = {x: new(*info[x].shape, like=info[x]) for x in extra_fields}
    prev_done = st.done.clone()
    stream = C.c_void_p(torch.cuda.current_stream(dev).cuda_stream) if dev.type == "cuda" else C.c_void_p(0)
    ptr = lambda t: C.c_void_p(t.data_ptr()) if t is not None else C.c_void_p(0)
    width = lambda t: 1 if t.dim() == 1 else t.shape[1]

    d = _lib.PostDesc()
    d.steps, d.prev_done, d.done, d.truncation, d.reward = (ptr(info["steps"]), ptr(prev_done), ptr(st.done),
                                                            ptr(info["truncation"]), ptr(st.reward))
    d.episode_length, d.action_repeat = ep.episode_length, 1
    ops = []
    fps = info["first_pipeline_state"]
    for name in st.pipeline_state._FIELDS:
        cur = st.pipeline_state.raw(name)
        ops.append((cur, cur, fps.raw(name), None))
    ops.append((st.obs, st.obs, info["first_obs"], nobs_log))
    logged = set()
    if ar.reset_info:
        for k2, v in info["first_info"].items():
            ops.append((info[k2], info[k2], v, sx_log.get(k2)))
            logged.add(k2)
    for x in extra_fields:
        if x not in logged and x != "truncation":
            ops.append((None, info[x], None, sx_log[x]))
    n_static = len(ops)
    px_log: Optional[dict] = None
    act_log = None
    dev_noise = _device_noise(policy)
    direct = dev_noise and _DIRECT_LOG
    if direct:
        na = base.action_size
        f32 = lambda *shape: torch.empty((T, *shape), dtype=torch.float32, device=dev)
        act_log = f32(B, na)
        px_log = {} if policy.deterministic else {"log_prob": f32(B), "rand_log_prob": f32(B), "raw_action": f32(B, na),
                                                  "logits": f32(B, 2 * na)}
    for t in range(T):
        if direct:
            actions, pex = policy(info["traj"], st.obs, None, step_offset=t, advance=False,
                                  out={"action": act_log[t], **{k2: v[t] for k2, v in px_log.items()}})
        elif dev_noise:
            actions, pex = policy(info["traj"], st.obs, None, step_offset=t, advance=False)
        else:
            actions, pex = policy(info["traj"], st.obs, key)
        base.step(st, actions)
        if px_log is None:
            act_log = new(*actions.shape, like=actions)
            px_log = {k2: new(*v.shape, like=v) for k2, v in pex.items()}
        step_ops = ops[:n_static] if direct else ops[:n_static] + [(None, actions.contiguous(), None, act_log)] + \
            [(None, v.contiguous(), None, px_log[k2]) for k2, v in pex.items()]
        assert len(step_ops) <= _lib.POST_MAX_OPS
        d.num_ops = len(step_ops)
        keep = []
        for i, (dst, src, first, log) in enumerate(step_ops):
            assert src.dtype in (torch.float32, torch.int32) and src.is_contiguous()
            o = d.ops[i]
            o.dst, o.src, o.first, o.width = ptr(dst), ptr(src), ptr(first), width(src)
            o.log = ptr(log[t]) if log is not None else C.c_void_p(0)
            keep.append(src)
        d.log_reward, d.log_discount = ptr(rew_log[t]), ptr(disc_log[t])
        d.log_truncation = ptr(sx_log["truncation"][t]) if "truncation" in sx_log else C.c_void_p(0)
        _lib.check(base._L, base._L.vnl_rollout_post(C.byref(d), B, stream))
        _generate_unroll_fused.hold = keep
    if dev_noise:
        policy.counter.add_(T)
    obs_log = torch.cat((obs0[None], nobs_log[:-1]), dim=0)
    data = Transition(observation=obs_log, action=act_log, reward=rew_log, discount=disc_log, next_observation=nobs_log,
                      extras={"policy_extras": px_log, "state_extras": sx_log})
    return st, data


class GraphedUnroll:

    def __init__(self, env, env_state: State, policy, key: torch.Generator, unroll_length: int,
                 extra_fields: Sequence[str] = ()):
        fz = _fusable(env)
        dev = env_state.obs.device
        if fz is None or dev.type != "cuda":
            raise ValueError("GraphedUnroll needs AutoResetWrapper(EpisodeWrapper(<env on a HIP device>)), action_repeat 1")
        dev_noise = _device_noise(policy)
        if not dev_noise and (key is None or key.device.type != "cuda"):
            raise ValueError("GraphedUnroll needs a torch.Generator on the device (its stream is captured with the graph)")
        self._args = (fz, env_state, policy, key, int(unroll_length), tuple(extra_fields))
        self.state = env_state
        gen_state = policy.counter.clone() if dev_noise else key.get_state()
        saved = _snapshot_state(env_state)
        side = torch.cuda.Stream(dev)
        side.wait_stream(torch.cuda.current_stream(dev))
        with torch.cuda.stream(side):
            _generate_unroll_fused(*self._args)
        torch.cuda.current_stream(dev).wait_stream(side)
        torch.cuda.synchronize(dev)
        _restore_state(env_state, saved)
        self.graph = torch.cuda.CUDAGraph()
        if dev_noise:
            policy.counter.copy_(gen_state)
        else:
            key.set_state(gen_state)
            self.graph.register_generator_state(key)
        with torch.cuda.graph(self.graph):
            _, self.data = _generate_unroll_fused(*self._args)
        self._hold = getattr(_generate_unroll_fused, "hold", None)
        _restore_state(env_state, saved)

    def __call__(self) -> Tuple[State, Transition]:
        self.graph.replay()
        return self.state, self.data


def _state_tensors(st: State):
    out = [st.pipeline_state.raw(n) for n in st.pipeline_state._FIELDS] + [st.obs, st.reward, st.done]
    for k in sorted(st.info):
        v = st.info[k]
        if isinstance(v, torch.Tensor):
            out.append(v)
        elif isinstance(v, dict):
            out += [v[k2] for k2 in sorted(v) if isinstance(v[k2], torch.Tensor)]
    seen, uniq = set(), []
    for t in out:
        if t.data_ptr() not in seen:
            seen.add(t.data_ptr())
            uniq.append(t)
    return uniq


def _snapshot_state(st: State):
    return [t.clone() for t in _state_tensors(st)]


def _restore_state(st: State, saved) -> None:
    for t, s in zip(_state_tensors(st), saved):
        t.copy_(s)


def generate_unroll(env, env_state: State, policy, key, unroll_length: int,
                    extra_fields: Sequence[str] = (), fused: Optional[bool] = None) -> Tuple[State, Transition]:
    fz = _fusable(env) if fused is not False else None
    if fused is True and fz is None:
        raise ValueError("fused rollout needs AutoResetWrapper(EpisodeWrapper(RodentTracking)), action_repeat 1")
    if fz is not None:
        return _generate_unroll_fused(fz, env_state, policy, key, unroll_length, tuple(extra_fields))
    data: Optional[Transition] = None
    for t in range(unroll_length):
        env_state, tr = actor_step(env, env_state, policy, key, extra_fields=extra_fields)
        if data is None:
            alloc = lambda x: torch.empty((unroll_length, *x.shape), dtype=x.dtype, device=x.device)
            data = tr.map(alloc)
        for dst, src in zip(_leaves(data), _leaves(tr)):
            dst[t].copy_(src)
    return env_state, data


def _leaves(tr: Transition):
    out = [tr.observation, tr.action, tr.reward, tr.discount, tr.next_observation]
    for g in sorted(tr.extras):
        out += [tr.extras[g][k] for k in sorted(tr.extras[g])]
    return out


class Evaluator:

    def __init__(self, eval_env, eval_policy_fn, num_eval_envs: int, episode_length: int, action_repeat: int,
                 key: Optional[torch.Generator]):
        self._key = key
        self._eval_walltime = 0.0
        self._env = EvalWrapper(eval_env)
        self._policy_fn = eval_policy_fn
        self._unroll = episode_length // action_repeat
        self._steps_per_unroll = episode_length * num_eval_envs

    def run_evaluation(self, policy_params, training_metrics: Dict[str, Any], aggregate_episodes: bool = True):
        t = time.time()
        state = self._env.reset(self._key)
        state, _ = generate_unroll(self._env, state, self._policy_fn(policy_params), self._key, self._unroll)
        em = state.info["eval_metrics"]
        if em.active_episodes.is_cuda:
            torch.cuda.synchronize(em.active_episodes.device)
        epoch_eval_time = time.time() - t
        metrics = {}
        for fn in (np.mean, np.std):
            suffix = "_std" if fn is np.std else ""
            metrics.update({f"eval/episode_{name}{suffix}": (fn(v.cpu().numpy()) if aggregate_episodes else v.cpu().numpy())
                            for name, v in em.episode_metrics.items()})
        metrics["eval/avg_episode_length"] = float(np.mean(em.episode_steps.cpu().numpy()))
        metrics["eval/epoch_eval_time"] = epoch_eval_time
        metrics["eval/sps"] = self._steps_per_unroll / epoch_eval_time
        self._eval_walltime += epoch_eval_time
        return {"eval/walltime": self._eval_walltime, **training_metrics, **metrics}
```

Before: 2.525 million env-steps/s.

## Fuse rollout post-processing into step kernel epilogue; add factor handoff variant

New measurement: 2.518 million env-steps/s. Within noise of the previous version (-0.3%).

```diff
diff --git a/__graft_entry__.py b/__graft_entry__.py
--- a/__graft_entry__.py
+++ b/__graft_entry__.py
@@ -14,8 +14,8 @@
 
     from concurrent.futures import ThreadPoolExecutor
 
-    with ThreadPoolExecutor(5) as pool:
-        futs = {v: pool.submit(hip_build.build, variant=v) for v in ("product", "spill", "noblk", "nospec", "tail")}
+    with ThreadPoolExecutor(6) as pool:
+        futs = {v: pool.submit(hip_build.build, variant=v) for v in ("product", "spill", "noblk", "nospec", "tail", "handoff")}
         paths = {v: f.result() for v, f in futs.items()}
     path = paths["product"]
     assert all(os.path.exists(p_) for p_ in paths.values()), paths
diff --git a/include/vnl.h b/include/vnl.h
--- a/include/vnl.h
+++ b/include/vnl.h
@@ -113,6 +113,9 @@
 } vnl_body_domain;
 int vnl_env_set_body_domain(vnl_env* env, const vnl_body_domain* domain, void* stream);
 
+int vnl_factor_schedule(const int32_t* dof_parent, int32_t nv, int32_t* ftime, int32_t* fslot, uint8_t* hand, uint16_t* plan,
+                        int32_t* steps);
+
 int vnl_env_debug(vnl_env*, int32_t enable, int32_t* row_stride);
 int vnl_env_scratch(const vnl_env*, const char* name, float** dev_ptr, int32_t* count);
 
@@ -162,6 +165,7 @@
   vnl_post_op ops[VNL_POST_MAX_OPS];
 } vnl_post_desc;
 int vnl_rollout_post(const vnl_post_desc*, int32_t num_envs, void* stream);
+int vnl_env_step_post(vnl_env*, const float* action, const vnl_state*, const vnl_post_desc*, void* stream);
 
 typedef struct vnl_ppo_head_args {
   int32_t T, B, act, latent;
diff --git a/vnl-brax-imitation_amd/_lib.py b/vnl-brax-imitation_amd/_lib.py
--- a/vnl-brax-imitation_amd/_lib.py
+++ b/vnl-brax-imitation_amd/_lib.py
@@ -149,13 +149,13 @@
 
 EXPORTS = (
     "vnl_last_error", "vnl_version", "vnl_model_create", "vnl_model_destroy", "vnl_env_create", "vnl_env_destroy",
-    "vnl_env_dims", "vnl_env_reset", "vnl_env_step", "vnl_env_fk", "vnl_env_debug", "vnl_env_scratch", "vnl_policy_create", "vnl_policy_destroy",
+    "vnl_env_dims", "vnl_env_reset", "vnl_env_step", "vnl_env_step_post", "vnl_env_fk", "vnl_env_debug", "vnl_env_scratch", "vnl_policy_create", "vnl_policy_destroy",
     "vnl_policy_num_params", "vnl_policy_forward", "vnl_policy_forward_noise", "vnl_rollout_post", "vnl_ppo_head", "vnl_adam_step", "vnl_gather_rows",
     "vnl_ppo_update_create", "vnl_ppo_update_destroy", "vnl_ppo_update_num_params", "vnl_ppo_update_buffer",
     "vnl_ppo_minibatch_grad",
     "vnl_ppo_minibatch_grad_part",
     "vnl_env_set_domain", "vnl_env_set_body_domain",
-    "vnl_prediction_corr_plan", "vnl_prediction_corr",
+    "vnl_prediction_corr_plan", "vnl_prediction_corr", "vnl_factor_schedule",
 )
 _HIP_ONLY = ("vnl_policy_", "vnl_ppo_update_", "vnl_ppo_minibatch_", "vnl_prediction_corr")
 
@@ -177,11 +177,13 @@
     lib.vnl_env_dims.argtypes = [vp, C.POINTER(Dims)]
     lib.vnl_env_reset.argtypes = [vp, vp, vp, C.POINTER(StatePtrs), vp]
     lib.vnl_env_step.argtypes = [vp, vp, C.POINTER(StatePtrs), vp]
+    lib.vnl_env_step_post.argtypes = [vp, vp, C.POINTER(StatePtrs), C.POINTER(PostDesc), vp]
     lib.vnl_env_fk.argtypes = [vp, vp, C.POINTER(StatePtrs), vp]
     lib.vnl_env_debug.argtypes = [vp, C.c_int32, C.POINTER(C.c_int32)]
     lib.vnl_env_scratch.argtypes = [vp, C.c_char_p, C.POINTER(vp), C.POINTER(C.c_int32)]
     lib.vnl_env_set_domain.argtypes = [vp, C.POINTER(Domain), vp]
     lib.vnl_env_set_body_domain.argtypes = [vp, C.POINTER(BodyDomain), vp]
+    lib.vnl_factor_schedule.argtypes = [vp, C.c_int32, vp, vp, vp, vp, C.POINTER(C.c_int32)]
     lib.vnl_rollout_post.argtypes = [C.POINTER(PostDesc), C.c_int32, vp]
     lib.vnl_ppo_head.argtypes = [C.POINTER(PPOHeadArgs), vp, vp]
     lib.vnl_gather_rows.argtypes = [C.POINTER(GatherDesc), vp]
diff --git a/vnl-brax-imitation_amd/csrc/build.py b/vnl-brax-imitation_amd/csrc/build.py
--- a/vnl-brax-imitation_amd/csrc/build.py
+++ b/vnl-brax-imitation_amd/csrc/build.py
@@ -16,6 +16,7 @@
     "spill": ("libvnl_spill.so", ["-DVNL_KERNEL_ATTR=__attribute__((amdgpu_waves_per_eu(4,4)))"]),
     "noblk": ("libvnl_noblk.so", ["-DVNL_NO_BLK", "-DVNL_KERNEL_ATTR=__attribute__((amdgpu_waves_per_eu(2,2)))"]),
     "tail": ("libvnl_tail.so", ["-DVNL_SOLVER_TAIL", "-DVNL_KERNEL_ATTR=__attribute__((amdgpu_waves_per_eu(2,2)))"]),
+    "handoff": ("libvnl_handoff.so", ["-DVNL_FACTOR_HANDOFF", "-DVNL_KERNEL_ATTR=__attribute__((amdgpu_waves_per_eu(2,2)))"]),
     "nospec": ("libvnl_nospec.so", ["-DVNL_NO_SPEC", "-DVNL_KERNEL_ATTR=__attribute__((amdgpu_waves_per_eu(2,2)))"]),
 }
 ENV_KERNELS = ("vnl_step_kernel", "vnl_reset_kernel")
diff --git a/vnl-brax-imitation_amd/csrc/vnl_body.h b/vnl-brax-imitation_amd/csrc/vnl_body.h
--- a/vnl-brax-imitation_amd/csrc/vnl_body.h
+++ b/vnl-brax-imitation_amd/csrc/vnl_body.h
@@ -82,6 +82,8 @@
   return x;
 }
 #define VNL_SEG_SUM(part, dsc, steps) (part = vnl_seg_sum(part, (dsc) >> 28, steps))
+VNL_HD int vnl_next_lane(int x) { return __builtin_amdgcn_update_dpp(0, x, 0x101, 0xf, 0xf, true); }
+VNL_HD float vnl_next_lane(float x) { return __builtin_bit_cast(float, vnl_next_lane(__builtin_bit_cast(int, x))); }
 #define VNL_WAVE_FENCE() __builtin_amdgcn_fence(__ATOMIC_ACQ_REL, "wavefront")
 #define VNL_LINE_HEADERS(out, base, stride)                                                       \
   do {                                                                                            \
@@ -840,6 +842,165 @@
     }
   }
 
+#ifdef VNL_FACTOR_HANDOFF
+  template <int NSET>
+  VNL_HD void factor_aba(vreal h) const {
+    constexpr int LW = 16;
+    const int sc = (LO(Mgrad) + 3) & ~3;
+    const int half = vnl_fac_handoff_room(MI(nv)) ? VNL_FAC_LINES * LW : 0;
+    const int VS = vstore();
+    vreal* g2 = fac2();
+    const int nsteps = MI(fac_steps);
+    v2r U[NSET][6], diag[NSET], ivs[NSET];
+    vreal S[NSET][6];
+    int dep[NSET], ftime[NSET], myline[NSET], adrs[NSET];
+    const unsigned short* mt[NSET];
+    unsigned nxt[NSET];
+    auto hset = [](int q) constexpr { return VNL_LANES == 1 || q == 0; };
+#pragma unroll
+    for (int q = 0; q < NSET; q++) {
+      const int a = (int)lane + q * VNL_LANES;
+      const bool ok = a < MI(nv);
+      const int aa = ok ? a : 0;
+      const S6 c = ld6(LO(cdof) + 6 * aa), f = inert_mul(LO(P) + 10 * m.dof_body[aa], c);
+      S[q][0] = c.a.x, S[q][1] = c.a.y, S[q][2] = c.a.z, S[q][3] = c.l.x, S[q][4] = c.l.y, S[q][5] = c.l.z;
+      U[q][0] = v2r{f.a.x, f.a.x}, U[q][1] = v2r{f.a.y, f.a.y}, U[q][2] = v2r{f.a.z, f.a.z};
+      U[q][3] = v2r{f.l.x, f.l.x}, U[q][4] = v2r{f.l.y, f.l.y}, U[q][5] = v2r{f.l.z, f.l.z};
+      const vreal arm = par<P_ARM>(aa);
+      diag[q] = v2r{arm, arm + h * par<P_DAMP>(aa)};
+      ivs[q] = v2r{vreal(0.), vreal(0.)};
+      adrs[q] = madr(aa), dep[q] = eadr(aa) - adrs[q];
+      myline[q] = m.dof_fslot[aa];
+      ftime[q] = ok ? m.dof_ftime[aa] : -1;
+      mt[q] = m.fac_plan + (size_t)aa * nsteps;
+      nxt[q] = (ok && nsteps > 0) ? mt[q][0] : 0u;
+    }
+    VNL_SYNC();
+    VNL_PROF(7);
+    auto absorb = [&](int q, const v2r* Uk, v2r ivk, int kend) {
+      v2r pa = v2r{S[q][0], S[q][0]} * Uk[0], pb = v2r{S[q][1], S[q][1]} * Uk[1];
+      pa += v2r{S[q][2], S[q][2]} * Uk[2], pb += v2r{S[q][3], S[q][3]} * Uk[3];
+      pa += v2r{S[q][4], S[q][4]} * Uk[4], pb += v2r{S[q][5], S[q][5]} * Uk[5];
+      const v2r Lk = (pa + pb) * ivk;
+#pragma unroll
+      for (int i = 0; i < 6; i++) U[q][i] -= Lk * Uk[i];
+      s[LO(LD) + kend - dep[q]] = Lk[0];
+    };
+    auto absorb_line = [&](int q, const R4& u0, const R4& u1, const R4& u2, const R4& hd) {
+      const v2r Uk[6] = {v2r{u0.x, u0.y}, v2r{u0.z, u0.w}, v2r{u1.x, u1.y}, v2r{u1.z, u1.w}, v2r{u2.x, u2.y}, v2r{u2.z, u2.w}};
+      absorb(q, Uk, v2r{hd.x, hd.y}, (int)hd.z);
+    };
+    auto absorb_next = [&](int q, bool take) {
+      v2r Uk[6], ivk;
+      int kend;
+#if VNL_LANES > 1
+#pragma unroll
+      for (int i = 0; i < 6; i++) Uk[i] = v2r{vnl_next_lane(U[q][i][0]), vnl_next_lane(U[q][i][1])};
+      ivk = v2r{vnl_next_lane(ivs[q][0]), vnl_next_lane(ivs[q][1])};
+      kend = vnl_next_lane(adrs[q] + dep[q]);
+#else
+      const int n = q + 1 < NSET ? q + 1 : q;
+#pragma unroll
+      for (int i = 0; i < 6; i++) Uk[i] = U[n][i];
+      ivk = ivs[n], kend = adrs[n] + dep[n];
+#endif
+      if (take) absorb(q, Uk, ivk, kend);
+    };
+    for (int step = 0; step < nsteps; step++) {
+      const int now = sc + (step & 1) * half, was = sc + ((step & 1) ^ 1) * half;
+      unsigned cur[NSET], late[NSET];
+      R4 pre[NSET][4];
+#pragma unroll
+      for (int q = 0; q < NSET; q++) {
+        cur[q] = nxt[q];
+        nxt[q] = (ftime[q] >= 0 && step + 1 < nsteps) ? mt[q][step + 1] : 0u;
+        late[q] = (cur[q] >> 6) & 63u;
+        if (hset(q)) {
+          const vreal* ln = s + was + (late[q] ? __builtin_ctz(late[q]) : 0) * LW;
+          pre[q][0] = ld4a(ln), pre[q][1] = ld4a(ln + 4), pre[q][2] = ld4a(ln + 8), pre[q][3] = ld4a(ln + 12);
+        }
+      }
+#pragma unroll
+      for (int q = 0; q < NSET; q++) {
+        if (ftime[q] == step) {
+          const int a = (int)lane + q * VNL_LANES;
+          v2r D = diag[q];
+#pragma unroll
+          for (int i = 0; i < 6; i++) D += v2r{S[q][i], S[q][i]} * U[q][i];
+          const v2r iv = v2r{vnl_recip(D[0]), vnl_recip(D[1])};
+          ivs[q] = iv;
+          vreal* ln = s + now + myline[q] * LW;
+          st4a(ln, U[q][0][0], U[q][0][1], U[q][1][0], U[q][1][1]);
+          st4a(ln + 4, U[q][2][0], U[q][2][1], U[q][3][0], U[q][3][1]);
+          st4a(ln + 8, U[q][4][0], U[q][4][1], U[q][5][0], U[q][5][1]);
+          st4a(ln + 12, iv[0], iv[1], (vreal)(adrs[q] + dep[q]), vreal(0.));
+          vreal* vs = s + VS + 12 * a;
+          const v2r v0 = U[q][0] * iv, v1 = U[q][1] * iv, v2 = U[q][2] * iv, v3_ = U[q][3] * iv, v4 = U[q][4] * iv, v5 = U[q][5] * iv;
+          st4a(vs, v0[0], v0[1], v1[0], v1[1]);
+          st4a(vs + 4, v2[0], v2[1], v3_[0], v3_[1]);
+          st4a(vs + 8, v4[0], v4[1], v5[0], v5[1]);
+          s[LO(dinv) + a] = iv[0];
+          g2[MI(nM) + a] = iv[1];
+        }
+      }
+#pragma unroll
+      for (int q = 0; q < NSET; q++) {
+        if (hset(q)) {
+          const bool take = (cur[q] & 0x1000u) && late[q] == 0u;
+          if (vnl_wave_any(take)) absorb_next(q, take);
+        }
+      }
+#pragma unroll
+      for (int q = 0; q < NSET; q++) {
+        if (hset(q) && late[q] != 0u) {
+          late[q] &= late[q] - 1u;
+          absorb_line(q, pre[q][0], pre[q][1], pre[q][2], pre[q][3]);
+        }
+      }
+      for (int pass = 1; pass < VNL_FAC_LINES; pass++) {
+        bool more = false;
+#pragma unroll
+        for (int q = 0; q < NSET; q++) more = more || (hset(q) && late[q] != 0u);
+        if (!vnl_wave_any(more)) break;
+#pragma unroll
+        for (int q = 0; q < NSET; q++) {
+          if (hset(q) && late[q] != 0u) {
+            const vreal* ln = s + was + __builtin_ctz(late[q]) * LW;
+            late[q] &= late[q] - 1u;
+            absorb_line(q, ld4a(ln), ld4a(ln + 4), ld4a(ln + 8), ld4a(ln + 12));
+          }
+        }
+      }
+#pragma unroll
+      for (int q = 0; q < NSET; q++) {
+        if (hset(q)) {
+          const bool take = (cur[q] & 0x1000u) && (cur[q] & 0xfc0u) != 0u;
+          if (vnl_wave_any(take)) absorb_next(q, take);
+        }
+      }
+      VNL_WAVE_FENCE();
+      for (int pass = 0; pass < VNL_FAC_LINES; pass++) {
+        bool more = false;
+#pragma unroll
+        for (int q = 0; q < NSET; q++) more = more || (cur[q] & 63u) != 0u;
+        if (!vnl_wave_any(more)) break;
+#pragma unroll
+        for (int q = 0; q < NSET; q++) {
+          if ((cur[q] & 63u) != 0u) {
+            const int k = __builtin_ctz(cur[q]);
+            cur[q] &= cur[q] - 1u;
+            const vreal* ln = s + now + k * LW;
+            absorb_line(q, ld4a(ln), ld4a(ln + 4), ld4a(ln + 8), ld4a(ln + 12));
+          }
+        }
+      }
+      VNL_WAVE_FENCE();
+    }
+    VNL_SYNC();
+    VNL_PROF(8);
+    VNL_PROF(9);
+  }
+#else
   template <int NSET>
   VNL_HD void factor_aba(vreal h) const {
     constexpr int LW = 16;
@@ -927,6 +1088,7 @@
     VNL_PROF(8);
     VNL_PROF(9);
   }
+#endif
 
   VNL_HD int vstore() const { return vnl_vstore(LO(P)); }
   VNL_HD int cvel_at() const { return vnl_cvel_at(LO(P), LO(smooth), MI(nbody), MI(nv)); }
diff --git a/vnl-brax-imitation_amd/csrc/vnl_domain.hip b/vnl-brax-imitation_amd/csrc/vnl_domain.hip
--- a/vnl-brax-imitation_amd/csrc/vnl_domain.hip
+++ b/vnl-brax-imitation_amd/csrc/vnl_domain.hip
@@ -19,12 +19,12 @@
 }
 
 int vnl_domain_step_(const KernelConsts* kc, int spec, int B, size_t lds, void* stream, const DevState& ds, const vreal* action,
-                     vreal* dump, vreal* dump_mid, int* trace) {
+                     vreal* dump, vreal* dump_mid, int* trace, const vnl_post_desc& post) {
   if (spec)
     hipLaunchKernelGGL((vnl_step_kernel<VnlSpecDom<VnlSpecRodent>>), dim3(B), dim3(64), lds, (hipStream_t)stream, kc, ds,
-                       action, dump, dump_mid, trace);
+                       action, dump, dump_mid, trace, post);
   else
     hipLaunchKernelGGL((vnl_step_kernel<VnlSpecDom<VnlSpecGeneric>>), dim3(B), dim3(64), lds, (hipStream_t)stream, kc, ds,
-                       action, dump, dump_mid, trace);
+                       action, dump, dump_mid, trace, post);
   return (int)hipGetLastError();
 }
diff --git a/vnl-brax-imitation_amd/csrc/vnl_env_kernels.h b/vnl-brax-imitation_amd/csrc/vnl_env_kernels.h
--- a/vnl-brax-imitation_amd/csrc/vnl_env_kernels.h
+++ b/vnl-brax-imitation_amd/csrc/vnl_env_kernels.h
@@ -1,4 +1,7 @@
 #pragma once
+#include <stddef.h>
+
+#include "../../include/vnl.h"
 #include "vnl_body.h"
 
 #ifndef VNL_KERNEL_ATTR
@@ -6,14 +9,111 @@
 #endif
 #define VNL_ENV_KERNEL __launch_bounds__(64) VNL_KERNEL_ATTR
 
+#ifndef VNL_POST_THREADS
+#define VNL_POST_THREADS 256
+#endif
+template <int THREADS, class D>
+VNL_HD void vnl_post_env(const D& d, const unsigned e, const unsigned tid) {
+  float st = d.steps ? ((d.prev_done && d.prev_done[e] != 0.f) ? 0.f : d.steps[e]) + (float)d.action_repeat : 0.f;
+  float done = d.done[e];
+  bool over = d.steps && st >= (float)d.episode_length;
+  float trunc = over ? 1.f - done : 0.f;
+  done = over ? 1.f : done;
+  if (THREADS > VNL_LANES) __syncthreads();
+  else VNL_SYNC_GLOBAL();
+  if (tid == 0) {
+    if (d.steps) d.steps[e] = st;
+    if (d.prev_done) d.prev_done[e] = done;
+    d.done[e] = done;
+    if (d.truncation) d.truncation[e] = trunc;
+    if (d.log_reward) d.log_reward[e] = d.reward[e];
+    if (d.log_discount) d.log_discount[e] = 1.f - done;
+    if (d.log_truncation) d.log_truncation[e] = trunc;
+  }
+  const bool reset = done != 0.f;
+  struct Trip {
+    const unsigned* src;
+    unsigned *dst, *log;
+    int n;
+  };
+  int k = 0, i0 = 0;
+  auto next_trip = [&](Trip& t) {
+    for (; k < d.num_ops; k++, i0 = 0) {
+      const auto& op = d.ops[k];
+      const bool from_first = op.first && reset;
+      const bool store = op.dst && (from_first || (const float*)op.dst != op.src);
+      if (i0 >= op.width || !(store || op.log)) continue;
+      const size_t at = (size_t)e * op.width + i0;
+      t = Trip{(const unsigned*)(from_first ? op.first : op.src) + at, store ? (unsigned*)op.dst + at : nullptr,
+               op.log ? (unsigned*)op.log + at : nullptr, op.width - i0};
+      i0 += 4 * THREADS;
+      return true;
+    }
+    return false;
+  };
+  constexpr int DEPTH = 8;
+  for (;;) {
+    Trip t[DEPTH];
+    unsigned v[DEPTH][4];
+    int nt = 0;
+    while (nt < DEPTH && next_trip(t[nt])) nt++;
+    if (nt == 0) break;
+#pragma unroll
+    for (int j = 0; j < DEPTH; j++) {
+      if (j < nt) {
+#pragma unroll
+        for (int u = 0; u < 4; u++) {
+          const int i = (int)tid + u * THREADS;
+          if (i < t[j].n) v[j][u] = t[j].src[i];
+        }
+      }
+    }
+#pragma unroll
+    for (int j = 0; j < DEPTH; j++) {
+      if (j < nt) {
+#pragma unroll
+        for (int u = 0; u < 4; u++) {
+          const int i = (int)tid + u * THREADS;
+          if (i < t[j].n) {
+            if (t[j].dst) t[j].dst[i] = v[j][u];
+            if (t[j].log) t[j].log[i] = v[j][u];
+          }
+        }
+      }
+    }
+  }
+}
+
+struct VnlStepArgs {
+  const KernelConsts* kc;
+  DevState st;
+  const vreal* action;
+  vreal *dump, *dump_mid;
+  int* trace;
+  vnl_post_desc post;
+};
+#if defined(__HIP_DEVICE_COMPILE__)
+#define VNL_STEP_ARGS(a) const VNL_CAS VnlStepArgs* a = (const VNL_CAS VnlStepArgs*)__builtin_amdgcn_kernarg_segment_ptr()
+#define VNL_STEP_ARG(a, f) ((a)->f)
+#else
+#define VNL_STEP_ARGS(a) const int a = 0
+#define VNL_STEP_ARG(a, f) (f)
+#endif
+
 template <class SP>
 __global__ void VNL_ENV_KERNEL vnl_step_kernel(const KernelConsts* kc, DevState st, const vreal* action,
-                                                      vreal* dump, vreal* dump_mid, int* trace) {
+                                                      vreal* dump, vreal* dump_mid, int* trace, vnl_post_desc post) {
   VNL_LDS_DECL(lds);
   const VNL_CAS KernelConsts* k = VNL_TO_CAS(KernelConsts, kc);
   EnvWaveT<SP> w{k->m, k->ev, st, k->L, lds, blockIdx.x, threadIdx.x, k, nullptr};
   w.step(action, dump_mid, trace);
-  if (dump) w.dump(dump);
+  VNL_STEP_ARGS(ka);
+  VNL_LAUNDER(ka);
+  if (VNL_STEP_ARG(ka, dump)) w.dump(VNL_STEP_ARG(ka, dump));
+  if (VNL_STEP_ARG(ka, post).done) {
+    VNL_SYNC_GLOBAL();
+    vnl_post_env<VNL_LANES>(VNL_STEP_ARG(ka, post), blockIdx.x, threadIdx.x);
+  }
 }
 
 template <class SP>
diff --git a/vnl-brax-imitation_amd/csrc/vnl_lib.hip b/vnl-brax-imitation_amd/csrc/vnl_lib.hip
--- a/vnl-brax-imitation_amd/csrc/vnl_lib.hip
+++ b/vnl-brax-imitation_amd/csrc/vnl_lib.hip
@@ -325,6 +325,69 @@
 static VnlDims dims_of(const DevModel& d) {
   return VnlDims{d.nq, d.nv, d.nu, d.nbody, d.njnt, d.ncg, d.ncon, d.nlimit, d.nefc, d.nM, d.iterations, d.ls_iterations, d.eulerdamp,
                  d.root_free, d.max_depth, d.jump_rounds, d.fac_steps, d.fac_route, d.solver_newton, d.blk_cfg, d.path_runs, d.nbody_out};
+}
+
+static int factor_schedule(const int* par, int nv, std::vector<int>& ftime, std::vector<int>& fslot,
+                           std::vector<unsigned char>& hand, std::vector<unsigned short>& plan) {
+  ftime.assign(nv, 0), fslot.assign(nv, 0), hand.assign(nv, 0);
+  std::vector<int> count;
+  for (int j = nv - 1; j >= 0; j--) {
+    int t = 0;
+    for (int i = j + 1; i < nv; i++)
+      if (par[i] == j) t = ftime[i] + 1 > t ? ftime[i] + 1 : t;
+    while ((int)count.size() <= t) count.push_back(0);
+    while (count[t] >= VNL_FAC_LINES) {
+      t++;
+      if ((int)count.size() <= t) count.push_back(0);
+    }
+    ftime[j] = t, fslot[j] = count[t]++;
+  }
+  for (int j = nv - 1; j >= 0; j--)
+    if (par[j] >= 0 && ftime[par[j]] <= ftime[j]) return -1;
+  const int nst = (int)count.size();
+  auto below = [&](int i, int a) {
+    for (int j = par[i]; j >= 0; j = par[j])
+      if (j == a) return true;
+    return false;
+  };
+#ifdef VNL_FACTOR_HANDOFF
+  if (vnl_fac_handoff_room(nv))
+    for (int j = 1; j < nv && j < 64; j++) {
+      if (par[j] != j - 1 || (j & 15) == 0) continue;
+      bool alone = true;
+      for (int i = 0; i < nv; i++) alone = alone && (i == j || ftime[i] != ftime[j] || !below(i, j - 1));
+      hand[j] = alone;
+    }
+#endif
+  plan.assign((size_t)nv * (nst > 0 ? nst : 1), 0);
+  std::vector<unsigned char> late((size_t)nv * (nst > 0 ? nst : 1), 0);
+  for (int j = 0; j < nv; j++)
+    if (hand[j])
+      for (int a = par[par[j]]; a >= 0; a = par[a]) late[(size_t)a * nst + ftime[j]] = 1;
+  for (int j = 0; j < nv; j++)
+    for (int a = par[j]; a >= 0; a = par[a]) {
+      if (hand[j] && a == par[j]) plan[(size_t)a * nst + ftime[j]] |= (unsigned short)(1u << 12);
+      else if (!late[(size_t)a * nst + ftime[j]]) plan[(size_t)a * nst + ftime[j]] |= (unsigned short)(1u << fslot[j]);
+      else if (ftime[a] <= ftime[j] + 1) return -1;
+      else plan[(size_t)a * nst + ftime[j] + 1] |= (unsigned short)(1u << (6 + fslot[j]));
+    }
+  return nst;
+}
+
+extern "C" int vnl_factor_schedule(const int32_t* dof_parent, int32_t nv, int32_t* ftime, int32_t* fslot, uint8_t* hand,
+                                   uint16_t* plan, int32_t* steps) {
+  if (!dof_parent || nv <= 0 || !ftime || !fslot || !hand || !plan || !steps) return fail(VNL_ERR_ARG, "vnl_factor_schedule: null argument");
+  for (int j = 0; j < nv; j++)
+    if (dof_parent[j] >= j || dof_parent[j] < -1) return fail(VNL_ERR_ARG, "vnl_factor_schedule: a parent must precede its dof");
+  std::vector<int> ft, fs;
+  std::vector<unsigned char> hd;
+  std::vector<unsigned short> pl;
+  const int nst = factor_schedule(dof_parent, nv, ft, fs, hd, pl);
+  if (nst < 0) return fail(VNL_ERR_UNSUPPORTED, "factorisation schedule is not causal");
+  for (int j = 0; j < nv; j++) ftime[j] = ft[j], fslot[j] = fs[j], hand[j] = hd[j];
+  for (size_t k = 0; k < (size_t)nv * nst; k++) plan[k] = pl[k];
+  *steps = nst;
+  return VNL_OK;
 }
 
 static int choose_routes(const DevModel& d, int deep1) {
@@ -586,21 +649,16 @@
     UPI(dof_body, I("dof_bodyid")) UPI(dof_Madr, madr) UPI(dof_depth, depth) UPI(M_anc, anc) UPI(M_row, row)
     UPI(dof_ndesc, ndesc)
     limrow_host = limrow;
-    std::vector<int> ftime(nv, 0), fslot(nv, 0), count;
-    for (int j = nv - 1; j >= 0; j--) {
-      int t = 0;
-      for (int i = j + 1; i <= j + ndesc[j]; i++)
-        if (par[i] == j) t = ftime[i] + 1 > t ? ftime[i] + 1 : t;
-      while ((int)count.size() <= t) count.push_back(0);
-      while (count[t] >= VNL_FAC_LINES) {
-        t++;
-        if ((int)count.size() <= t) count.push_back(0);
-      }
-      ftime[j] = t, fslot[j] = count[t]++;
-    }
-    for (int j = nv - 1; j >= 0; j--)
-      if (par[j] >= 0 && ftime[par[j]] <= ftime[j]) return fail(VNL_ERR_UNSUPPORTED, "factorisation schedule is not causal");
-    d.fac_steps = (int)count.size();
+    std::vector<int> ftime, fslot;
+    std::vector<unsigned char> fhand;
+    std::vector<unsigned short> fplan;
+    d.fac_steps = factor_schedule(par.data(), nv, ftime, fslot, fhand, fplan);
+    if (d.fac_steps < 0) return fail(VNL_ERR_UNSUPPORTED, "factorisation schedule is not causal");
+    {
+      const unsigned short* dp = nullptr;
+      if ((rc = upload<unsigned short, unsigned short>(env, fplan, &dp)) != VNL_OK) return rc;
+      d.fac_plan = dp;
+    }
     UPI(dof_ftime, ftime) UPI(dof_fslot, fslot)
     {
       int deep1 = 0;
@@ -993,7 +1051,7 @@
 int vnl_domain_reset_(const KernelConsts* kc, int spec, int B, size_t lds, void* stream, const DevState& ds, const int* start_frame,
                       const vreal* noise, vreal* dump, int* trace);
 int vnl_domain_step_(const KernelConsts* kc, int spec, int B, size_t lds, void* stream, const DevState& ds, const vreal* action,
-                     vreal* dump, vreal* dump_mid, int* trace);
+                     vreal* dump, vreal* dump_mid, int* trace, const vnl_post_desc& post);
 
 static int to_dev_state(const vnl_state* s, DevState* d) {
   const void* ptrs[] = {s->qpos, s->qvel, s->act, s->qacc_warmstart, s->xpos, s->xquat, s->subtree_com1,
@@ -1048,8 +1106,16 @@
   return VNL_OK;
 }
 
-extern "C" int vnl_env_step(vnl_env* env, const float* action, const vnl_state* state, void* stream) {
-  if (!env || !action || !state) return fail(VNL_ERR_ARG, "vnl_env_step: null argument");
+static int check_post_desc(const vnl_post_desc* desc, const char* who) {
+  if (!desc || !desc->done) return fail(VNL_ERR_ARG, "%s: null argument", who);
+  if (desc->num_ops < 0 || desc->num_ops > VNL_POST_MAX_OPS) return fail(VNL_ERR_ARG, "%s: too many ops", who);
+  for (int k = 0; k < desc->num_ops; k++)
+    if (!desc->ops[k].src || desc->ops[k].width <= 0) return fail(VNL_ERR_ARG, "%s: bad op", who);
+  if ((desc->log_reward && !desc->reward)) return fail(VNL_ERR_ARG, "%s: log_reward without reward", who);
+  return VNL_OK;
+}
+
+static int launch_step(vnl_env* env, const float* action, const vnl_state* state, const vnl_post_desc& post, void* stream) {
   DevState ds;
   int rc = to_dev_state(state, &ds);
   if (rc != VNL_OK) return rc;
@@ -1058,19 +1124,33 @@
   if (env->has_dom) {
     HIPCHK((hipError_t)vnl_domain_step_(env->kc, env->spec, env->B, env->lds_bytes, stream, ds, (const vreal*)action,
                                         env->debug == 1 ? env->dump : nullptr, env->debug == 2 ? env->dump : nullptr,
-                                        env->debug ? env->trace : nullptr));
+                                        env->debug ? env->trace : nullptr, post));
     return VNL_OK;
   }
   if (env->spec)
     hipLaunchKernelGGL((vnl_step_kernel<VnlSpecRodent>), dim3(env->B), dim3(64), env->lds_bytes, (hipStream_t)stream,
                        (const KernelConsts*)env->kc, ds, (const vreal*)action, env->debug == 1 ? env->dump : nullptr,
-                       env->debug == 2 ? env->dump : nullptr, env->debug ? env->trace : nullptr);
+                       env->debug == 2 ? env->dump : nullptr, env->debug ? env->trace : nullptr, post);
   else
     hipLaunchKernelGGL((vnl_step_kernel<VnlSpecGeneric>), dim3(env->B), dim3(64), env->lds_bytes, (hipStream_t)stream,
                        (const KernelConsts*)env->kc, ds, (const vreal*)action, env->debug == 1 ? env->dump : nullptr,
-                       env->debug == 2 ? env->dump : nullptr, env->debug ? env->trace : nullptr);
+                       env->debug == 2 ? env->dump : nullptr, env->debug ? env->trace : nullptr, post);
   HIPCHK(hipGetLastError());
   return VNL_OK;
+}
+
+extern "C" int vnl_env_step(vnl_env* env, const float* action, const vnl_state* state, void* stream) {
+  if (!env || !action || !state) return fail(VNL_ERR_ARG, "vnl_env_step: null argument");
+  static const vnl_post_desc no_post = {};
+  return launch_step(env, action, state, no_post, stream);
+}
+
+extern "C" int vnl_env_step_post(vnl_env* env, const float* action, const vnl_state* state, const vnl_post_desc* desc,
+                                 void* stream) {
+  if (!env || !action || !state) return fail(VNL_ERR_ARG, "vnl_env_step_post: null argument");
+  int rc = check_post_desc(desc, "vnl_env_step_post");
+  if (rc != VNL_OK) return rc;
+  return launch_step(env, action, state, *desc, stream);
 }
 
 
@@ -1307,48 +1387,14 @@
 }
 #endif
 
-#ifndef VNL_POST_THREADS
-#define VNL_POST_THREADS 256
-#endif
 __global__ void __launch_bounds__(VNL_POST_THREADS) vnl_post_kernel(vnl_post_desc d) {
-  const unsigned e = blockIdx.x, tid = threadIdx.x;
-  float st = d.steps ? ((d.prev_done && d.prev_done[e] != 0.f) ? 0.f : d.steps[e]) + (float)d.action_repeat : 0.f;
-  float done = d.done[e];
-  bool over = d.steps && st >= (float)d.episode_length;
-  float trunc = over ? 1.f - done : 0.f;
-  done = over ? 1.f : done;
-  __syncthreads();
-  if (tid == 0) {
-    if (d.steps) d.steps[e] = st;
-    if (d.prev_done) d.prev_done[e] = done;
-    d.done[e] = done;
-    if (d.truncation) d.truncation[e] = trunc;
-    if (d.log_reward) d.log_reward[e] = d.reward[e];
-    if (d.log_discount) d.log_discount[e] = 1.f - done;
-    if (d.log_truncation) d.log_truncation[e] = trunc;
-  }
-  const bool reset = done != 0.f;
-  for (int k = 0; k < d.num_ops; k++) {
-    const vnl_post_op& op = d.ops[k];
-    const bool from_first = op.first && reset;
-    const unsigned* src = (const unsigned*)(from_first ? op.first : op.src) + (size_t)e * op.width;
-    unsigned* dst = op.dst ? (unsigned*)op.dst + (size_t)e * op.width : nullptr;
-    unsigned* log = op.log ? (unsigned*)op.log + (size_t)e * op.width : nullptr;
-    const bool store = dst && (from_first || (const float*)op.dst != op.src);
-    for (int i = (int)tid; i < op.width; i += VNL_POST_THREADS) {
-      unsigned v = src[i];
-      if (store) dst[i] = v;
-      if (log) log[i] = v;
-    }
-  }
+  vnl_post_env<VNL_POST_THREADS>(d, blockIdx.x, threadIdx.x);
 }
 
 extern "C" int vnl_rollout_post(const vnl_post_desc* desc, int32_t num_envs, void* stream) {
-  if (!desc || num_envs <= 0 || !desc->done) return fail(VNL_ERR_ARG, "vnl_rollout_post: null argument");
-  if (desc->num_ops < 0 || desc->num_ops > VNL_POST_MAX_OPS) return fail(VNL_ERR_ARG, "vnl_rollout_post: too many ops");
-  for (int k = 0; k < desc->num_ops; k++)
-    if (!desc->ops[k].src || desc->ops[k].width <= 0) return fail(VNL_ERR_ARG, "vnl_rollout_post: bad op");
-  if ((desc->log_reward && !desc->reward)) return fail(VNL_ERR_ARG, "vnl_rollout_post: log_reward without reward");
+  if (num_envs <= 0) return fail(VNL_ERR_ARG, "vnl_rollout_post: null argument");
+  int rc = check_post_desc(desc, "vnl_rollout_post");
+  if (rc != VNL_OK) return rc;
   hipLaunchKernelGGL(vnl_post_kernel, dim3(num_envs), dim3(VNL_POST_THREADS), 0, (hipStream_t)stream, *desc);
   HIPCHK(hipGetLastError());
   return VNL_OK;
diff --git a/vnl-brax-imitation_amd/csrc/vnl_types.h b/vnl-brax-imitation_amd/csrc/vnl_types.h
--- a/vnl-brax-imitation_amd/csrc/vnl_types.h
+++ b/vnl-brax-imitation_amd/csrc/vnl_types.h
@@ -20,6 +20,8 @@
 #define VNL_LIVE_MAX 128
 #define VNL_BLK_W 13
 #define VNL_FAC_LINES 6
+
+constexpr bool vnl_fac_handoff_room(int nv) { return 2 * VNL_FAC_LINES * 16 + 3 <= 6 * nv; }
 
 #define VNL_ROUTE_LDS 1
 #define VNL_ROUTE_ROWS16 2
@@ -62,6 +64,7 @@
   const int* fac_guest;
   const unsigned* blk_tab;
   const unsigned char* fac_match;
+  const unsigned short* fac_plan;
   const int *dof_ndesc;
   const unsigned char* lvl_tab;
   const vreal *dof_armature, *dof_damping;
diff --git a/vnl-brax-imitation_amd/envs/rodent.py b/vnl-brax-imitation_amd/envs/rodent.py
--- a/vnl-brax-imitation_amd/envs/rodent.py
+++ b/vnl-brax-imitation_amd/envs/rodent.py
@@ -353,7 +353,11 @@
         ev = getattr(self, "kernel_events", None)
         if ev is not None:
             ev[0].record()
-        _lib.check(self._L, self._L.vnl_env_step(self._env_h, a.data_ptr(), C.byref(p), self._stream()))
+        post, self.step_post = getattr(self, "step_post", None), None
+        if post is not None:
+            _lib.check(self._L, self._L.vnl_env_step_post(self._env_h, a.data_ptr(), C.byref(p), C.byref(post), self._stream()))
+        else:
+            _lib.check(self._L, self._L.vnl_env_step(self._env_h, a.data_ptr(), C.byref(p), self._stream()))
         if ev is not None:
             ev[1].record()
         self._hold = (a,)
diff --git a/vnl-brax-imitation_amd/ppo_imitation/acting.py b/vnl-brax-imitation_amd/ppo_imitation/acting.py
--- a/vnl-brax-imitation_amd/ppo_imitation/acting.py
+++ b/vnl-brax-imitation_amd/ppo_imitation/acting.py
@@ -54,6 +54,7 @@
 
 
 _DIRECT_LOG = True
+_STEP_EPILOGUE = True
 
 
 def _generate_unroll_fused(fz, env_state: State, policy, key, unroll_length: int, extra_fields) -> Tuple[State, Transition]:
@@ -97,6 +98,7 @@
     act_log = None
     dev_noise = _device_noise(policy)
     direct = dev_noise and _DIRECT_LOG
+    epilogue = _STEP_EPILOGUE and hasattr(base._L, "vnl_env_step_post")
     if direct:
         na = base.action_size
         f32 = lambda *shape: torch.empty((T, *shape), dtype=torch.float32, device=dev)
@@ -111,7 +113,6 @@
             actions, pex = policy(info["traj"], st.obs, None, step_offset=t, advance=False)
         else:
             actions, pex = policy(info["traj"], st.obs, key)
-        base.step(st, actions)
         if px_log is None:
             act_log = new(*actions.shape, like=actions)
             px_log = {k2: new(*v.shape, like=v) for k2, v in pex.items()}
@@ -128,7 +129,12 @@
             keep.append(src)
         d.log_reward, d.log_discount = ptr(rew_log[t]), ptr(disc_log[t])
         d.log_truncation = ptr(sx_log["truncation"][t]) if "truncation" in sx_log else C.c_void_p(0)
-        _lib.check(base._L, base._L.vnl_rollout_post(C.byref(d), B, stream))
+        if epilogue:
+            base.step_post = d
+            base.step(st, actions)
+        else:
+            base.step(st, actions)
+            _lib.check(base._L, base._L.vnl_rollout_post(C.byref(d), B, stream))
         _generate_unroll_fused.hold = keep
     if dev_noise:
         policy.counter.add_(T)
```
